# AlgoLab/PIntron

Hardware: AMD Instinct MI355X
Metric: ESTs aligned/sec (whole node) + DP Mcells/s; bit-exact factorizations vs ref (higher is better)
Workload: dtype u8/int32

## Files before the change

include/pintron_gpu.h:

```cpp
#ifndef PINTRON_GPU_H
#define PINTRON_GPU_H

#include <stddef.h>
#include <stdint.h>

#ifdef __cplusplus
extern "C" {
#endif

#define PGPU_OK       0
#define PGPU_EDEVICE (-5)
#define PGPU_ENOMEM  (-12)
#define PGPU_EINVAL  (-22)
#define PGPU_ENOSPC  (-28)
#define PGPU_ERANGE  (-34)
#define PGPU_ENOSYS  (-38)

typedef struct pgpu_ctx pgpu_ctx;
typedef struct pgpu_index pgpu_index;
typedef struct pgpu_dp_plan pgpu_dp_plan;

int pgpu_init(int device, pgpu_ctx** ctx);
int pgpu_destroy(pgpu_ctx* ctx);
const char* pgpu_last_error(const pgpu_ctx* ctx);
// ... 85 lines not shown
  uint64_t est_off; uint32_t est_len;
  uint32_t first_exon, n_exons;
  uint32_t reserved;
  int32_t  suffpref_length_on_est, suffpref_length_for_intron, suffpref_length_on_gen, min_intron_length;
} pgpu_chain_query;

typedef struct {
  int32_t  status;
  uint32_t done;
  uint32_t dropped_first;
  uint32_t pad;
} pgpu_chain_result;

int pgpu_index_refine_chains(pgpu_ctx* ctx, const pgpu_index* idx, const char* ests, size_t ests_len,
                             const pgpu_factor* exons, size_t n_exons_total,
                             const pgpu_chain_query* q, size_t n,
                             pgpu_factor* out_exons, uint8_t* out_steps, pgpu_chain_result* out);
double pgpu_index_refine_chains_kernel_ms(void);

typedef struct {
  uint32_t min_factor_len;
  uint32_t reserved;
  double   min_string_depth_rate;
} pgpu_pairing_params;

typedef struct { int32_t p, t, l; } pgpu_pairing;

int pgpu_pairings(pgpu_ctx* ctx, const pgpu_index* idx,
                  const char* patterns, const uint64_t* pat_off, size_t n_pat,
                  const pgpu_pairing_params* params,
                  pgpu_pairing* out, size_t out_cap, uint64_t* out_first, size_t* n_out);

typedef struct pgpu_pairing_plan pgpu_pairing_plan;
int pgpu_pairing_plan_create(pgpu_ctx* ctx, const pgpu_index* idx, const char* patterns,
                             const uint64_t* pat_off, size_t n_pat, pgpu_pairing_plan** plan);
int pgpu_pairing_plan_create_resident(pgpu_ctx* ctx, const pgpu_index* idx, const char* patterns,
                                      const uint64_t* pat_off, size_t n_pat, pgpu_pairing_plan** plan);
int pgpu_pairing_plan_run(pgpu_ctx* ctx, pgpu_pairing_plan* plan, const pgpu_pairing_params* params);
uint64_t pgpu_pairing_plan_count(const pgpu_pairing_plan* plan);
uint64_t pgpu_pairing_plan_positions(const pgpu_pairing_plan* plan);
double pgpu_pairing_plan_kernel_ms(const pgpu_pairing_plan* plan, int k);
int pgpu_pairing_plan_fetch(pgpu_ctx* ctx, pgpu_pairing_plan* plan, pgpu_pairing* out, size_t out_cap,
                            uint64_t* out_first);
int pgpu_pairing_plan_destroy(pgpu_ctx* ctx, pgpu_pairing_plan* plan);

typedef struct {
  uint32_t min_factor_len;
  int32_t  min_intron_length, max_intron_length;
  uint32_t max_pairings_in_MEG;
  double   max_prefix_discarded_rate, max_suffix_discarded_rate, max_freq_shortest_pairing;
  uint32_t trans_red, short_edge_comp;
} pgpu_meg_params;

#define PGPU_MEG_MAX_VERTICES 64
#define PGPU_MEG_MAX_DEGREE   32
#define PGPU_MEG_TOO_COMPLEX  1u
#define PGPU_MEG_UNAVAILABLE  2u
int pgpu_pairing_plan_run_meg(pgpu_ctx* ctx, pgpu_pairing_plan* plan, const pgpu_meg_params* params);
uint64_t pgpu_pairing_plan_meg_bytes(const pgpu_pairing_plan* plan);
int pgpu_pairing_plan_fetch_meg(pgpu_ctx* ctx, pgpu_pairing_plan* plan, void* out, size_t out_cap,
                                uint64_t* rec_first);
double pgpu_pairing_plan_meg_ms(const pgpu_pairing_plan* plan);

int pgpu_host_alloc(pgpu_ctx* ctx, size_t bytes, void** out);
int pgpu_host_free(pgpu_ctx* ctx, void* p);

typedef struct pgpu_comm pgpu_comm;
typedef struct { char bytes[128]; } pgpu_comm_id;
int pgpu_comm_unique_id(pgpu_ctx* ctx, pgpu_comm_id* id);
int pgpu_comm_init(pgpu_ctx* ctx, int rank, int world, const pgpu_comm_id* id, pgpu_comm** comm);
int pgpu_gather(pgpu_ctx* ctx, pgpu_comm* comm, const void* send, uint64_t send_bytes,
                void* recv, uint64_t recv_cap, uint64_t* counts);
int pgpu_allgather(pgpu_ctx* ctx, pgpu_comm* comm, const void* send, uint64_t bytes, void* recv);
int pgpu_comm_destroy(pgpu_ctx* ctx, pgpu_comm* comm);

enum pgpu_dp_kind {
  PGPU_DP_ALIGN = 0,
  PGPU_DP_GAP = 1,
  PGPU_DP_ED = 2,
  PGPU_DP_KBAND = 3,
  PGPU_DP_LCF = 4,
  PGPU_DP_BORDERS = 5,
  PGPU_DP_AFFIX = 6,
  PGPU_DP_NKINDS = 7
};

#define PGPU_JOB_A_GENOMIC 1u
#define PGPU_JOB_B_GENOMIC 2u

typedef struct {
  uint32_t kind;
  uint32_t flags;
  uint64_t a_off, b_off;
  uint32_t a_len, b_len;
  uint32_t p0, p1, p2;
  uint32_t tail;
} pgpu_dp_job;

typedef struct {
  int32_t status;
  int32_t v[6];
  int32_t pad;
  uint64_t str[2];
} pgpu_dp_result;

#define PGPU_MAX_ROWS_LEV     65536u
#define PGPU_MAX_ROWS_BORDERS 4096u
#define PGPU_MAX_ROWS_GAP     2048u
#define PGPU_MAX_GAP_SIDE    16000u
#define PGPU_MAX_GAP_CELLS (1ull << 27)
#define PGPU_MAX_COLS      1048576u

int pgpu_dp_plan_create(pgpu_ctx* ctx, const pgpu_index* idx,
                        const pgpu_dp_job* jobs, size_t n_jobs,
                        const char* arena, size_t arena_len, pgpu_dp_plan** plan);
typedef struct { const pgpu_dp_job* jobs; size_t n_jobs; const char* arena; size_t arena_len; } pgpu_dp_part;
int pgpu_dp_plan_create_parts(pgpu_ctx* ctx, const pgpu_index* idx, const pgpu_dp_part* parts, size_t n_parts,
                              pgpu_dp_plan** plan);
int pgpu_dp_plan_launch(pgpu_ctx* ctx, pgpu_dp_plan* plan);
int pgpu_dp_plan_sync(pgpu_ctx* ctx, pgpu_dp_plan* plan);
size_t pgpu_dp_plan_string_bytes(const pgpu_dp_plan* plan);
int pgpu_dp_plan_fetch(pgpu_ctx* ctx, pgpu_dp_plan* plan, pgpu_dp_result* results,
                       char* strings, size_t strings_cap);
int pgpu_dp_plan_results_to_device(pgpu_ctx* ctx, pgpu_dp_plan* plan, void* device_dst, size_t cap);
int pgpu_dp_plan_destroy(pgpu_ctx* ctx, pgpu_dp_plan* plan);

uint64_t pgpu_dp_plan_cells(const pgpu_dp_plan* plan, int kind);
uint64_t pgpu_dp_plan_algo_bytes(const pgpu_dp_plan* plan, int kind);
double   pgpu_dp_plan_kernel_ms(const pgpu_dp_plan* plan, int kind);
uint64_t pgpu_dp_plan_launches(const pgpu_dp_plan* plan, int kind);

typedef struct {
  char     name[48];
  int32_t  kind;
  int32_t  pad;
  uint64_t jobs, cells, algo_bytes;
  double   ms;
  double   t0_ms;
} pgpu_group_info;
int pgpu_dp_plan_n_groups(const pgpu_dp_plan* plan);
int pgpu_dp_plan_group_info(const pgpu_dp_plan* plan, int i, pgpu_group_info* out);

int pgpu_dp_batch(pgpu_ctx* ctx, const pgpu_index* idx,
                  const pgpu_dp_job* jobs, size_t n_jobs, const char* arena, size_t arena_len,
                  pgpu_dp_result* results, char* strings, size_t strings_cap,
                  size_t* strings_used);

#ifdef __cplusplus
}
#endif
#endif
```

pintron_amd/capi.py:

```python
import ctypes as C
import os

_HERE = os.path.dirname(os.path.abspath(__file__))
LIB_PATH = os.path.join(_HERE, "lib", "libpintron_gpu.so")

PGPU_OK, PGPU_EDEVICE, PGPU_ENOMEM, PGPU_EINVAL, PGPU_ENOSPC, PGPU_ERANGE, PGPU_ENOSYS = \
    0, -5, -12, -22, -28, -34, -38
ALIGN, GAP, ED, KBAND, LCF, BORDERS, AFFIX = range(7)
KIND_NAMES = ["ALIGN", "GAP", "ED", "KBAND", "LCF", "BORDERS", "AFFIX"]
JOB_A_GENOMIC, JOB_B_GENOMIC = 1, 2


class DpJob(C.Structure):
    _fields_ = [("kind", C.c_uint32), ("flags", C.c_uint32), ("a_off", C.c_uint64),
                ("b_off", C.c_uint64), ("a_len", C.c_uint32), ("b_len", C.c_uint32),
                ("p0", C.c_uint32), ("p1", C.c_uint32), ("p2", C.c_uint32), ("tail", C.c_uint32)]


class DpResult(C.Structure):
    _fields_ = [("status", C.c_int32), ("v", C.c_int32 * 6), ("pad", C.c_int32),
                ("str", C.c_uint64 * 2)]


class GroupInfo(C.Structure):
    _fields_ = [("name", C.c_char * 48), ("kind", C.c_int32), ("pad", C.c_int32),
                ("jobs", C.c_uint64), ("cells", C.c_uint64), ("algo_bytes", C.c_uint64),
                ("ms", C.c_double), ("t0_ms", C.c_double)]


class PairingParams(C.Structure):
    _fields_ = [("min_factor_len", C.c_uint32), ("reserved", C.c_uint32),
                ("min_string_depth_rate", C.c_double)]


class Pairing(C.Structure):
    _fields_ = [("p", C.c_int32), ("t", C.c_int32), ("l", C.c_int32)]


class FindQuery(C.Structure):
    _fields_ = [("pat_off", C.c_uint64), ("pat_len", C.c_uint32), ("reserved", C.c_uint32),
                ("lo", C.c_uint32), ("hi", C.c_uint32)]


class Intron(C.Structure):
    _fields_ = [("start", C.c_uint32), ("end", C.c_uint32)]


class SexonQuery(C.Structure):
    _fields_ = [("e_off", C.c_uint64), ("elen", C.c_uint32), ("allgstart", C.c_uint32), ("allglen", C.c_uint32),
                ("f1slen", C.c_uint32), ("f2plen", C.c_uint32), ("min_intron_len", C.c_uint32), ("reserved", C.c_uint32)]


class SexonResult(C.Structure):
    _fields_ = [("status", C.c_int32), ("len", C.c_uint32), ("offstart", C.c_uint32), ("offend", C.c_uint32),
                ("gpos", C.c_uint32), ("i1type", C.c_uint32), ("i2type", C.c_uint32), ("pad", C.c_uint32)]


class Factor(C.Structure):
    _fields_ = [("EST_start", C.c_int32), ("EST_end", C.c_int32), ("GEN_start", C.c_int32), ("GEN_end", C.c_int32)]


class RefineQuery(C.Structure):
    _fields_ = [("est_off", C.c_uint64), ("est_len", C.c_uint32), ("flags", C.c_uint32), ("rows_off", C.c_uint64),
                ("dim", C.c_uint32), ("factor_cut", C.c_int32), ("intron_start", C.c_int32), ("intron_end", C.c_int32),
                ("intron_start_on_align", C.c_int32), ("intron_end_on_align", C.c_int32), ("donor", Factor), ("acceptor", Factor),
                ("suffpref_length_on_est", C.c_int32), ("suffpref_length_for_intron", C.c_int32),
                ("suffpref_length_on_gen", C.c_int32), ("min_intron_length", C.c_int32)]


class RefineResult(C.Structure):
    _fields_ = [("status", C.c_int32), ("refined", C.c_int32), ("path", C.c_int32), ("pad", C.c_int32),
                ("donor", Factor), ("acceptor", Factor)]


class ChainQuery(C.Structure):
    _fields_ = [("est_off", C.c_uint64), ("est_len", C.c_uint32), ("first_exon", C.c_uint32), ("n_exons", C.c_uint32),
                ("reserved", C.c_uint32), ("suffpref_length_on_est", C.c_int32), ("suffpref_length_for_intron", C.c_int32),
                ("suffpref_length_on_gen", C.c_int32), ("min_intron_length", C.c_int32)]


class ChainResult(C.Structure):
    _fields_ = [("status", C.c_int32), ("done", C.c_uint32), ("dropped_first", C.c_uint32), ("pad", C.c_uint32)]


REFINE_MAX_DIM, REFINE_MAX_ED, REFINE_FIRST_INTRON = 1024, 256, 1
CHAIN_MAX_EST_WINDOW, CHAIN_MAX_GEN_WINDOW = 192, 320
_FACTOR_DTYPE = [("EST_start", "<i4"), ("EST_end", "<i4"), ("GEN_start", "<i4"), ("GEN_end", "<i4")]
REFINE_QUERY_DTYPE = [("est_off", "<u8"), ("est_len", "<u4"), ("flags", "<u4"), ("rows_off", "<u8"), ("dim", "<u4"),
                      ("factor_cut", "<i4"), ("intron_start", "<i4"), ("intron_end", "<i4"), ("intron_start_on_align", "<i4"),
                      ("intron_end_on_align", "<i4"), ("donor", _FACTOR_DTYPE), ("acceptor", _FACTOR_DTYPE),
                      ("suffpref_length_on_est", "<i4"), ("suffpref_length_for_intron", "<i4"), ("suffpref_length_on_gen", "<i4"),
                      ("min_intron_length", "<i4")]
REFINE_RESULT_DTYPE = [("status", "<i4"), ("refined", "<i4"), ("path", "<i4"), ("pad", "<i4"), ("donor", _FACTOR_DTYPE),
                       ("acceptor", _FACTOR_DTYPE)]

CHAIN_QUERY_DTYPE = [("est_off", "<u8"), ("est_len", "<u4"), ("first_exon", "<u4"), ("n_exons", "<u4"), ("reserved", "<u4"),
                     ("suffpref_length_on_est", "<i4"), ("suffpref_length_for_intron", "<i4"), ("suffpref_length_on_gen", "<i4"),
                     ("min_intron_length", "<i4")]
CHAIN_RESULT_DTYPE = [("status", "<i4"), ("done", "<u4"), ("dropped_first", "<u4"), ("pad", "<u4")]
FACTOR_DTYPE = _FACTOR_DTYPE

SEXON_MAX_ELEN = 64
SEXON_QUERY_DTYPE = [("e_off", "<u8"), ("elen", "<u4"), ("allgstart", "<u4"), ("allglen", "<u4"), ("f1slen", "<u4"),
                     ("f2plen", "<u4"), ("min_intron_len", "<u4"), ("reserved", "<u4"), ("_pad", "<u4")]
SEXON_RESULT_DTYPE = [("status", "<i4"), ("len", "<u4"), ("offstart", "<u4"), ("offend", "<u4"), ("gpos", "<u4"),
                      ("i1type", "<u4"), ("i2type", "<u4"), ("pad", "<u4")]

assert C.sizeof(DpJob) == 48 and C.sizeof(DpResult) == 48 and C.sizeof(FindQuery) == 24
assert C.sizeof(Intron) == 8 and C.sizeof(SexonQuery) == 40 and C.sizeof(SexonResult) == 32
assert C.sizeof(Factor) == 16 and C.sizeof(RefineQuery) == 96 and C.sizeof(RefineResult) == 48
assert C.sizeof(ChainQuery) == 40 and C.sizeof(ChainResult) == 16

EXPORTS = [
    "pgpu_init", "pgpu_destroy", "pgpu_last_error", "pgpu_abi_version", "pgpu_set_timing", "pgpu_device_numa_node",
    "pgpu_index_build", "pgpu_index_destroy", "pgpu_index_suffix_array", "pgpu_index_save", "pgpu_index_load", "pgpu_pairings",
    "pgpu_index_find", "pgpu_index_find_kernel_ms",
    "pgpu_index_classify", "pgpu_index_score5", "pgpu_index_small_exons", "pgpu_index_small_exons_kernel_ms",
    "pgpu_index_refine_introns", "pgpu_index_refine_introns_kernel_ms",
    "pgpu_index_refine_chains", "pgpu_index_refine_chains_kernel_ms",
    "pgpu_pairing_plan_create", "pgpu_pairing_plan_create_resident", "pgpu_pairing_plan_run", "pgpu_pairing_plan_count",
    "pgpu_pairing_plan_positions", "pgpu_pairing_plan_kernel_ms", "pgpu_pairing_plan_fetch",
    "pgpu_pairing_plan_destroy",
    "pgpu_pairing_plan_run_meg", "pgpu_pairing_plan_meg_bytes", "pgpu_pairing_plan_fetch_meg",
    "pgpu_pairing_plan_meg_ms", "pgpu_host_alloc", "pgpu_host_free",
    "pgpu_comm_unique_id", "pgpu_comm_init", "pgpu_gather", "pgpu_allgather", "pgpu_comm_destroy",
    "pgpu_range_push", "pgpu_range_pop", "pgpu_build_info",
    "pgpu_dp_plan_create", "pgpu_dp_plan_create_parts", "pgpu_dp_plan_launch", "pgpu_dp_plan_sync",
    "pgpu_dp_plan_string_bytes", "pgpu_dp_plan_fetch", "pgpu_dp_plan_destroy",
    "pgpu_dp_plan_results_to_device",
    "pgpu_dp_plan_cells", "pgpu_dp_plan_algo_bytes", "pgpu_dp_plan_kernel_ms",
    "pgpu_dp_plan_launches", "pgpu_dp_plan_n_groups", "pgpu_dp_plan_group_info", "pgpu_dp_batch",
]

_lib = None


class PgpuError(RuntimeError):
    def __init__(self, code, msg):
        super().__init__("pgpu error %d: %s" % (code, msg))
        self.code = code


def lib():
    global _lib
    if _lib is None:
        if not os.path.exists(LIB_PATH):
            raise ImportError("%s is missing: run `python -c 'import __graft_entry__ as g; "
                              "g.build()'` (hipcc --offload-arch=gfx950)" % LIB_PATH)
        L = C.CDLL(LIB_PATH)
        vp, u64, sz = C.c_void_p, C.c_uint64, C.c_size_t
        L.pgpu_init.argtypes = [C.c_int, C.POINTER(vp)]
        L.pgpu_destroy.argtypes = [vp]
        L.pgpu_set_timing.argtypes = [vp, C.c_int]
        L.pgpu_last_error.argtypes = [vp]
        L.pgpu_last_error.restype = C.c_char_p
        L.pgpu_build_info.restype = C.c_char_p
        L.pgpu_range_push.argtypes = [C.c_char_p]
        L.pgpu_range_push.restype = None
        L.pgpu_range_pop.restype = None
        L.pgpu_allgather.argtypes = [vp, vp, vp, u64, vp]
        L.pgpu_index_build.argtypes = [vp, C.c_char_p, sz, C.POINTER(vp)]
        L.pgpu_index_destroy.argtypes = [vp, vp]
        L.pgpu_index_save.argtypes = [vp, vp, C.c_char_p, C.c_char_p]
        L.pgpu_index_load.argtypes = [vp, C.c_char_p, C.c_char_p, sz, C.POINTER(vp)]
        L.pgpu_index_suffix_array.argtypes = [vp, vp, C.POINTER(C.c_uint32), sz]
        L.pgpu_index_find.argtypes = [vp, vp, C.c_char_p, sz, C.POINTER(FindQuery), sz,
                                      C.POINTER(C.c_uint32), sz, C.POINTER(u64), C.POINTER(sz)]
        L.pgpu_index_find_kernel_ms.argtypes = [C.c_int]
        L.pgpu_index_find_kernel_ms.restype = C.c_double
        L.pgpu_index_classify.argtypes = [vp, vp, C.POINTER(Intron), sz, C.POINTER(C.c_uint8)]
        L.pgpu_index_score5.argtypes = [vp, vp, C.c_int, C.POINTER(C.c_double), sz]
        L.pgpu_index_small_exons.argtypes = [vp, vp, C.c_char_p, sz, C.POINTER(SexonQuery), sz, C.POINTER(SexonResult)]
        L.pgpu_index_small_exons_kernel_ms.argtypes = []
        L.pgpu_index_small_exons_kernel_ms.restype = C.c_double
        L.pgpu_index_refine_introns.argtypes = [vp, vp, C.c_char_p, sz, C.c_char_p, sz, C.POINTER(RefineQuery), sz,
                                                C.POINTER(RefineResult)]
        L.pgpu_index_refine_introns_kernel_ms.argtypes = []
        L.pgpu_index_refine_introns_kernel_ms.restype = C.c_double
        L.pgpu_index_refine_chains.argtypes = [vp, vp, C.c_char_p, sz, C.POINTER(Factor), sz, C.POINTER(ChainQuery), sz,
                                               C.POINTER(Factor), C.POINTER(C.c_uint8), C.POINTER(ChainResult)]
        L.pgpu_index_refine_chains_kernel_ms.argtypes = []
        L.pgpu_index_refine_chains_kernel_ms.restype = C.c_double
        L.pgpu_pairing_plan_run_meg.argtypes = [vp, vp, vp]
        L.pgpu_pairing_plan_meg_bytes.argtypes = [vp]
        L.pgpu_pairing_plan_meg_bytes.restype = u64
        L.pgpu_pairing_plan_meg_ms.argtypes = [vp]
        L.pgpu_pairing_plan_meg_ms.restype = C.c_double
        L.pgpu_pairing_plan_fetch_meg.argtypes = [vp, vp, vp, sz, C.POINTER(u64)]
        L.pgpu_host_alloc.argtypes = [vp, sz, C.POINTER(vp)]
        L.pgpu_host_free.argtypes = [vp, vp]
        L.pgpu_comm_unique_id.argtypes = [vp, vp]
        L.pgpu_comm_init.argtypes = [vp, C.c_int, C.c_int, vp, C.POINTER(vp)]
        L.pgpu_gather.argtypes = [vp, vp, C.c_char_p, u64, vp, u64, C.POINTER(u64)]
        L.pgpu_comm_destroy.argtypes = [vp, vp]
        L.pgpu_pairings.argtypes = [vp, vp, C.c_char_p, C.POINTER(u64), sz,
                                    C.POINTER(PairingParams), C.POINTER(Pairing), sz,
                                    C.POINTER(u64), C.POINTER(sz)]
        L.pgpu_pairing_plan_create.argtypes = [vp, vp, C.c_char_p, C.POINTER(u64), sz, C.POINTER(vp)]
        L.pgpu_pairing_plan_create_resident.argtypes = [vp, vp, C.c_char_p, C.POINTER(u64), sz, C.POINTER(vp)]
        L.pgpu_pairing_plan_run.argtypes = [vp, vp, C.POINTER(PairingParams)]
        L.pgpu_pairing_plan_count.argtypes = [vp]
        L.pgpu_pairing_plan_count.restype = u64
        L.pgpu_pairing_plan_positions.argtypes = [vp]
        L.pgpu_pairing_plan_positions.restype = u64
        L.pgpu_pairing_plan_kernel_ms.argtypes = [vp, C.c_int]
        L.pgpu_pairing_plan_kernel_ms.restype = C.c_double
        L.pgpu_pairing_plan_fetch.argtypes = [vp, vp, C.POINTER(Pairing), sz, C.POINTER(u64)]
        L.pgpu_pairing_plan_destroy.argtypes = [vp, vp]
        L.pgpu_dp_plan_create_parts.argtypes = [vp, vp, vp, sz, C.POINTER(vp)]
        L.pgpu_dp_plan_create.argtypes = [vp, vp, C.POINTER(DpJob), sz, C.c_char_p, sz,
                                          C.POINTER(vp)]
        L.pgpu_dp_plan_launch.argtypes = [vp, vp]
        L.pgpu_dp_plan_sync.argtypes = [vp, vp]
        L.pgpu_dp_plan_string_bytes.argtypes = [vp]
        L.pgpu_dp_plan_string_bytes.restype = sz
        L.pgpu_dp_plan_fetch.argtypes = [vp, vp, C.POINTER(DpResult), C.c_char_p, sz]
        L.pgpu_dp_plan_destroy.argtypes = [vp, vp]
        L.pgpu_dp_plan_results_to_device.argtypes = [vp, vp, vp, sz]
        for nm in ("pgpu_dp_plan_cells", "pgpu_dp_plan_algo_bytes", "pgpu_dp_plan_launches"):
            getattr(L, nm).argtypes = [vp, C.c_int]
            getattr(L, nm).restype = u64
        L.pgpu_dp_plan_kernel_ms.argtypes = [vp, C.c_int]
        L.pgpu_dp_plan_kernel_ms.restype = C.c_double
        L.pgpu_dp_plan_n_groups.argtypes = [vp]
        L.pgpu_dp_plan_group_info.argtypes = [vp, C.c_int, C.POINTER(GroupInfo)]
        L.pgpu_dp_batch.argtypes = [vp, vp, C.POINTER(DpJob), sz, C.c_char_p, sz,
                                    C.POINTER(DpResult), C.c_char_p, sz, C.POINTER(sz)]
        _lib = L
    return _lib


class Context:

    def __init__(self, device=0):
        self.L = lib()
        self.h = C.c_void_p()
        rc = self.L.pgpu_init(device, C.byref(self.h))
        if rc != PGPU_OK:
            raise PgpuError(rc, "pgpu_init(%d) failed (no usable gfx950 device?)" % device)
        self.L.pgpu_set_timing(self.h, 1)

    def check(self, rc):
        if rc != PGPU_OK:
            raise PgpuError(rc, self.L.pgpu_last_error(self.h).decode())

    def close(self):
        if self.h:
            self.L.pgpu_destroy(self.h)
            self.h = C.c_void_p()

    def __enter__(self):
        return self

    def __exit__(self, *a):
        self.close()


class Index:
    def __init__(self, ctx: Context, genomic: bytes, load_from=None):
        self.ctx = ctx
        self.h = C.c_void_p()
        self.n = len(genomic)
        self.genomic = genomic
        if load_from is None:
            ctx.check(ctx.L.pgpu_index_build(ctx.h, genomic, len(genomic), C.byref(self.h)))
        else:
            rc = ctx.L.pgpu_index_load(ctx.h, os.fsencode(load_from), genomic, len(genomic), C.byref(self.h))
            if rc != PGPU_OK:
                raise PgpuError(rc, "index file %s does not fit this sequence" % load_from)

    def save(self, path):
        self.ctx.check(self.ctx.L.pgpu_index_save(self.ctx.h, self.h, self.genomic, os.fsencode(path)))

    def suffix_array(self):
        import numpy as np
        sa = np.empty(self.n, dtype=np.uint32)
        self.ctx.check(self.ctx.L.pgpu_index_suffix_array(
            self.ctx.h, self.h, sa.ctypes.data_as(C.POINTER(C.c_uint32)), self.n))
        return sa

    def find_raw(self, blob: bytes, queries, n_queries: int, out=None):
        import numpy as np
        first = np.zeros(n_queries + 1, dtype=np.uint64)
        total = C.c_size_t(0)
        rc = self.ctx.L.pgpu_index_find(
            self.ctx.h, self.h, blob, len(blob), queries, n_queries,
            out.ctypes.data_as(C.POINTER(C.c_uint32)) if out is not None else None, len(out) if out is not None else 0,
            first.ctypes.data_as(C.POINTER(C.c_uint64)), C.byref(total))
        return rc, first, total.value

    def find(self, patterns, windows=None):
        import numpy as np
        n = len(patterns)
        if windows is None:
            windows = [(0, self.n)] * n
        if len(windows) != n:
            raise ValueError("one window per pattern")
        lens = np.fromiter((len(p) for p in patterns), dtype=np.uint64, count=n)
        offs = np.zeros(n + 1, dtype=np.uint64)
        np.cumsum(lens, out=offs[1:])
        q = np.zeros(n, dtype=np.dtype([("pat_off", "<u8"), ("pat_len", "<u4"), ("reserved", "<u4"),
                                        ("lo", "<u4"), ("hi", "<u4")]))
        q["pat_off"], q["pat_len"] = offs[:n], lens
        if n:
            w = np.asarray(windows, dtype=np.uint32).reshape(n, 2)
            q["lo"], q["hi"] = w[:, 0], w[:, 1]
# ... 123 lines not shown
        self._blob = b"".join(patterns)
        self._off = np.zeros(len(patterns) + 1, dtype=np.uint64)
        np.cumsum([len(p) for p in patterns], out=self._off[1:])
        self.h = C.c_void_p()
        create = ctx.L.pgpu_pairing_plan_create_resident if resident else ctx.L.pgpu_pairing_plan_create
        ctx.check(create(ctx.h, index.h, self._blob, self._off.ctypes.data_as(C.POINTER(C.c_uint64)),
                         self.n_pat, C.byref(self.h)))

    def run(self, min_factor_len=15, rate=0.2):
        prm = PairingParams(min_factor_len, 0, rate)
        self.ctx.check(self.ctx.L.pgpu_pairing_plan_run(self.ctx.h, self.h, C.byref(prm)))
        return self.ctx.L.pgpu_pairing_plan_count(self.h)

    def stage_ms(self):
        return {s: self.ctx.L.pgpu_pairing_plan_kernel_ms(self.h, k) for k, s in enumerate(self.STAGES)}

    def fetch(self):
        import numpy as np
        n = self.ctx.L.pgpu_pairing_plan_count(self.h)
        out = np.zeros((max(n, 1), 3), dtype=np.int32)
        first = np.zeros(self.n_pat + 1, dtype=np.uint64)
        self.ctx.check(self.ctx.L.pgpu_pairing_plan_fetch(
            self.ctx.h, self.h, out.ctypes.data_as(C.POINTER(Pairing)), n,
            first.ctypes.data_as(C.POINTER(C.c_uint64))))
        return out[:n], first

    def run_meg(self, min_factor_len=15, min_intron_length=40, max_intron_length=0, max_pairings_in_MEG=80,
                max_prefix_discarded_rate=0.6, max_suffix_discarded_rate=0.6, max_freq_shortest_pairing=0.4,
                trans_red=True, short_edge_comp=True):
        prm = MegParams(min_factor_len, min_intron_length, max_intron_length, max_pairings_in_MEG,
                        max_prefix_discarded_rate, max_suffix_discarded_rate, max_freq_shortest_pairing,
                        int(trans_red), int(short_edge_comp))
        self.ctx.check(self.ctx.L.pgpu_pairing_plan_run_meg(self.ctx.h, self.h, C.byref(prm)))
        return self.ctx.L.pgpu_pairing_plan_meg_bytes(self.h)

    def fetch_meg(self):
        import numpy as np
        n = self.ctx.L.pgpu_pairing_plan_meg_bytes(self.h)
        out = np.zeros(max(n, 1), dtype=np.uint8)
        first = np.zeros(self.n_pat + 1, dtype=np.uint64)
        self.ctx.check(self.ctx.L.pgpu_pairing_plan_fetch_meg(
            self.ctx.h, self.h, out.ctypes.data_as(C.c_void_p), n, first.ctypes.data_as(C.POINTER(C.c_uint64))))
        raw = out.tobytes()
        return [raw[int(first[i]):int(first[i + 1])] for i in range(self.n_pat)]

    def close(self):
        if self.h:
            self.ctx.L.pgpu_pairing_plan_destroy(self.ctx.h, self.h)
            self.h = C.c_void_p()


class DpPart(C.Structure):
    _fields_ = [("jobs", C.c_void_p), ("n_jobs", C.c_size_t), ("arena", C.c_void_p), ("arena_len", C.c_size_t)]


class JobList:

    def __init__(self):
        self.jobs = []
        self.chunks = []
        self.size = 0

    def _put(self, b: bytes) -> int:
        off = self.size
        self.chunks.append(b)
        self.size += len(b)
        return off

    def add(self, kind, a: bytes, b: bytes, p0=0, p1=0, p2=0, b_tail: bytes = b"",
            a_gen_off=None, b_gen_off=None, tail=None):
        flags = 0
        if a_gen_off is None:
            a_off = self._put(a)
        else:
            a_off, flags = a_gen_off, flags | JOB_A_GENOMIC
        if b_gen_off is None:
            b_off = self._put(b + b_tail)
        else:
            b_off, flags = b_gen_off, flags | JOB_B_GENOMIC
        self.jobs.append(DpJob(kind, flags, a_off, b_off, len(a), len(b), p0, p1, p2,
                               len(b_tail) if tail is None else tail))
        return len(self.jobs) - 1

    def arrays(self):
        arr = (DpJob * max(len(self.jobs), 1))(*self.jobs)
        return arr, b"".join(self.chunks)


class Plan:
    def __init__(self, ctx: Context, joblist: JobList, index: Index = None):
        self.ctx = ctx
        self.n = len(joblist.jobs)
        self._jobs, self._arena = joblist.arrays()
        self.h = C.c_void_p()
        ctx.check(ctx.L.pgpu_dp_plan_create(ctx.h, index.h if index else None, self._jobs, self.n,
                                            self._arena, len(self._arena), C.byref(self.h)))

    @classmethod
    def from_parts(cls, ctx: Context, joblists, index: Index = None):
        self = cls.__new__(cls)
        self.ctx = ctx
        self.n = sum(len(jl.jobs) for jl in joblists)
        self._keep = []
        parts = (DpPart * max(len(joblists), 1))()
        for k, jl in enumerate(joblists):
            jobs, arena = jl.arrays()
            buf = C.create_string_buffer(arena, len(arena) + 1)
            self._keep += [jobs, buf]
            parts[k] = DpPart(C.cast(jobs, C.c_void_p), len(jl.jobs), C.cast(buf, C.c_void_p), len(arena))
        self.h = C.c_void_p()
        ctx.check(ctx.L.pgpu_dp_plan_create_parts(ctx.h, index.h if index else None, parts, len(joblists), C.byref(self.h)))
        return self

    def launch(self):
        self.ctx.check(self.ctx.L.pgpu_dp_plan_launch(self.ctx.h, self.h))

    def sync(self):
        self.ctx.check(self.ctx.L.pgpu_dp_plan_sync(self.ctx.h, self.h))

    def fetch(self):
        L = self.ctx.L
        nbytes = L.pgpu_dp_plan_string_bytes(self.h)
        res = (DpResult * max(self.n, 1))()
        sbuf = C.create_string_buffer(max(nbytes, 1))
        self.ctx.check(L.pgpu_dp_plan_fetch(self.ctx.h, self.h, res, sbuf, nbytes))
        return res, sbuf.raw

    def results_to_device(self, device_ptr: int, cap: int):
        self.ctx.check(self.ctx.L.pgpu_dp_plan_results_to_device(self.ctx.h, self.h, device_ptr, cap))

    def groups(self):
        L = self.ctx.L
        out = []
        for i in range(L.pgpu_dp_plan_n_groups(self.h)):
            g = GroupInfo()
            L.pgpu_dp_plan_group_info(self.h, i, C.byref(g))
            out.append(dict(name=g.name.decode(), kind=g.kind, jobs=g.jobs, cells=g.cells,
                            algo_bytes=g.algo_bytes, ms=g.ms, t0_ms=g.t0_ms))
        return out

    def close(self):
        if self.h:
            self.ctx.L.pgpu_dp_plan_destroy(self.ctx.h, self.h)
            self.h = C.c_void_p()


def cstr(buf: bytes, off: int) -> bytes:
    end = buf.index(b"\0", off)
    return buf[off:end]


def decode(kind, r: DpResult, strings: bytes):
    v = r.v
    if r.status != PGPU_OK:
        return dict(status=r.status)
    if kind == ALIGN:
        return dict(status=0, score=v[0], dim=v[1], ea=cstr(strings, r.str[0]),
                    ga=cstr(strings, r.str[1]))
    if kind == GAP:
        return dict(status=0, dim=v[0], factor_cut=v[1], intron_start=v[2], intron_end=v[3],
                    intron_start_on_align=v[4], intron_end_on_align=v[5],
                    ea=cstr(strings, r.str[0]), ga=cstr(strings, r.str[1]))
    if kind == ED:
        return dict(status=0, score=v[0])
    if kind == KBAND:
        return dict(status=0, ok=v[0], edit=v[1], dust=v[2])
    if kind == LCF:
        return dict(status=0, len=v[0], occ1=v[1], occ2=v[2])
    if kind == BORDERS:
        return dict(status=0, ok=v[0], off_p=v[1], off_t1=v[2], off_t2=v[3], ed=v[4])
    if kind == AFFIX:
        return dict(status=0, valid=v[0], ecut=v[1], gcut=v[2])
    raise ValueError(kind)


def run_jobs(ctx: Context, joblist: JobList, index: Index = None):
    plan = Plan(ctx, joblist, index)
    try:
        plan.launch()
        plan.sync()
        res, strings = plan.fetch()
        return [decode(joblist.jobs[i].kind, res[i], strings) for i in range(plan.n)]
    finally:
        plan.close()
```

pintron_amd/csrc/pgpu_api.hip:

```cpp
#include <algorithm>
#include <cstdarg>
#include <cstdio>
#include <cstdlib>
#include <cstring>
#include <ctime>
#include <time.h>
#include <new>
#include <mutex>
#include <vector>

#include "pgpu_internal.h"
#include "pgpu_index.h"

struct BufPool {
  static constexpr int SLOTS = 24;
  void* ptr[SLOTS] = {nullptr};
  size_t cap[SLOTS] = {0};
  bool busy = false;
  int sharers = 0;
  const void* owner = nullptr;
};

struct pgpu_ctx {
  int device = 0;
  hipStream_t stream = nullptr;
  char err[512] = {0};
  BufPool pools[2];
  bool timing = false;
  static constexpr int NAUX = 4;
  hipStream_t aux[NAUX] = {nullptr};
  hipEvent_t ev_upload = nullptr;
  hipEvent_t ev_aux[NAUX] = {nullptr};
  hipEvent_t ev_done = nullptr;
  hipEvent_t ev_wait = nullptr;
  long wait_poll_us = 20;
  int poison = -1;
  void* pin[2] = {nullptr, nullptr};
  size_t pin_cap[2] = {0, 0};
  std::vector<hipEvent_t> ev_pool;
};

static int wait_stream(pgpu_ctx* ctx, hipStream_t st) {
  if (hipEventRecord(ctx->ev_done, st) != hipSuccess) return -1;
  if (ctx->wait_poll_us != 0) {
    for (;;) {
      const hipError_t q = hipEventQuery(ctx->ev_done);
      if (q == hipSuccess) return 0;
      if (q != hipErrorNotReady) return -1;
      if (ctx->wait_poll_us > 0) { struct timespec ts = {0, ctx->wait_poll_us * 1000L}; nanosleep(&ts, nullptr); }
    }
  }
  return hipEventSynchronize(ctx->ev_done) == hipSuccess ? 0 : -1;
}

static void* pinned(pgpu_ctx* ctx, int slot, size_t bytes) {
  if (ctx->pin_cap[slot] < bytes) {
    if (ctx->pin[slot]) (void)hipHostFree(ctx->pin[slot]);
    ctx->pin[slot] = nullptr; ctx->pin_cap[slot] = 0;
    const size_t want = std::max<size_t>(bytes + bytes / 2 + 4096, (size_t)2 << 20);
    if (hipHostMalloc(&ctx->pin[slot], want, hipHostMallocDefault) != hipSuccess) return nullptr;
    pgpu_trace_alloc(slot ? "ctx pinned down" : "ctx pinned up", ctx->pin[slot], want);
    ctx->pin_cap[slot] = want;
  }
  return ctx->pin[slot];
}

bool pgpu_ctx_pool_acquire(pgpu_ctx* ctx, int pool) {
  if (ctx->pools[pool].busy) return false;
  ctx->pools[pool].busy = true;
  return true;
}
void pgpu_ctx_pool_release(pgpu_ctx* ctx, int pool) { ctx->pools[pool].busy = false; ctx->pools[pool].owner = nullptr; }
bool pgpu_ctx_pool_share(pgpu_ctx* ctx, int pool) {
  BufPool& p = ctx->pools[pool];
  if (p.busy && p.sharers == 0) return false;
  p.busy = true; ++p.sharers;
  return true;
}
void pgpu_ctx_pool_unshare(pgpu_ctx* ctx, int pool, const void* who) {
  BufPool& p = ctx->pools[pool];
  if (p.owner == who) p.owner = nullptr;
  if (p.sharers > 0 && --p.sharers == 0) p.busy = false;
}
void pgpu_ctx_pool_set_owner(pgpu_ctx* ctx, int pool, const void* who) { ctx->pools[pool].owner = who; }
const void* pgpu_ctx_pool_owner(const pgpu_ctx* ctx, int pool) { return ctx->pools[pool].owner; }
void* pgpu_ctx_pool_get(pgpu_ctx* ctx, int pool, int slot, size_t bytes) {
  BufPool& p = ctx->pools[pool];
  if (bytes == 0) bytes = 16;
  if (p.cap[slot] < bytes) {
    if (p.ptr[slot]) (void)hipFree(p.ptr[slot]);
    p.ptr[slot] = nullptr; p.cap[slot] = 0;
    const size_t want = std::max<size_t>(bytes + bytes / 2 + 4096, pool == 0 ? (size_t)64 << 20 : 0);
    if (hipMalloc(&p.ptr[slot], want) != hipSuccess) {
      if (hipMalloc(&p.ptr[slot], bytes) != hipSuccess) return nullptr;
      p.cap[slot] = bytes;
    } else p.cap[slot] = want;
    pgpu_trace_alloc(pool ? "device pool 1" : "device pool 0", p.ptr[slot], p.cap[slot]);
  }
  return p.ptr[slot];
}
bool pgpu_ctx_timing(const pgpu_ctx* ctx) { return ctx->timing; }

extern "C" int pgpu_device_numa_node(pgpu_ctx* ctx) {
  if (!ctx) return -1;
  char bdf[64] = {0};
  if (hipDeviceGetPCIBusId(bdf, (int)sizeof bdf - 1, ctx->device) != hipSuccess) return -1;
  for (char* c = bdf; *c; ++c) if (*c >= 'A' && *c <= 'F') *c = (char)(*c - 'A' + 'a');
  char path[160];
  snprintf(path, sizeof path, "/sys/bus/pci/devices/%s/numa_node", bdf);
  FILE* f = fopen(path, "r");
  if (!f) return -1;
  int node = -1;
  if (fscanf(f, "%d", &node) != 1) node = -1;
  fclose(f);
  return node;
}

extern "C" int pgpu_set_timing(pgpu_ctx* ctx, int enabled) {
  if (!ctx) return PGPU_EINVAL;
  ctx->timing = enabled != 0;
  return PGPU_OK;
}

static int set_err(pgpu_ctx* ctx, int code, const char* fmt, ...) {
  if (ctx) {
    va_list ap;
    va_start(ap, fmt);
    vsnprintf(ctx->err, sizeof(ctx->err), fmt, ap);
    va_end(ap);
  }
  return code;
}

#define HIP_TRY(ctx, call)                                                                  \
  do {                                                                                      \
    hipError_t e_ = (call);                                                                 \
    if (e_ != hipSuccess)                                                                   \
      return set_err(ctx, e_ == hipErrorOutOfMemory ? PGPU_ENOMEM : PGPU_EDEVICE,           \
                     "%s failed: %s (%s:%d)", #call, hipGetErrorString(e_), __FILE__, __LINE__); \
  } while (0)

hipStream_t pgpu_ctx_stream(pgpu_ctx* ctx) { return ctx->stream; }
hipError_t pgpu_ctx_wait(pgpu_ctx* ctx) {
  if (ctx->wait_poll_us <= 0) return hipStreamSynchronize(ctx->stream);
  hipError_t e = hipEventRecord(ctx->ev_wait, ctx->stream);
  if (e != hipSuccess) return e;
  const struct timespec ts = {0, ctx->wait_poll_us * 5000L};
  for (;;) {
    e = hipEventQuery(ctx->ev_wait);
    if (e != hipErrorNotReady) return e;
    nanosleep(&ts, nullptr);
  }
}
int pgpu_ctx_bind(pgpu_ctx* ctx) {
  const hipError_t e = hipSetDevice(ctx->device);
  return e == hipSuccess ? PGPU_OK : set_err(ctx, PGPU_EDEVICE, "hipSetDevice(%d) failed: %s", ctx->device, hipGetErrorString(e));
}
int pgpu_ctx_fail(pgpu_ctx* ctx, int code, const char* msg) { return set_err(ctx, code, "%s", msg); }

extern "C" int pgpu_abi_version(void) { return 1; }

#include <dlfcn.h>
namespace {
struct Roctx { int state = 0; int (*push)(const char*) = nullptr; int (*pop)() = nullptr; };
Roctx g_roctx;
bool roctx_ready() {
  if (g_roctx.state) return g_roctx.state > 0;
  bool want = false;
  { const char* m = getenv("PGPU_MARKERS"); if (m) want = m[0] != '0'; else {
      const char* t = getenv("ROCP_TOOL_LIBRARIES"); const char* pl = getenv("LD_PRELOAD");
      want = (t && t[0]) || (pl && strstr(pl, "rocprofiler")); } }
  if (want) {
    void* so = nullptr;
    for (const char* n : { "librocprofiler-sdk-roctx.so.1", "librocprofiler-sdk-roctx.so", "libroctx64.so.4", "libroctx64.so" })
      if ((so = dlopen(n, RTLD_NOW | RTLD_GLOBAL)) != nullptr) break;
    if (so) {
      *(void**)(&g_roctx.push) = dlsym(so, "roctxRangePushA");
      *(void**)(&g_roctx.pop) = dlsym(so, "roctxRangePop");
    }
  }
  g_roctx.state = (g_roctx.push && g_roctx.pop) ? 1 : -1;
  return g_roctx.state > 0;
}
}
extern "C" void pgpu_range_push(const char* name) { if (roctx_ready()) g_roctx.push(name ? name : ""); }
extern "C" void pgpu_range_pop(void) { if (roctx_ready()) g_roctx.pop(); }

extern "C" const char* pgpu_build_info(void) {
  static char info[256];
  if (!info[0]) {
    const char* stamp = __DATE__ " " __TIME__ " " __VERSION__;
    unsigned long long h = 1469598103934665603ull;
    for (const char* c = stamp; *c; ++c) { h ^= (unsigned char)*c; h *= 1099511628211ull; }
    snprintf(info, sizeof info, "libpintron_gpu abi %d, gfx950, built %s %s, hip %d.%d.%d, stamp %016llx", pgpu_abi_version(), __DATE__,
             __TIME__, HIP_VERSION_MAJOR, HIP_VERSION_MINOR, HIP_VERSION_PATCH, h);
  }
  return info;
}

static bool aux_stream(pgpu_ctx* ctx, int i) {
  if (!ctx->aux[i] && hipStreamCreateWithFlags(&ctx->aux[i], hipStreamNonBlocking) != hipSuccess) { ctx->aux[i] = nullptr; return false; }
  if (!ctx->ev_aux[i] && hipEventCreateWithFlags(&ctx->ev_aux[i], hipEventDisableTiming) != hipSuccess) { ctx->ev_aux[i] = nullptr; return false; }
  return true;
}

static hipEvent_t g_base_event[64];
static std::mutex g_base_mu;
static hipEvent_t base_event(int device, hipStream_t st) {
  if (device < 0 || device >= 64) return nullptr;
  std::lock_guard<std::mutex> lk(g_base_mu);
  if (!g_base_event[device]) {
    hipEvent_t e = nullptr;
    if (hipEventCreate(&e) == hipSuccess && hipEventRecord(e, st) == hipSuccess && hipEventSynchronize(e) == hipSuccess) g_base_event[device] = e;
    else if (e) hipEventDestroy(e);
  }
  return g_base_event[device];
}

extern "C" int pgpu_init(int device, pgpu_ctx** out) {
  if (!out) return PGPU_EINVAL;
  *out = nullptr;
  int n = 0;
  if (hipGetDeviceCount(&n) != hipSuccess || n <= 0) return PGPU_EDEVICE;
  if (device < 0 || device >= n) return PGPU_EINVAL;
  hipDeviceProp_t prop;
  if (hipGetDeviceProperties(&prop, device) != hipSuccess) return PGPU_EDEVICE;
  if (strncmp(prop.gcnArchName, "gfx950", 6) != 0) return PGPU_EDEVICE;
  if (hipSetDevice(device) != hipSuccess) return PGPU_EDEVICE;
  pgpu_ctx* ctx = new (std::nothrow) pgpu_ctx();
  if (!ctx) return PGPU_ENOMEM;
  ctx->device = device;
  if (hipStreamCreateWithFlags(&ctx->stream, hipStreamNonBlocking) != hipSuccess) {
    delete ctx;
    return PGPU_EDEVICE;
  }
  if (hipEventCreateWithFlags(&ctx->ev_upload, hipEventDisableTiming) != hipSuccess) { delete ctx; return PGPU_EDEVICE; }
  if (hipEventCreateWithFlags(&ctx->ev_done, hipEventDisableTiming | hipEventBlockingSync) != hipSuccess) { delete ctx; return PGPU_EDEVICE; }
  if (hipEventCreateWithFlags(&ctx->ev_wait, hipEventDisableTiming) != hipSuccess) { delete ctx; return PGPU_EDEVICE; }
  { const char* f = getenv("PGPU_WAIT"); if (f) ctx->wait_poll_us = atol(f); }
  { const char* f = getenv("PGPU_POISON"); if (f && f[0]) ctx->poison = atoi(f) & 255; }
  base_event(device, ctx->stream);
  *out = ctx;
  return PGPU_OK;
}

extern "C" int pgpu_destroy(pgpu_ctx* ctx) {
  if (!ctx) return PGPU_EINVAL;
  hipSetDevice(ctx->device);
  hipStreamSynchronize(ctx->stream);
  for (auto& pl : ctx->pools) for (auto& q : pl.ptr) if (q) hipFree(q);
  for (auto& a : ctx->aux) if (a) { hipStreamSynchronize(a); hipStreamDestroy(a); }
  if (ctx->ev_upload) hipEventDestroy(ctx->ev_upload);
  if (ctx->ev_done) hipEventDestroy(ctx->ev_done);
  if (ctx->ev_wait) hipEventDestroy(ctx->ev_wait);
  for (auto& e : ctx->ev_aux) if (e) hipEventDestroy(e);
  for (auto& e : ctx->ev_pool) if (e) hipEventDestroy(e);
  for (auto& q : ctx->pin) if (q) hipHostFree(q);
  hipStreamDestroy(ctx->stream);
  delete ctx;
  return PGPU_OK;
}

extern "C" const char* pgpu_last_error(const pgpu_ctx* ctx) { return ctx ? ctx->err : "null context"; }

namespace {

uint32_t row_class(uint32_t rows) {
  if (rows > 4096u) return ROW_CLASS_STRIPS;
  uint32_t R = 1;
  while (64u * R < rows) R <<= 1;
  return R;
}

enum DpRoute : uint8_t {
  RT_ALIGN_STRIPS, RT_ALIGN_COOP, RT_ALIGN_WAVE, RT_GAP_SLOW, RT_GAP, RT_ED, RT_KBAND, RT_LCF,
  RT_BORDERS_SLOW, RT_BORDERS_COOP, RT_BORDERS_WAVE, RT_AFFIX_STRIPS, RT_AFFIX_COOP, RT_AFFIX_WAVE,
  RT_LCFSA, RT_LCFW, RT_ALIGNB,
  RT_BATCH,
  RT_COUNT
};

enum BatchPlace { OUTSIDE, SEGMENT, ROLE_BORDERS, ROLE_AFFIX, ROLE_ALIGN };

using WsBytes = size_t (*)(uint32_t la, uint32_t lb, uint32_t R);
size_t ws_align_wave(uint32_t, uint32_t lb, uint32_t) { return ((size_t)lb + 64) * 64; }
size_t ws_align_coop(uint32_t, uint32_t lb, uint32_t R) { return ((size_t)lb + 256) * 256 * align_coop_entry_bytes(R); }
size_t ws_align_strips(uint32_t la, uint32_t lb, uint32_t R) {
  return 2 * strip_bnd_bytes(lb) + (size_t)((la + 4095u) / 4096u) * ((size_t)lb + 64) * 64 * align_entry_bytes(R);
}
size_t ws_gap(uint32_t, uint32_t lb, uint32_t R) { return ((size_t)lb + 64) * 64 * gap_entry_bytes(R); }
size_t ws_gap_slow(uint32_t la, uint32_t lb, uint32_t) { return (size_t)9 * ((size_t)la + 1) * 4 + ((size_t)la + 1) * ((size_t)lb + 1); }
size_t ws_borders_slow(uint32_t la, uint32_t, uint32_t) { return (size_t)7 * ((size_t)la + 1) * 4; }
size_t ws_affix_strips(uint32_t, uint32_t lb, uint32_t) { return 2 * strip_bnd_bytes(lb); }
size_t ws_ed_strips(uint32_t la, uint32_t lb, uint32_t R) { return R == ROW_CLASS_STRIPS ? 2 * strip_bnd_bytes(std::max(la, lb)) : 0; }

using AlgoBytes = uint64_t (*)(uint64_t la, uint64_t lb, uint64_t p2);
uint64_t bytes_operands(uint64_t la, uint64_t lb, uint64_t) { return la + lb; }
uint64_t bytes_align(uint64_t la, uint64_t lb, uint64_t) { return la + lb + la * lb + 3 * (la + lb); }
uint64_t bytes_gap(uint64_t la, uint64_t lb, uint64_t) { return la + lb + 3 * la * lb + 3 * (la + lb); }
uint64_t bytes_borders(uint64_t la, uint64_t lb, uint64_t p2) { return la + std::min(lb, 2 * std::min(la + p2, lb)) + 2 * 8 * la; }
uint64_t bytes_lcfsa(uint64_t, uint64_t lb, uint64_t) { return lb + 64u * 96u; }

struct RouteInfo {
  const char* name;
  int kind;
  int family;
  WsBytes ws_bytes;
  bool strings;
  uint32_t cell_factor;
  AlgoBytes algo_bytes;
  BatchPlace place;
  int seg_pos;
  uint32_t big_from;
  long weight; bool by_rows; int lane; DpLauncher launch;
  bool keyed;
};

constexpr RouteInfo ROUTES[] = {
  {"lev_wave<ALIGN,strips>",  PGPU_DP_ALIGN,   KF_ALIGN,   ws_align_strips, true,  1, bytes_align,    OUTSIDE,      0,  0,  5000, false,  2, launch_align_big,    false},
  {"align_coop",              PGPU_DP_ALIGN,   KF_ALIGN,   ws_align_coop,   true,  1, bytes_align,    ROLE_ALIGN,   0,  0,     0, false,  0, nullptr,             false},
  {"lev_wave<ALIGN>",         PGPU_DP_ALIGN,   KF_ALIGN,   ws_align_wave,   true,  1, bytes_align,    SEGMENT,      1,  0,     0, false,  0, nullptr,             false},
  {"gap_slow",                PGPU_DP_GAP,     KF_GAP,     ws_gap_slow,     true,  3, bytes_gap,      OUTSIDE,      0,  0,  4000, false,  3, launch_gap_slow,     false},
  {"gap_wave",                PGPU_DP_GAP,     KF_GAP,     ws_gap,          true,  3, bytes_gap,      SEGMENT,      2,  8,  4000, false,  3, launch_gap_big,      false},
  {"lev_wave<ED>",            PGPU_DP_ED,      KF_ED,      ws_ed_strips,    false, 1, bytes_operands, SEGMENT,      8, 32,  1000, false,  1, launch_ed_big,       false},
  {"lev_wave<KBAND>",         PGPU_DP_KBAND,   KF_KBAND,   ws_ed_strips,    false, 1, bytes_operands, SEGMENT,      3, 32,  2000, false,  2, launch_kband_big,    false},
  {"lcf",                     PGPU_DP_LCF,     KF_LCF,     nullptr,         false, 1, bytes_operands, OUTSIDE,      0,  0,  3000, false,  3, launch_lcf,          true},
  {"borders_slow",            PGPU_DP_BORDERS, KF_BORDERS, ws_borders_slow, false, 2, bytes_borders,  OUTSIDE,      0,  0, 10000, true,   1, launch_borders_slow, false},
  {"borders_coop",            PGPU_DP_BORDERS, KF_BORDERS, nullptr,         false, 2, bytes_borders,  ROLE_BORDERS, 0,  0, 10000, true,   1, launch_borders_coop, false},
  {"lev_wave<BORDERS,R=1>",   PGPU_DP_BORDERS, KF_BORDERS, nullptr,         false, 2, bytes_borders,  SEGMENT,      4,  0,     0, false,  0, nullptr,             false},
  {"lev_wave<AFFIX,strips>",  PGPU_DP_AFFIX,   KF_AFFIX,   ws_affix_strips, false, 1, bytes_operands, OUTSIDE,      0,  0, 10000, true,   0, launch_affix_strips, false},
  {"affix_coop",              PGPU_DP_AFFIX,   KF_AFFIX,   nullptr,         false, 1, bytes_operands, ROLE_AFFIX,   0,  0,     0, false,  0, nullptr,             false},
  {"lev_wave<AFFIX,R=1>",     PGPU_DP_AFFIX,   KF_AFFIX,   nullptr,         false, 1, bytes_operands, SEGMENT,      5,  0,     0, false,  0, nullptr,             false},
  {"lcf_sa",                  PGPU_DP_LCF,     KF_LCFSA,   nullptr,         false, 0, bytes_lcfsa,    SEGMENT,      6,  0,     0, false,  0, nullptr,             false},
  {"lcf_small",               PGPU_DP_LCF,     KF_LCFW,    nullptr,         false, 1, bytes_operands, SEGMENT,      7,  0,     0, false,  0, nullptr,             false},
  {"align_band",              PGPU_DP_ALIGN,   KF_ALIGNB,  ws_align_coop,   true,  1, bytes_align,    SEGMENT,      0,  0,     0, false,  0, nullptr,             false},
  {"dp_batch",                PGPU_DP_ALIGN,   KF_COUNT,   nullptr,         false, 0, nullptr,        OUTSIDE,      0,  0, 20000, false, -1, nullptr,             false},
};
static_assert(sizeof ROUTES / sizeof ROUTES[0] == RT_COUNT, "one entry per route, in the enum's order");
constexpr bool routes_consistent() {
  unsigned seen = 0;
  for (const RouteInfo& ri : ROUTES) {
    if (ri.lane >= pgpu_ctx::NAUX) return false;
    if (ri.big_from && (ri.place != SEGMENT || !ri.launch)) return false;
    if (ri.place != SEGMENT) continue;
    if (ri.seg_pos >= MAX_WAVE_SEGS || (seen & (1u << ri.seg_pos))) return false;
    seen |= 1u << ri.seg_pos;
  }
  return true;
}
static_assert(routes_consistent(), "routing table");

struct Slice { size_t first = 0, count = 0; uint64_t cells = 0, algo_bytes = 0; };

struct Group {
  DpRoute route;
  Slice own;
  uint32_t max_chunks = 0, max_l2 = 0;
  uint32_t max_rows = 0;
  hipEvent_t ev0 = nullptr, ev1 = nullptr;
  float ms = 0.f;
  float t0_ms = -1.f;
};

struct BatchPlan {
  BatchDesc desc;
  uint32_t bc_max_rows;
  int ab_start, ab_count;
};

struct Keyed { DevJob j; uint64_t a_off, b_off; bool ag, bg; DpRoute route; uint32_t R; uint64_t size; };

}

struct pgpu_dp_plan {
  size_t n_jobs = 0;
  std::vector<Group> groups;
  std::vector<pgpu_dp_result> prefill;
  DevJob* d_jobs = nullptr;
  DevResult* d_results = nullptr;
  uint8_t* d_arena = nullptr;
  uint8_t* d_ws = nullptr;
  uint8_t* d_strs = nullptr;
  unsigned long long* d_keys = nullptr;
  size_t n_dev_jobs = 0, ws_bytes = 0, strs_bytes = 0, n_keys = 0;
  uint64_t cells[PGPU_DP_NKINDS] = {0}, algo_bytes[PGPU_DP_NKINDS] = {0};
  double ms[PGPU_DP_NKINDS] = {0};
  uint64_t launches[PGPU_DP_NKINDS] = {0};
  bool launched = false, synced = false;
  bool pooled = false;
  pgpu_ctx* owner = nullptr;
  uint8_t* d_base = nullptr;
  uint8_t* h_up = nullptr; uint8_t* h_down = nullptr;
  size_t up_bytes = 0, off_results = 0, down_bytes = 0;
  BatchPlan batch{};
  std::vector<uint32_t> lcf_out;
  size_t off_keys = 0;
  bool lcf_decoded = false;
};

static void plan_free(pgpu_dp_plan* p) {
  if (!p) return;
  if (p->pooled) pgpu_ctx_pool_release(p->owner, 0);
  else {
    for (auto& g : p->groups) {
      if (g.ev0) hipEventDestroy(g.ev0);
      if (g.ev1) hipEventDestroy(g.ev1);
    }
    if (p->d_base) hipFree(p->d_base);
    if (p->h_up) hipHostFree(p->h_up);
    if (p->h_down) hipHostFree(p->h_down);
  }
  delete p;
}

extern "C" int pgpu_dp_plan_create(pgpu_ctx* ctx, const pgpu_index* idx, const pgpu_dp_job* jobs,
                                   size_t n_jobs, const char* arena, size_t arena_len,
                                   pgpu_dp_plan** out) {
  const pgpu_dp_part one = { jobs, n_jobs, arena, arena_len };
  return pgpu_dp_plan_create_parts(ctx, idx, &one, 1, out);
}

static int classify(const pgpu_dp_job& in, const char* arena, bool ag, bool bg, const LcfIndexView& lcf, Keyed& k) {
  const uint32_t la = in.a_len, lb = in.b_len;
  k.size = (uint64_t)la * lb;
  switch (in.kind) {
    case PGPU_DP_ALIGN:
      if (la > PGPU_MAX_ROWS_LEV || lb > PGPU_MAX_COLS) return PGPU_ERANGE;
      k.R = row_class(la);
      if (la > 64u && la <= 4096u && (la > lb ? la - lb : lb - la) <= ALIGN_BAND_HALF) k.route = RT_ALIGNB;
      else k.route = k.R == 1 ? RT_ALIGN_WAVE : (k.R == ROW_CLASS_STRIPS ? RT_ALIGN_STRIPS : RT_ALIGN_COOP);
      return PGPU_OK;
    case PGPU_DP_GAP:
      if (lb > PGPU_MAX_GAP_SIDE || la > PGPU_MAX_GAP_SIDE || ((uint64_t)la + 1) * ((uint64_t)lb + 1) > PGPU_MAX_GAP_CELLS) return PGPU_ERANGE;
      k.R = la > PGPU_MAX_ROWS_GAP ? ROW_CLASS_STRIPS : row_class(la);
      k.route = k.R == ROW_CLASS_STRIPS ? RT_GAP_SLOW : RT_GAP;
      return PGPU_OK;
    case PGPU_DP_ED:
      if (std::min(la, lb) > PGPU_MAX_ROWS_LEV || std::max(la, lb) > PGPU_MAX_COLS) return PGPU_ERANGE;
      k.R = row_class(std::min(la, lb)); k.route = RT_ED;
      return PGPU_OK;
    case PGPU_DP_KBAND: {
      const uint32_t n = std::max(la, lb), m = std::min(la, lb), ub = in.p0;
      if (n > PGPU_MAX_COLS || m > PGPU_MAX_ROWS_LEV) return PGPU_ERANGE;
      k.R = row_class(m); k.route = RT_KBAND;
      if (2ull * ub + 1 < n) k.size = (uint64_t)m * (2ull * ub + 1);
      return PGPU_OK;
    }
    case PGPU_DP_LCF:
      if (lb > 65535u || la >= (1u << 28)) return PGPU_ERANGE;
      k.R = 0; k.route = RT_LCF;
      if (lcf.focc && lcf.rmq && ag && !bg && in.a_off == 0 && la <= lcf.first_bad && lb <= 64u) {
        const unsigned char* b = (const unsigned char*)arena + in.b_off;
        bool acgt = true;
        uint32_t n_wild = 0, wild_at = 0;
        for (uint32_t q = 0; q < lb && acgt; ++q) {
          if (b[q] == 'N' || b[q] == 'n') { ++n_wild; wild_at = q; }
          else acgt = b[q] == 'A' || b[q] == 'C' || b[q] == 'G' || b[q] == 'T';
        }
        if (acgt && n_wild <= 1u) { k.route = RT_LCFSA; k.j.p0 = n_wild ? wild_at + 1u : 0u; }
      }
      if (k.route == RT_LCF && (uint64_t)la * lb <= 16384u && la + lb <= 4096u) k.route = RT_LCFW;
      return PGPU_OK;
    case PGPU_DP_BORDERS: {
      const uint64_t t_win = std::min<uint64_t>((uint64_t)la + in.p2, lb);
      if (la > PGPU_MAX_ROWS_LEV || t_win > PGPU_MAX_COLS) return PGPU_ERANGE;
      if (in.p0 > in.p1 || in.p1 > la) return PGPU_EINVAL;
      k.R = row_class(la); k.size = (uint64_t)la * t_win;
      k.route = k.R == 1 ? RT_BORDERS_WAVE : (k.R == ROW_CLASS_STRIPS ? RT_BORDERS_SLOW : RT_BORDERS_COOP);
      return PGPU_OK;
    }
    case PGPU_DP_AFFIX:
      if (la > PGPU_MAX_ROWS_LEV || lb > PGPU_MAX_COLS) return PGPU_ERANGE;
      k.R = row_class(la);
      k.route = k.R == 1 ? RT_AFFIX_WAVE : (k.R == ROW_CLASS_STRIPS ? RT_AFFIX_STRIPS : RT_AFFIX_COOP);
      return PGPU_OK;
    default: return PGPU_EINVAL;
  }
}

static std::vector<Keyed> classify_jobs(const pgpu_dp_part* parts, size_t n_parts, size_t n_jobs, const LcfIndexView& lcf,
                                        bool has_genomic, size_t gen_len, std::vector<pgpu_dp_result>& prefill) {
  std::vector<Keyed> v;
  v.reserve(n_jobs);
  prefill.assign(n_jobs, pgpu_dp_result{});
  size_t i = 0, part_base = 0;
  for (size_t q = 0; q < n_parts; part_base += parts[q].arena_len, ++q)
    for (size_t w = 0; w < parts[q].n_jobs; ++w, ++i) {
      const pgpu_dp_job& in = parts[q].jobs[w];
      const size_t own_arena = parts[q].arena_len;
      prefill[i].status = PGPU_EINVAL;
      if (in.kind >= PGPU_DP_NKINDS) continue;
      const bool ag = in.flags & PGPU_JOB_A_GENOMIC, bg = in.flags & PGPU_JOB_B_GENOMIC;
      if ((ag || bg) && !has_genomic) continue;
      const size_t a_space = ag ? gen_len : own_arena, b_space = bg ? gen_len : own_arena;
      if (in.a_off > a_space || in.a_len > a_space - in.a_off) continue;
      if (in.b_off > b_space || in.b_len > b_space - in.b_off) continue;
      Keyed k{};
      k.a_off = in.a_off + (ag ? 0 : part_base); k.b_off = in.b_off + (bg ? 0 : part_base); k.ag = ag; k.bg = bg;
      k.j.la = in.a_len; k.j.lb = in.b_len;
      k.j.p0 = in.p0; k.j.p1 = in.p1; k.j.p2 = in.p2; k.j.tail = in.tail;
      k.j.out_idx = (uint32_t)i;
      prefill[i].status = classify(in, parts[q].arena, ag, bg, lcf, k);
      if (prefill[i].status != PGPU_OK) continue;
      k.j.r_class = k.R;
      v.push_back(k);
    }
  return v;
}

static void sort_jobs(std::vector<Keyed>& v) {
  auto key_of = [](const Keyed& k) -> uint32_t {
    uint32_t rcls = 0;
    while ((1u << rcls) < k.R) ++rcls;
    const uint32_t mag = 63u - (uint32_t)__builtin_clzll(k.size | 1ull);
    return ((uint32_t)ROUTES[k.route].family << 10) | ((7u - rcls) << 6) | (63u - mag);
  };
  constexpr uint32_t NKEYS = (uint32_t)KF_COUNT << 10;
  std::vector<uint32_t> start(NKEYS + 1, 0);
  std::vector<uint32_t> kk(v.size());
  for (size_t q = 0; q < v.size(); ++q) { kk[q] = key_of(v[q]); ++start[kk[q] + 1]; }
  for (uint32_t c = 0; c < NKEYS; ++c) start[c + 1] += start[c];
  std::vector<Keyed> sorted;
  sorted.resize(v.size());
  for (size_t q = 0; q < v.size(); ++q) sorted[start[kk[q]]++] = v[q];
  v.swap(sorted);
}

struct DpSpace { size_t ws = 0, strs = 0; };
static DpSpace assign_workspace(std::vector<Keyed>& v, std::vector<uint32_t>& lcf_out) {
  DpSpace sp;
  for (auto& k : v) {
    const RouteInfo& ri = ROUTES[k.route];
    const size_t wb = ri.ws_bytes ? ri.ws_bytes(k.j.la, k.j.lb, k.R) : 0;
    if (wb) { k.j.ws_off = sp.ws; sp.ws += wb; }
    if (ri.strings) { k.j.str_off = sp.strs; sp.strs += 2 * ((size_t)k.j.la + k.j.lb + 1); }
    if (ri.keyed) lcf_out.push_back(k.j.out_idx);
    sp.ws = (sp.ws + 15) & ~(size_t)15;
  }
  return sp;
}

static void form_groups(const std::vector<Keyed>& v, std::vector<Group>& groups, std::vector<Slice>& batched,
                        uint64_t* cells, uint64_t* algo_bytes) {
  for (size_t i = 0, j; i < v.size(); i = j) {
    const RouteInfo& ri = ROUTES[v[i].route];
    Group g{};
    g.route = v[i].route;
    Slice big, rest;
    for (j = i; j < v.size() && v[j].route == g.route && !(ri.keyed && j - i == 65535); ++j) {
      const Keyed& k = v[j];
      Slice& s = ri.big_from && k.R >= ri.big_from ? big : rest;
      ++s.count; s.cells += ri.cell_factor * k.size; s.algo_bytes += ri.algo_bytes(k.j.la, k.j.lb, k.j.p2);
      g.max_rows = std::max(g.max_rows, k.j.la);
      if (ri.keyed) {
        g.max_chunks = std::max(g.max_chunks, (uint32_t)(((uint64_t)k.j.la + k.j.lb + 254) / 256));
        g.max_l2 = std::max(g.max_l2, k.j.lb);
      }
    }
    big.first = i; rest.first = i + big.count;
    cells[ri.kind] += big.cells + rest.cells; algo_bytes[ri.kind] += big.algo_bytes + rest.algo_bytes;
    const bool in_batch = ri.place == ROLE_BORDERS ? dp_batch_lds_bytes(true, 1, g.max_rows, 1, 1) <= DP_BATCH_MAX_LDS : ri.place != OUTSIDE;
    g.own = in_batch ? big : rest;
    groups.push_back(g);
    batched.push_back(in_batch ? rest : Slice{});
  }
}

static void form_batch(std::vector<Group>& groups, const std::vector<Slice>& batched, BatchPlan& b) {
  Group m{};
  m.route = RT_BATCH;
  const Slice* seg[MAX_WAVE_SEGS] = {nullptr};
  int seg_family[MAX_WAVE_SEGS] = {0};
  BatchDesc& d = b.desc;
  for (size_t gi = 0; gi < groups.size(); ++gi) {
    const Slice& s = batched[gi];
    if (!s.count) continue;
    const RouteInfo& ri = ROUTES[groups[gi].route];
    switch (ri.place) {
      case SEGMENT:      seg[ri.seg_pos] = &s; seg_family[ri.seg_pos] = ri.family; break;
      case ROLE_BORDERS: d.bc_start = (int)s.first; d.bc_count = (int)s.count; b.bc_max_rows = groups[gi].max_rows; break;
      case ROLE_AFFIX:   d.ac_start = (int)s.first; d.ac_count = (int)s.count; break;
      case ROLE_ALIGN:   d.lc_start = (int)s.first; d.lc_count = (int)s.count; break;
      case OUTSIDE:      break;
    }
    if (groups[gi].route == RT_ALIGNB) { b.ab_start = (int)s.first; b.ab_count = (int)s.count; }
    m.own.count += s.count; m.own.cells += s.cells; m.own.algo_bytes += s.algo_bytes;
  }
  int waves = 0;
  for (int q = 0; q < MAX_WAVE_SEGS; ++q) {
    if (!seg[q]) continue;
    d.segs.family[d.segs.n] = seg_family[q]; d.segs.start[d.segs.n] = (int)seg[q]->first; d.segs.count[d.segs.n] = (int)seg[q]->count;
    ++d.segs.n;
    waves += (int)seg[q]->count;
  }
  d.wave_blocks = (waves + 3) / 4;
  if (m.own.count) groups.push_back(m);
}

static int plan_upload(pgpu_ctx* ctx, pgpu_dp_plan* p, const pgpu_dp_part* parts, size_t n_parts, size_t arena_len,
                       const std::vector<Keyed>& v, const uint8_t* d_gen) {
  if (ctx->timing) {
    const size_t need = 2 * p->groups.size();
    if (p->pooled) {
      while (ctx->ev_pool.size() < need) {
        hipEvent_t e = nullptr;
        if (hipEventCreate(&e) != hipSuccess) return set_err(ctx, PGPU_EDEVICE, "hipEventCreate failed");
        ctx->ev_pool.push_back(e);
      }
      for (size_t g = 0; g < p->groups.size(); ++g) { p->groups[g].ev0 = ctx->ev_pool[2 * g]; p->groups[g].ev1 = ctx->ev_pool[2 * g + 1]; }
    } else {
      for (auto& g : p->groups)
        if (hipEventCreate(&g.ev0) != hipSuccess || hipEventCreate(&g.ev1) != hipSuccess) return set_err(ctx, PGPU_EDEVICE, "hipEventCreate failed");
    }
  }

  auto up256 = [](size_t x) { return (x + 255) & ~(size_t)255; };
  const size_t n_jobs = p->n_jobs, strs = p->strs_bytes;
  const size_t off_arena = 0;
  const size_t off_jobs = up256(arena_len + 16);
  const size_t off_keys = up256(off_jobs + std::max<size_t>(v.size(), 1) * sizeof(DevJob));
  const size_t off_results = up256(off_keys + (p->n_keys + 1) * sizeof(unsigned long long));
  const size_t off_strs = off_results + std::max<size_t>(n_jobs, 1) * sizeof(DevResult);
  const size_t off_ws = up256(off_strs + strs + 16);
  const size_t total = off_ws + p->ws_bytes + 16;
  p->up_bytes = off_strs;
  p->off_results = off_results;
  p->off_keys = off_keys;
  p->down_bytes = (off_strs - off_keys) + strs;
  if (p->pooled) {
    p->d_base = (uint8_t*)pgpu_ctx_pool_get(ctx, 0, 0, total);
    p->h_up = (uint8_t*)pinned(ctx, 0, p->up_bytes);
    p->h_down = (uint8_t*)pinned(ctx, 1, p->down_bytes + 16);
  } else {
    void* q = nullptr;
    if (hipMalloc(&q, total) == hipSuccess) p->d_base = (uint8_t*)q;
    if (hipHostMalloc(&q, p->up_bytes, hipHostMallocDefault) == hipSuccess) p->h_up = (uint8_t*)q;
    if (hipHostMalloc(&q, p->down_bytes + 16, hipHostMallocDefault) == hipSuccess) p->h_down = (uint8_t*)q;
  }
  if (!p->d_base || !p->h_up || !p->h_down)
    return set_err(ctx, PGPU_ENOMEM, "batch buffers (%zu B device, %zu B pinned) could not be allocated", total, p->up_bytes + p->down_bytes);
  p->d_arena = p->d_base + off_arena;
  p->d_jobs = (DevJob*)(p->d_base + off_jobs);
  p->d_keys = (unsigned long long*)(p->d_base + off_keys);
  p->d_results = (DevResult*)(p->d_base + off_results);
  p->d_strs = p->d_base + off_strs;
  p->d_ws = p->d_base + off_ws;

  {
    size_t at = off_arena;
    for (size_t q = 0; q < n_parts; ++q) { if (parts[q].arena_len) memcpy(p->h_up + at, parts[q].arena, parts[q].arena_len); at += parts[q].arena_len; }
  }
  DevJob* hj = (DevJob*)(p->h_up + off_jobs);
  for (size_t q = 0; q < v.size(); ++q) {
    DevJob d = v[q].j;
    d.a = (v[q].ag ? d_gen : p->d_arena) + v[q].a_off;
    d.b = (v[q].bg ? d_gen : p->d_arena) + v[q].b_off;
    hj[q] = d;
  }
  memset(p->h_up + off_keys, 0, off_results - off_keys);
  if (n_jobs) memcpy(p->h_up + off_results, p->prefill.data(), n_jobs * sizeof(DevResult));
  const hipError_t e = hipMemcpyAsync(p->d_base, p->h_up, p->up_bytes, hipMemcpyHostToDevice, ctx->stream);
  if (e != hipSuccess) return set_err(ctx, PGPU_EDEVICE, "upload failed: %s", hipGetErrorString(e));
  if (ctx->poison >= 0) {
    if (hipMemsetAsync(p->d_base + off_strs, ctx->poison, total - off_strs, ctx->stream) != hipSuccess) return set_err(ctx, PGPU_EDEVICE, "poison fill failed");
  }
  return PGPU_OK;
}

extern "C" int pgpu_dp_plan_create_parts(pgpu_ctx* ctx, const pgpu_index* idx, const pgpu_dp_part* parts,
                                         size_t n_parts, pgpu_dp_plan** out) {
  if (!ctx || !out || (n_parts && !parts)) return set_err(ctx, PGPU_EINVAL, "bad argument");
  *out = nullptr;
  size_t n_jobs = 0, arena_len = 0;
  for (size_t q = 0; q < n_parts; ++q) {
    if ((parts[q].n_jobs && !parts[q].jobs) || (parts[q].arena_len && !parts[q].arena)) return set_err(ctx, PGPU_EINVAL, "bad argument");
    n_jobs += parts[q].n_jobs; arena_len += parts[q].arena_len;
  }
  if (n_jobs >= (size_t)1 << 30) return set_err(ctx, PGPU_EINVAL, "too many jobs");
  HIP_TRY(ctx, hipSetDevice(ctx->device));
  pgpu_dp_plan* p = new (std::nothrow) pgpu_dp_plan();
  if (!p) return set_err(ctx, PGPU_ENOMEM, "out of host memory");
  p->n_jobs = n_jobs;
  p->owner = ctx;
  p->pooled = pgpu_ctx_pool_acquire(ctx, 0);
  p->batch.desc.ix = pgpu_index_lcf_view(idx);

  std::vector<Keyed> v = classify_jobs(parts, n_parts, n_jobs, p->batch.desc.ix, idx != nullptr, idx ? pgpu_index_length(idx) : 0, p->prefill);
  sort_jobs(v);
  const DpSpace sp = assign_workspace(v, p->lcf_out);
  p->ws_bytes = sp.ws; p->strs_bytes = sp.strs; p->n_keys = p->lcf_out.size(); p->n_dev_jobs = v.size();
  std::vector<Slice> batched;
  form_groups(v, p->groups, batched, p->cells, p->algo_bytes);
  form_batch(p->groups, batched, p->batch);

  const int rc = plan_upload(ctx, p, parts, n_parts, arena_len, v, idx ? pgpu_index_genomic(idx) : nullptr);
  if (rc != PGPU_OK) { plan_free(p); return rc; }
  *out = p;
  return PGPU_OK;
}

extern "C" int pgpu_dp_plan_launch(pgpu_ctx* ctx, pgpu_dp_plan* p) {
  if (!ctx || !p) return set_err(ctx, PGPU_EINVAL, "bad argument");
  HIP_TRY(ctx, hipSetDevice(ctx->device));
  p->synced = false; p->lcf_decoded = false;
  std::vector<size_t> order;
  std::vector<size_t> key_of(p->groups.size(), 0);
  auto weight = [&](size_t gi) -> long {
    const RouteInfo& ri = ROUTES[p->groups[gi].route];
    return ri.weight + (ri.by_rows ? (long)p->groups[gi].max_rows : 0);
  };
  {
    size_t kb = 0;
    for (size_t gi = 0; gi < p->groups.size(); ++gi) {
      const Group& g = p->groups[gi];
      if (ROUTES[g.route].keyed) { key_of[gi] = kb; kb += g.own.count; }
      if (g.own.count) order.push_back(gi);
    }
    std::stable_sort(order.begin(), order.end(), [&](size_t a, size_t b) { return weight(a) > weight(b); });
  }
  unsigned used_mask = 0;
  for (size_t gi : order) { const int l = ROUTES[p->groups[gi].route].lane; if (l >= 0) used_mask |= 1u << l; }
  if (used_mask) {
    HIP_TRY(ctx, hipEventRecord(ctx->ev_upload, ctx->stream));
    for (int i = 0; i < pgpu_ctx::NAUX; ++i)
      if (used_mask & (1u << i)) {
        if (!aux_stream(ctx, i)) return set_err(ctx, PGPU_EDEVICE, "auxiliary stream %d could not be created", i);
        HIP_TRY(ctx, hipStreamWaitEvent(ctx->aux[i], ctx->ev_upload, 0));
      }
  }
  for (size_t gi : order) {
    Group& g = p->groups[gi];
    const RouteInfo& ri = ROUTES[g.route];
    hipStream_t st = ri.lane >= 0 ? ctx->aux[ri.lane] : ctx->stream;
    if (g.ev0) HIP_TRY(ctx, hipEventRecord(g.ev0, st));
    pgpu_range_push(ri.name);
    struct PopAtExit { ~PopAtExit() { pgpu_range_pop(); } } pop_at_exit;
    if (g.route == RT_BATCH) {
      if (!launch_dp_batch(p->d_jobs, p->batch.desc, p->batch.bc_max_rows, p->d_results, p->d_ws, p->d_strs, st))
        return set_err(ctx, PGPU_EDEVICE, "batch launch: LDS budget exceeded");
    } else {
      if (!ri.launch) return set_err(ctx, PGPU_EDEVICE, "no kernel for %zu jobs of %s outside the batch launch", g.own.count, ri.name);
      ri.launch(DpLaunch{p->d_jobs + g.own.first, (int)g.own.count, g.max_rows, g.max_chunks, g.max_l2, p->d_results, p->d_ws,
                         p->d_strs, p->d_keys + key_of[gi], st});
    }
    if (g.ev1) HIP_TRY(ctx, hipEventRecord(g.ev1, st));
    if (g.route == RT_BATCH) launch_align_fallback(p->d_jobs + p->batch.ab_start, p->batch.ab_count, p->d_results, p->d_ws, p->d_strs, st);
    HIP_TRY(ctx, hipGetLastError());
  }
  for (int i = 0; i < pgpu_ctx::NAUX; ++i) {
    if (!(used_mask & (1u << i))) continue;
    HIP_TRY(ctx, hipEventRecord(ctx->ev_aux[i], ctx->aux[i]));
    HIP_TRY(ctx, hipStreamWaitEvent(ctx->stream, ctx->ev_aux[i], 0));
  }
  if (p->down_bytes)
    HIP_TRY(ctx, hipMemcpyAsync(p->h_down, p->d_base + p->off_keys, p->down_bytes, hipMemcpyDeviceToHost, ctx->stream));
  p->launched = true;
  return PGPU_OK;
}

static void decode_lcf_keys(pgpu_dp_plan* p) {
  if (p->lcf_decoded) return;
  p->lcf_decoded = true;
  const unsigned long long* keys = (const unsigned long long*)p->h_down;
  DevResult* res = (DevResult*)(p->h_down + (p->off_results - p->off_keys));
  for (size_t k = 0; k < p->lcf_out.size(); ++k) {
    DevResult& r = res[p->lcf_out[k]];
    const unsigned long long key = keys[k];
    r.status = PGPU_OK;
    r.v[0] = (int32_t)(key >> 44);
    r.v[1] = key ? (int32_t)(0x0FFFFFFFu - (uint32_t)((key >> 16) & 0x0FFFFFFFu)) : 0;
    r.v[2] = key ? (int32_t)(0xFFFFu - (uint32_t)(key & 0xFFFFu)) : 0;
  }
}

extern "C" int pgpu_dp_plan_sync(pgpu_ctx* ctx, pgpu_dp_plan* p) {
  if (!ctx || !p) return set_err(ctx, PGPU_EINVAL, "bad argument");
  if (wait_stream(ctx, ctx->stream) != 0) return set_err(ctx, PGPU_EDEVICE, "waiting for the batch failed");
  p->synced = p->launched;
  if (p->launched) {
    decode_lcf_keys(p);
    for (int k = 0; k < PGPU_DP_NKINDS; ++k) { p->ms[k] = 0; p->launches[k] = 0; }
    for (auto& g : p->groups) {
      float ms = 0.f;
      if (!g.own.count) continue;
      if (g.ev0 && g.ev1 && hipEventElapsedTime(&ms, g.ev0, g.ev1) == hipSuccess) g.ms = ms;
      if (g.ev0) { hipEvent_t b = base_event(ctx->device, ctx->stream); float t0 = 0.f; g.t0_ms = (b && hipEventElapsedTime(&t0, b, g.ev0) == hipSuccess) ? t0 : -1.f; }
      p->ms[ROUTES[g.route].kind] += g.ms;
      p->launches[ROUTES[g.route].kind] += 1;
    }
  }
  return PGPU_OK;
}

extern "C" size_t pgpu_dp_plan_string_bytes(const pgpu_dp_plan* p) { return p ? p->strs_bytes : 0; }

extern "C" int pgpu_dp_plan_fetch(pgpu_ctx* ctx, pgpu_dp_plan* p, pgpu_dp_result* results,
                                  char* strings, size_t cap) {
  if (!ctx || !p || (p->n_jobs && !results)) return set_err(ctx, PGPU_EINVAL, "bad argument");
  if (p->strs_bytes && strings && cap < p->strs_bytes) return set_err(ctx, PGPU_ENOSPC, "string buffer too small: need %zu", p->strs_bytes);
  if (!p->launched) return set_err(ctx, PGPU_EINVAL, "the plan has not been launched");
  if (!p->synced && wait_stream(ctx, ctx->stream) != 0) return set_err(ctx, PGPU_EDEVICE, "result download failed");
  p->synced = true;
  decode_lcf_keys(p);
  const size_t rb = p->n_jobs * sizeof(DevResult);
  if (rb) memcpy(results, p->h_down + (p->off_results - p->off_keys), rb);
  if (p->strs_bytes && strings) memcpy(strings, p->h_down + (p->down_bytes - p->strs_bytes), p->strs_bytes);
  return PGPU_OK;
}

extern "C" int pgpu_dp_plan_results_to_device(pgpu_ctx* ctx, pgpu_dp_plan* p, void* dst, size_t cap) {
  if (!ctx || !p || !dst) return set_err(ctx, PGPU_EINVAL, "bad argument");
  const size_t bytes = p->n_jobs * sizeof(DevResult);
  if (cap < bytes) return set_err(ctx, PGPU_ENOSPC, "device buffer too small: need %zu", bytes);
  HIP_TRY(ctx, hipSetDevice(ctx->device));
  if (!p->launched) return set_err(ctx, PGPU_EINVAL, "the plan has not been launched");
  if (!p->synced && wait_stream(ctx, ctx->stream) != 0) return set_err(ctx, PGPU_EDEVICE, "result download failed");
  p->synced = true;
  decode_lcf_keys(p);
  if (bytes) HIP_TRY(ctx, hipMemcpyAsync(dst, p->h_down + (p->off_results - p->off_keys), bytes, hipMemcpyHostToDevice, ctx->stream));
  HIP_TRY(ctx, hipStreamSynchronize(ctx->stream));
  return PGPU_OK;
}

extern "C" int pgpu_dp_plan_destroy(pgpu_ctx* ctx, pgpu_dp_plan* p) {
  if (!ctx || !p) return PGPU_EINVAL;
  hipSetDevice(ctx->device);
  hipStreamSynchronize(ctx->stream);
  plan_free(p);
  return PGPU_OK;
}

extern "C" uint64_t pgpu_dp_plan_cells(const pgpu_dp_plan* p, int kind) {
  return (p && kind >= 0 && kind < PGPU_DP_NKINDS) ? p->cells[kind] : 0;
}
extern "C" uint64_t pgpu_dp_plan_algo_bytes(const pgpu_dp_plan* p, int kind) {
  return (p && kind >= 0 && kind < PGPU_DP_NKINDS) ? p->algo_bytes[kind] : 0;
}
extern "C" double pgpu_dp_plan_kernel_ms(const pgpu_dp_plan* p, int kind) {
  return (p && kind >= 0 && kind < PGPU_DP_NKINDS) ? p->ms[kind] : 0.0;
}
extern "C" uint64_t pgpu_dp_plan_launches(const pgpu_dp_plan* p, int kind) {
  return (p && kind >= 0 && kind < PGPU_DP_NKINDS) ? p->launches[kind] : 0;
}

extern "C" int pgpu_dp_plan_n_groups(const pgpu_dp_plan* p) { return p ? (int)p->groups.size() : 0; }

extern "C" int pgpu_dp_plan_group_info(const pgpu_dp_plan* p, int i, pgpu_group_info* out) {
  if (!p || !out || i < 0 || i >= (int)p->groups.size()) return PGPU_EINVAL;
  const Group& g = p->groups[i];
  memset(out, 0, sizeof(*out));
  snprintf(out->name, sizeof(out->name), "%s", ROUTES[g.route].name);
  out->kind = ROUTES[g.route].kind; out->jobs = g.own.count; out->cells = g.own.cells; out->algo_bytes = g.own.algo_bytes;
  out->ms = g.ms; out->t0_ms = g.t0_ms;
  return PGPU_OK;
}

extern "C" int pgpu_dp_batch(pgpu_ctx* ctx, const pgpu_index* idx, const pgpu_dp_job* jobs,
                             size_t n_jobs, const char* arena, size_t arena_len,
                             pgpu_dp_result* results, char* strings, size_t strings_cap,
                             size_t* strings_used) {
  pgpu_dp_plan* p = nullptr;
  int rc = pgpu_dp_plan_create(ctx, idx, jobs, n_jobs, arena, arena_len, &p);
  if (rc != PGPU_OK) return rc;
  if (strings_used) *strings_used = p->strs_bytes;
  rc = pgpu_dp_plan_launch(ctx, p);
  if (rc == PGPU_OK) rc = pgpu_dp_plan_sync(ctx, p);
  if (rc == PGPU_OK) rc = pgpu_dp_plan_fetch(ctx, p, results, strings, strings_cap);
  pgpu_dp_plan_destroy(ctx, p);
  return rc;
}
```

pintron_amd/csrc/pgpu_chain.hip:

```cpp
#include <stdlib.h>
#include <string.h>

#include "pgpu_internal.h"
#include "pgpu_wave_dp.h"
#include "pgpu_refine_body.h"

namespace {

constexpr int MAX_EW = PGPU_CHAIN_MAX_EST_WINDOW;
constexpr int MAX_GW = PGPU_CHAIN_MAX_GEN_WINDOW;
constexpr uint32_t CHAIN_R = 4;
static_assert(MAX_EW <= 64 * (int)CHAIN_R && MAX_EW + MAX_GW <= MAX_DIM, "the caps fit the sweep and the decision");

constexpr size_t WS_DIRS = ((size_t)MAX_GW + 64) * 64 * CHAIN_R;
constexpr size_t WS_STRS = WS_DIRS;
constexpr size_t WS_STRS_BYTES = (2 * ((size_t)MAX_EW + MAX_GW + 1) + 15) & ~(size_t)15;
constexpr size_t WS_WIN_E = WS_STRS + WS_STRS_BYTES;
constexpr size_t WS_WIN_G = WS_WIN_E + ((MAX_EW + 15) & ~15);
constexpr size_t WS_RES = WS_WIN_G + ((MAX_GW + 15) & ~15);
constexpr size_t WS_WAVE = (WS_RES + sizeof(DevResult) + 255) & ~(size_t)255;

struct ChainLds {
  union {
    struct { __attribute__((aligned(16))) uint8_t win[TB_WIN_BYTES]; uint8_t path[TB_PATH]; } tb;
    RefineLds refine;
  };
};

__device__ __forceinline__ int append_piece(uint8_t* dst, int at, int cap, const Seq& s, int index, int length, int lane) {
  if (at > cap) return at;
  if (index < 0) { length += index; index = 0; }
  if (length > cap - at + 1) length = cap - at + 1;
  const Piece p = substring(s, index, length, lane);
  if (p.len > cap - at) return cap + 1;
  for (int k = lane; k < p.len; k += 64) dst[at + k] = s.p[p.start + k];
  return at + p.len;
}

__global__ __launch_bounds__(64)
void chain_kernel(const uint8_t* __restrict__ T, uint32_t n, const uint8_t* __restrict__ ests, const pgpu_factor* __restrict__ exons,
                  const pgpu_chain_query* __restrict__ queries, uint32_t n_chains, uint8_t* __restrict__ ws,
                  pgpu_factor* __restrict__ out_exons, uint8_t* __restrict__ out_steps, pgpu_chain_result* __restrict__ out) {
  __shared__ ChainLds S;
  const int lane = (int)threadIdx.x;
  uint8_t* const w = ws + (size_t)blockIdx.x * WS_WAVE;
  uint8_t* const win_e = w + WS_WIN_E;
  uint8_t* const win_g = w + WS_WIN_G;
  DevResult* const res = reinterpret_cast<DevResult*>(w + WS_RES);
  for (uint32_t c = blockIdx.x; c < n_chains; c += gridDim.x) {
    const pgpu_chain_query q = queries[c];
    Seq est, gen;
    est.p = ests + q.est_off; est.len = (int)q.est_len;
    gen.p = T; gen.len = (int)n;
    const int sp_est = q.suffpref_length_on_est, sp_int = q.suffpref_length_for_intron, sp_gen = q.suffpref_length_on_gen;
    pgpu_chain_result cr;
    cr.status = PGPU_OK; cr.done = 0; cr.dropped_first = 0; cr.pad = 0;
    pgpu_factor donor = exons[q.first_exon];
    const int first_est_start = donor.EST_start;
    int second_est_start = 0;
    uint32_t i = 0;
    for (; i + 1 < q.n_exons; ++i) {
      const pgpu_factor acceptor = exons[q.first_exon + i + 1];
      int dsl_gen = donor.GEN_start;
      if (donor.GEN_end - sp_gen + 1 >= dsl_gen) dsl_gen = donor.GEN_end - sp_gen + 1;
      int dsl_est = donor.EST_start;
      if (donor.EST_end - sp_est + 1 >= dsl_est) dsl_est = donor.EST_end - sp_est + 1;
      int apr_gen = acceptor.GEN_end;
      if (acceptor.GEN_start + sp_gen - 1 <= apr_gen) apr_gen = acceptor.GEN_start + sp_gen - 1;
      int apr_est = acceptor.EST_end;
      if (acceptor.EST_start + sp_est - 1 <= apr_est) apr_est = acceptor.EST_start + sp_est - 1;
      int le = 0, lg = 0;
      le = append_piece(win_e, le, MAX_EW, est, dsl_est, donor.EST_end - dsl_est + 1, lane);
      if (donor.EST_end != acceptor.EST_start - 1)
        le = append_piece(win_e, le, MAX_EW, est, donor.EST_end + 1, acceptor.EST_start - donor.EST_end - 1, lane);
      le = append_piece(win_e, le, MAX_EW, est, acceptor.EST_start, apr_est - acceptor.EST_start + 1, lane);
      lg = append_piece(win_g, lg, MAX_GW, gen, dsl_gen, donor.GEN_end - dsl_gen + 1, lane);
      lg = append_piece(win_g, lg, MAX_GW, gen, donor.GEN_end + 1, sp_int, lane);
      lg = append_piece(win_g, lg, MAX_GW, gen, acceptor.GEN_start - sp_int, sp_int, lane);
      lg = append_piece(win_g, lg, MAX_GW, gen, acceptor.GEN_start, apr_gen - acceptor.GEN_start + 1, lane);
      if (le > MAX_EW || lg > MAX_GW) { cr.status = PGPU_ERANGE; break; }
      DevJob job;
      job.a = win_e; job.b = win_g; job.la = (uint32_t)le; job.lb = (uint32_t)lg;
      job.p0 = job.p1 = job.p2 = job.tail = 0;
      job.ws_off = 0; job.str_off = WS_STRS; job.out_idx = 0;
      job.r_class = le <= 64 ? 1u : (le <= 128 ? 2u : 4u);
      own_stores_visible();
      switch (job.r_class) {
        case 1:  gap_wave_body<1>(job, res, w, (uint32_t)lane); break;
        case 2:  gap_wave_body<2>(job, res, w, (uint32_t)lane); break;
        default: gap_wave_body<4>(job, res, w, (uint32_t)lane); break;
      }
      own_stores_visible();
      gap_traceback_wave(job, res, w, w, (uint32_t)lane, S.tb.win, S.tb.path);
      own_stores_visible();
      pgpu_refine_query rq;
      rq.est_off = q.est_off; rq.est_len = q.est_len; rq.flags = i == 0 ? PGPU_REFINE_FIRST_INTRON : 0u;
      rq.rows_off = 0; rq.dim = (uint32_t)__builtin_amdgcn_readfirstlane(res->v[0]);
      rq.factor_cut = __builtin_amdgcn_readfirstlane(res->v[1]);
      rq.intron_start = __builtin_amdgcn_readfirstlane(res->v[2]);
      rq.intron_end = __builtin_amdgcn_readfirstlane(res->v[3]);
      rq.intron_start_on_align = __builtin_amdgcn_readfirstlane(res->v[4]);
      rq.intron_end_on_align = __builtin_amdgcn_readfirstlane(res->v[5]);
      rq.donor = donor; rq.acceptor = acceptor;
      rq.suffpref_length_on_est = sp_est; rq.suffpref_length_for_intron = sp_int; rq.suffpref_length_on_gen = sp_gen;
      rq.min_intron_length = q.min_intron_length;
      const int dim = (int)rq.dim;
      const uint8_t* const row_e = w + (uint32_t)__builtin_amdgcn_readfirstlane((int)res->str[0]);
      const uint8_t* const row_g = w + (uint32_t)__builtin_amdgcn_readfirstlane((int)res->str[1]);
      __syncthreads();
      for (int k = lane; k < dim; k += 64) { S.refine.rows[k] = row_e[k]; S.refine.rows[dim + k] = row_g[k]; }
      __syncthreads();
      pgpu_refine_result r;
      r.status = PGPU_OK; r.refined = 0; r.path = 0; r.pad = 0; r.donor = donor; r.acceptor = acceptor;
      refine_decide(S.refine, S.refine.rows, S.refine.rows + dim, dim, rq, T, n, ests, lane, r);
      __syncthreads();
      if (r.status != PGPU_OK) { cr.status = PGPU_ERANGE; break; }
      if (lane == 0) {
        out_exons[q.first_exon + i] = r.donor;
        out_steps[q.first_exon + i + 1] = (uint8_t)((uint32_t)r.path | ((uint32_t)r.refined << 7));
      }
      if (i == 0) second_est_start = r.acceptor.EST_start;
      donor = r.acceptor;
    }
    cr.done = i;
    if (lane == 0) out_exons[q.first_exon + i] = donor;
    if (cr.status == PGPU_OK && q.n_exons > 1 && first_est_start == second_est_start) cr.dropped_first = 1;
    if (lane == 0) out[c] = cr;
  }
}

thread_local double t_chain_ms = 0.0;

inline size_t up256(size_t x) { return (x + 255) & ~(size_t)255; }

struct CallBuffers {
  uint8_t* d = nullptr; hipEvent_t ev[2] = {nullptr, nullptr}; hipStream_t st; bool failed = false;
  explicit CallBuffers(hipStream_t s) : st(s) {}
  ~CallBuffers() {
    if (failed) (void)hipStreamSynchronize(st);
    for (auto& e : ev) if (e) (void)hipEventDestroy(e);
    (void)hipFree(d);
  }
};

bool coordinate_ok(int32_t v, size_t len) { return v >= -1 && (v < 0 || (size_t)v <= len); }

constexpr unsigned WAVES_PER_CU = 16;

}

#define TRY_HIP(call)                                                                        \
  do {                                                                                       \
    hipError_t e_ = (call);                                                                  \
    if (e_ != hipSuccess) { cb.failed = true;                                                \
      return pgpu_ctx_fail(ctx, e_ == hipErrorOutOfMemory ? PGPU_ENOMEM : PGPU_EDEVICE, hipGetErrorString(e_)); } \
  } while (0)

extern "C" double pgpu_index_refine_chains_kernel_ms(void) { return t_chain_ms; }

extern "C" int pgpu_index_refine_chains(pgpu_ctx* ctx, const pgpu_index* idx, const char* ests, size_t ests_len,
                                        const pgpu_factor* exons, size_t n_exons_total,
                                        const pgpu_chain_query* q, size_t n,
                                        pgpu_factor* out_exons, uint8_t* out_steps, pgpu_chain_result* out) {
  static_assert(sizeof(pgpu_chain_query) == 40 && sizeof(pgpu_chain_result) == 16 && sizeof(pgpu_factor) == 16, "ABI layout");
  if (!ctx || !idx || (n && (!q || !out)) || (ests_len && !ests) || (n_exons_total && (!exons || !out_exons || !out_steps)))
    return PGPU_EINVAL;
  if (n > 0x7fffffffull || n_exons_total > 0x7fffffffull)
    return pgpu_ctx_fail(ctx, PGPU_EINVAL, "more than 2^31 - 1 chains or exons in one call");
  const size_t glen = pgpu_index_length(idx);
  struct Freed { uint8_t* p; ~Freed() { free(p); } } named_block{ (uint8_t*)calloc(n_exons_total ? n_exons_total : 1, 1) };
  uint8_t* const named = named_block.p;
  if (!named) return pgpu_ctx_fail(ctx, PGPU_ENOMEM, "no memory for the table of the exons the chains name");
  for (size_t i = 0; i < n; ++i) {
    const pgpu_chain_query& x = q[i];
    bool ok = x.est_off <= ests_len && x.est_len <= ests_len - x.est_off && x.est_len <= 0x7fffffffu && x.reserved == 0 &&
              x.n_exons != 0 && x.first_exon <= n_exons_total && x.n_exons <= n_exons_total - x.first_exon;
    for (int32_t v : { x.suffpref_length_on_est, x.suffpref_length_for_intron, x.suffpref_length_on_gen })
      ok = ok && v >= 0 && v <= (1 << 24);
    for (uint32_t k = 0; ok && k < x.n_exons; ++k) {
      const pgpu_factor& f = exons[x.first_exon + k];
      ok = !named[x.first_exon + k] && coordinate_ok(f.EST_start, x.est_len) && coordinate_ok(f.EST_end, x.est_len) &&
           coordinate_ok(f.GEN_start, glen) && coordinate_ok(f.GEN_end, glen);
      named[x.first_exon + k] = 1;
      if (ok && k + 1 < x.n_exons) {
        const pgpu_factor& g = exons[x.first_exon + k + 1];
        ok = f.EST_end < g.EST_start && f.GEN_end < g.GEN_start;
      }
    }
    if (!ok)
      return pgpu_ctx_fail(ctx, PGPU_EINVAL, "bad chain query (a range past its buffer, reserved != 0, no exon, an exon two chains "
                                             "share, a donor that is not in front of its acceptor, or a coordinate outside what it "
                                             "indexes)");
  }
  t_chain_ms = 0.0;
  if (n == 0) {
    if (n_exons_total) { memcpy(out_exons, exons, n_exons_total * sizeof(pgpu_factor)); memset(out_steps, 0, n_exons_total); }
    return PGPU_OK;
  }
  if (pgpu_ctx_bind(ctx) != PGPU_OK) return PGPU_EDEVICE;
  hipStream_t st = pgpu_ctx_stream(ctx);
  CallBuffers cb(st);
  pgpu_range_push("refine chains");
  struct PopAtExit { ~PopAtExit() { pgpu_range_pop(); } } pop_at_exit;
  int dev = 0, cus = 0;
  TRY_HIP(hipGetDevice(&dev));
  TRY_HIP(hipDeviceGetAttribute(&cus, hipDeviceAttributeMultiprocessorCount, dev));
  const size_t waves = n < (size_t)cus * WAVES_PER_CU ? n : (size_t)cus * WAVES_PER_CU;
  const size_t ex_bytes = n_exons_total * sizeof(pgpu_factor);
  const size_t o_ex = up256(ests_len + 64), o_q = o_ex + up256(ex_bytes), o_oex = o_q + up256(n * sizeof(pgpu_chain_query)),
               o_st = o_oex + up256(ex_bytes), o_r = o_st + up256(n_exons_total), o_ws = o_r + up256(n * sizeof(pgpu_chain_result)),
               total = o_ws + waves * WS_WAVE;
  TRY_HIP(hipMalloc((void**)&cb.d, total));
  if (pgpu_ctx_timing(ctx)) for (auto& e : cb.ev) TRY_HIP(hipEventCreate(&e));
  if (ests_len) TRY_HIP(hipMemcpyAsync(cb.d, ests, ests_len, hipMemcpyHostToDevice, st));
  TRY_HIP(hipMemcpyAsync(cb.d + o_ex, exons, ex_bytes, hipMemcpyHostToDevice, st));
  TRY_HIP(hipMemcpyAsync(cb.d + o_q, q, n * sizeof(pgpu_chain_query), hipMemcpyHostToDevice, st));
  TRY_HIP(hipMemcpyAsync(cb.d + o_oex, cb.d + o_ex, ex_bytes, hipMemcpyDeviceToDevice, st));
  TRY_HIP(hipMemsetAsync(cb.d + o_st, 0, n_exons_total, st));
  if (cb.ev[0]) TRY_HIP(hipEventRecord(cb.ev[0], st));
  hipLaunchKernelGGL(chain_kernel, dim3((unsigned)waves), dim3(64), 0, st, pgpu_index_genomic(idx), (uint32_t)glen, cb.d,
                     (const pgpu_factor*)(cb.d + o_ex), (const pgpu_chain_query*)(cb.d + o_q), (uint32_t)n, cb.d + o_ws,
                     (pgpu_factor*)(cb.d + o_oex), cb.d + o_st, (pgpu_chain_result*)(cb.d + o_r));
  if (cb.ev[1]) TRY_HIP(hipEventRecord(cb.ev[1], st));
  TRY_HIP(hipMemcpyAsync(out_exons, cb.d + o_oex, ex_bytes, hipMemcpyDeviceToHost, st));
  TRY_HIP(hipMemcpyAsync(out_steps, cb.d + o_st, n_exons_total, hipMemcpyDeviceToHost, st));
  TRY_HIP(hipMemcpyAsync(out, cb.d + o_r, n * sizeof(pgpu_chain_result), hipMemcpyDeviceToHost, st));
  TRY_HIP(pgpu_ctx_wait(ctx));
  TRY_HIP(hipGetLastError());
  if (cb.ev[0]) { float ms = 0.f; (void)hipEventElapsedTime(&ms, cb.ev[0], cb.ev[1]); t_chain_ms = ms; }
  return PGPU_OK;
}
```

pintron_amd/csrc/pgpu_internal.h:

```cpp
#pragma once

#include <hip/hip_runtime.h>
#include <stdint.h>

#include "../../include/pintron_gpu.h"
#include "pgpu_index.h"

struct DevJob {
  const uint8_t* a;
  const uint8_t* b;
  uint32_t la, lb;
  uint32_t p0, p1, p2, tail;
  uint64_t ws_off;
  uint64_t str_off;
  uint32_t out_idx;
  uint32_t r_class;
};
static_assert(sizeof(DevJob) == 64, "DevJob layout");

using DevResult = pgpu_dp_result;

enum KernelFamily {
  KF_ALIGN = 0, KF_GAP, KF_ED, KF_KBAND, KF_LCF, KF_BORDERS, KF_AFFIX,
  KF_LCFSA,
  KF_LCFW,
  KF_ALIGNB,
  KF_COUNT
};

constexpr uint32_t ROW_CLASS_STRIPS = 128;
constexpr int32_t ALIGN_BAND_RETRY = 1;
constexpr uint32_t ALIGN_BAND_HALF = 31u;

constexpr int MAX_WAVE_SEGS = 10;
struct WaveSegs { int n; int start[MAX_WAVE_SEGS]; int count[MAX_WAVE_SEGS]; int family[MAX_WAVE_SEGS]; };
struct BatchDesc { WaveSegs segs; int wave_blocks; int bc_start, bc_count, ac_start, ac_count, lc_start, lc_count; LcfIndexView ix; };
constexpr size_t DP_BATCH_MAX_LDS = 64 * 1024;
size_t dp_batch_lds_bytes(bool wave_jobs, int bc_count, uint32_t bc_max_rows, int ac_count, int lc_count);
bool launch_dp_batch(const DevJob* jobs, const BatchDesc& d, uint32_t bc_max_rows, DevResult* res, uint8_t* ws, uint8_t* strs,
                     hipStream_t st);
void launch_align_fallback(const DevJob* jobs, int njobs, DevResult* res, uint8_t* ws, uint8_t* strs, hipStream_t st);

struct DpLaunch {
  const DevJob* jobs; int njobs;
  uint32_t max_rows;
  uint32_t max_chunks, max_l2;
  DevResult* res; uint8_t* ws; uint8_t* strs;
  unsigned long long* keys;
  hipStream_t st;
};
using DpLauncher = void (*)(const DpLaunch&);
void launch_align_big(const DpLaunch& l);
void launch_ed_big(const DpLaunch& l);
void launch_kband_big(const DpLaunch& l);
void launch_gap_big(const DpLaunch& l);
void launch_gap_slow(const DpLaunch& l);
void launch_borders_coop(const DpLaunch& l);
void launch_borders_slow(const DpLaunch& l);
void launch_affix_strips(const DpLaunch& l);
void launch_lcf(const DpLaunch& l);

__host__ __device__ inline size_t strip_bnd_bytes(uint32_t nc) { return (((size_t)nc + 1) * 4 + 15) & ~(size_t)15; }
static inline uint32_t align_entry_bytes(uint32_t R) { return R == ROW_CLASS_STRIPS ? 16u : (R <= 4 ? 1u : R / 4); }
static inline uint32_t align_coop_entry_bytes(uint32_t r_class) { const uint32_t R = r_class <= 4 ? 1u : r_class / 4; return R <= 4 ? 1u : R / 4; }
static inline uint32_t gap_entry_bytes(uint32_t R) { return R; }
```

pintron_amd/host/ef_fact.c:

```c
#include <math.h>
#include <stdlib.h>
#include <string.h>

#include "estfact.h"

typedef struct { int p, t, l; } ptl;

static size_t view_len(const char* s, int index, int length) {
  if (length <= 0) return 0;
  const char* z = (const char*)memchr(s + index, 0, (size_t)length);
  return z ? (size_t)(z - (s + index)) : (size_t)length;
}

char* ef_real_substring(int index, int length, const char* s) {
  if (index < 0) { length += index; index = 0; }
  if (length < 0) length = 0;
  char* r = (char*)malloc((size_t)length + 1);
  strncpy(r, s + index, (size_t)length);
  r[length] = '\0';
  return r;
}

static ef_factor* factor_new(int es, int ee, int gs, int ge) {
  ef_factor* f = (ef_factor*)malloc(sizeof(ef_factor));
// ... 782 lines not shown
  for (size_t v = 0; v < nx; ++v) if (slot[v] >= 0 && rs[slot[v]].v[2] != 0) idx[n++] = (int)v + 1;
  fact = keep_best_run(fact, idx, n);
  if (!efl_empty(fact)) {
    ef_phase(EFP_NOISY);
    n = 0;
    int index = 1;
    size_t v = 0;
    it = efl_begin(fact);
    while (efi_has_next(&it)) {
      const ef_factor* x = (const ef_factor*)efi_next(&it);
      while (v < nx && xs[v] != x) ++v;
      const bool ok = v < nx && slot[v] >= 0 && rs[slot[v]].v[0] != 0;
      if (!ok) idx[n++] = index;
      ++index;
    }
    fact = keep_best_run(fact, idx, n);
  }
  if (!small) { free(xs); free(slot); free(idx); free(rq); free(rs); }
  return fact;
}

static ef_list* clean_candidates(ef_list* cands, ef_list* flist, unsigned est_len, const char* GEN, const char* EST,
                                 const ef_config* cfg, ef_backend* be) {
  ef_iter ci = efl_begin(cands);
  while (efi_has_next(&ci)) {
    ef_list* f = (ef_list*)efi_next(&ci);
    bool ok = not_source_sink(f, (int)est_len);
    if (ok) ok = exon_start_end_ok(f);
    if (ok) { ef_phase(EFP_ENDPOINTS); f = handle_endpoints(f, GEN, EST, cfg, be); if (efl_empty(f)) ok = false; }
    if (ok) { ef_phase(EFP_EXTERNAL); f = ef_clean_external_exons(f, GEN, EST, be); if (efl_empty(f)) ok = false; }
    if (ok) { ef_phase(EFP_DUST); f = clean_complexity_and_noise(f, GEN, EST, cfg, be); if (efl_empty(f)) ok = false; }
    ef_phase(EFP_ADD);
    if (ok) ok = est_coverage_ok(f, EST);
    if (ok) {
      bool added;
      flist = ef_add_if_not_exists(f, flist, cfg, &added);
      if (!added) ef_factorization_free(f);
    } else {
      ef_factorization_free(f);
    }
  }
  efl_free(cands, NULL);
  return flist;
}

static bool chain_embedding(const void* rec, const ef_config* cfg, const char* GEN, ef_work* wk, emb** out) {
  const uint32_t* head = (const uint32_t*)rec;
  const uint32_t nv = head[0];
  if (nv < 2 || nv > 64) return false;
  const int32_t* vt = (const int32_t*)((const char*)rec + 16);
  const uint16_t* first = (const uint16_t*)((const char*)rec + 16 + 12 * (size_t)nv);
  const uint8_t* tgt = (const uint8_t*)rec + 16 + 12 * (size_t)nv + 2 * ((size_t)nv + 1);
  if (vt[0] != EF_SOURCE_START) return false;
  uint8_t path[64];
  uint64_t seen = 0;
  uint32_t k = 0, n = 0;
  for (;;) {
    if (seen >> k & 1u) return false;
    seen |= 1ull << k; path[n++] = (uint8_t)k;
    const uint32_t deg = (uint32_t)first[k + 1] - first[k];
    if (deg == 0) break;
    if (deg != 1) return false;
    k = tgt[first[k]];
    if (k >= nv) return false;
  }
  if (n != nv || vt[3 * (size_t)path[n - 1]] != EF_SINK_START) return false;
  wk->used += nv;
  ef_pairing node;
  memset(&node, 0, sizeof node);
  emb* e = emb_new(1);
  { const int32_t* s3 = vt + 3 * (size_t)path[n - 1]; e->e[0].p = s3[0]; e->e[0].t = s3[1]; e->e[0].l = s3[2]; }
  for (uint32_t q = n - 1; q-- > 0 && e;) {
    const int32_t* v3 = vt + 3 * (size_t)path[q];
    node.p = v3[0]; node.t = v3[1]; node.l = v3[2];
    emb* nx = update_embedding(e, &node, GEN, cfg);
    embedding_free(e);
    e = nx;
    if (e) ++wk->used;
  }
  *out = e;
  return true;
}

ef_est* ef_get_est_factorizations(const ef_seq* est_info, ef_meg* V, const ef_config* cfg,
                                  const ef_seq* gen_info, ef_backend* be) {
  ef_phase(EFP_EMBED);
  ef_est* est = (ef_est*)calloc(1, sizeof(ef_est));
  est->info = est_info;
  const char* GEN = gen_info->seq;
  const char* EST = est_info->seq;
  const unsigned est_len = (unsigned)V->n - 2;
  ef_list* flist = efl_new();
  ef_work wk = { 0, work_limit(cfg) };
  emb* chain = NULL;
  if (V->rec && !V->v && ef_chain_fast_path && chain_embedding(V->rec, cfg, GEN, &wk, &chain)) {
    if (ef_prof_on) ++ef_prof.chain_graphs;
    if (wk.used > wk.limit) {
      if (chain) embedding_free(chain);
      efl_free(flist, ef_factorization_free);
      free(est);
      return NULL;
    }
    if (chain) {
      ef_list* embs = efl_new();
      efl_push_back(embs, chain);
      ef_list* cands = factorizations_from_embeddings(embs, cfg);
      efl_free(embs, embedding_free);
      flist = clean_candidates(cands, flist, est_len, GEN, EST, cfg, be);
    }
  } else {
  if (ef_prof_on) ++ef_prof.other_graphs;
  V = ef_meg_lists(V);
  EF_MEG_FOR_POS(V, i, 0, V->n) {
    ef_iter it = efl_begin(V->v[i]);
    while (efi_has_next(&it)) { ef_pairing* p = (ef_pairing*)efi_next(&it); p->visited = false; p->emb_memo = NULL; }
  }
  EF_MEG_FOR_POS(V, i, 0, V->n) {
    ef_iter it = efl_begin(V->v[i]);
    while (efi_has_next(&it)) {
      ef_pairing* root = (ef_pairing*)efi_next(&it);
      if (root->visited) continue;
      ef_phase(EFP_EMBED);
      ef_list* embs = subtree_embeddings(root, cfg, GEN, &wk);
      if (!embs) {
        EF_MEG_FOR_POS(V, j, 0, V->n) {
          ef_iter jt = efl_begin(V->v[j]);
          while (efi_has_next(&jt)) { ef_pairing* q = (ef_pairing*)efi_next(&jt); if (q->emb_memo) { efl_free(q->emb_memo, embedding_free); q->emb_memo = NULL; } }
        }
        efl_free(flist, ef_factorization_free);
        free(est);
        return NULL;
      }
      flist = clean_candidates(factorizations_from_embeddings(embs, cfg), flist, est_len, GEN, EST, cfg, be);
    }
  }
  EF_MEG_FOR_POS(V, i, 0, V->n) {
    ef_iter it = efl_begin(V->v[i]);
    while (efi_has_next(&it)) { ef_pairing* p = (ef_pairing*)efi_next(&it); if (p->emb_memo) { efl_free(p->emb_memo, embedding_free); p->emb_memo = NULL; } }
  }
  }
  {
    unsigned long long hw = __atomic_load_n(&work_high_water, __ATOMIC_RELAXED);
    while (wk.used > hw && !__atomic_compare_exchange_n(&work_high_water, &hw, wk.used, true, __ATOMIC_RELAXED, __ATOMIC_RELAXED)) { }
  }

  ef_phase(EFP_FILTERS);
  {
    const size_t nf = efl_size(flist);
    double cov_small[32];
    double* cov = nf < 32 ? cov_small : (double*)malloc((nf + 1) * sizeof(double));
    double max_cov = 0.0;
    size_t k = 0;
    ef_iter it = efl_begin(flist);
    while (efi_has_next(&it)) {
      ef_list* f = (ef_list*)efi_next(&it);
      bool src_sink = false;
      if (efl_size(f) == 1) {
        const ef_factor* h = (const ef_factor*)efl_head(f);
        if (h->EST_start < 0 || h->EST_start >= (int)est_len) { cov[k] = -1.0; src_sink = true; }
      }
      if (!src_sink) { cov[k] = coverage_of(f, est_len); if (max_cov < cov[k]) max_cov = cov[k]; }
      ++k;
    }
    k = 0;
    it = efl_begin(flist);
    const int slen = (int)strlen(EST);
    while (efi_has_next(&it)) {
      efi_next(&it);
      const double c = cov[k++];
      if (c == -1.0 || max_cov - c > cfg->max_coverage_diff) efi_remove(&it, ef_factorization_free);
      else if ((max_cov - c) * slen > 100) efi_remove(&it, ef_factorization_free);
    }
    if (cov != cov_small) free(cov);
  }
  {
    const size_t nf = efl_size(flist);
    int gl_small[32];
    int* gl = nf < 32 ? gl_small : (int*)malloc((nf + 1) * sizeof(int));
    int min_gl = -1;
    size_t k = 0;
    ef_iter it = efl_begin(flist);
    while (efi_has_next(&it)) {
      gl[k] = gap_length_of((ef_list*)efi_next(&it));
      if (min_gl == -1 || min_gl > gl[k]) min_gl = gl[k];
      ++k;
    }
    k = 0;
    it = efl_begin(flist);
    while (efi_has_next(&it)) {
      efi_next(&it);
      const int g = gl[k++];
      if (cfg->max_gapLength_diff != -1 && g - min_gl > cfg->max_gapLength_diff) efi_remove(&it, ef_factorization_free);
    }
    if (gl != gl_small) free(gl);
  }
  ef_phase(EFP_GAPERR);
  if (be->ahead) {
    ef_ahead_collect(be, true);
    ef_iter it = efl_begin(flist);
    while (efi_has_next(&it)) check_gap_errors((ef_list*)efi_next(&it), EST, GEN, cfg, be);
    ef_ahead_collect(be, false);
    if (ef_ahead_flush(be) != 0) { fprintf(stderr, "* FATAL dynamic-programming backend failed\n"); abort(); }
  }
  {
    ef_iter it = efl_begin(flist);
    while (efi_has_next(&it)) {
      ef_list* f = (ef_list*)efi_next(&it);
      if (!check_gap_errors(f, EST, GEN, cfg, be)) efi_remove(&it, ef_factorization_free);
    }
  }
  if (cfg->max_number_of_factorizations != 0 && (int)efl_size(flist) > cfg->max_number_of_factorizations) {
    efl_free(flist, ef_factorization_free);
    flist = efl_new();
  }
  ef_phase(EFP_INTRON);
  {
    enum { GAP_AHEAD_MAX = 24 };
    ef_gap_ahead* pre = NULL; size_t n_pre = 0;
    if (be->ahead && be->dp_many) {
      size_t total = 0;
      ef_iter it = efl_begin(flist);
      while (efi_has_next(&it)) { const size_t k = efl_size((ef_list*)efi_next(&it)); total += k ? k - 1 : 0; }
      if (total >= 2 && total <= GAP_AHEAD_MAX) {
        pre = (ef_gap_ahead*)malloc(total * sizeof(ef_gap_ahead));
        ef_dp_req rq[GAP_AHEAD_MAX]; ef_dp_res rs[GAP_AHEAD_MAX];
        it = efl_begin(flist);
        while (efi_has_next(&it)) {
          ef_list* f = (ef_list*)efi_next(&it);
          if (efl_empty(f)) continue;
          ef_iter fi = efl_begin(f);
          const ef_factor* donor = (const ef_factor*)efi_next(&fi);
          while (efi_has_next(&fi)) {
            const ef_factor* acc = (const ef_factor*)efi_next(&fi);
            ef_gap_window_build(cfg, gen_info, est_info, donor, acc, &pre[n_pre].w);
            pre[n_pre].donor = *donor; pre[n_pre].acceptor = *acc;
            const ef_dp_req q = { EF_DP_GAP, pre[n_pre].w.seq_est, pre[n_pre].w.le, pre[n_pre].w.seq_gen, pre[n_pre].w.lg, 0, 0, 0, 0, 1 };
            rq[n_pre++] = q;
            donor = acc;
          }
        }
        memset(rs, 0, n_pre * sizeof(ef_dp_res));
        if (be->dp_many(be->self, rq, rs, n_pre) != 0) { fprintf(stderr, "* FATAL gap alignment backend failed\n"); abort(); }
        for (size_t k = 0; k < n_pre; ++k) pre[k].res = rs[k];
        if (ef_prof_on) ef_prof.ahead_asked += n_pre;
      }
    }
    size_t at = 0;
    ef_iter it = efl_begin(flist);
    while (efi_has_next(&it)) {
      ef_list* f = (ef_list*)efi_next(&it);
      if (efl_empty(f)) continue;
      ef_iter fi = efl_begin(f);
      ef_factor* donor = (ef_factor*)efi_next(&fi);
      bool first = true;
      while (efi_has_next(&fi)) {
        ef_factor* acc = (ef_factor*)efi_next(&fi);
        ef_refine_intron(cfg, gen_info, est_info, donor, acc, first, be, pre && at < n_pre ? &pre[at] : NULL);
        ++at;
        first = false;
        donor = acc;
      }
      fi = efl_begin(f);
      const ef_factor* e1 = (const ef_factor*)efi_next(&fi);
      if (efi_has_next(&fi)) {
        const ef_factor* e2 = (const ef_factor*)efi_next(&fi);
        if (e1->EST_start == e2->EST_start) free(efl_pop_front(f));
      }
    }
    for (size_t k = 0; k < n_pre; ++k) { ef_gap_window_release(&pre[k].w); ef_dp_res_release(&pre[k].res); }
    free(pre);
  }
  ef_phase(EFP_TAIL);
  est->polyA_signals = efl_new();
  est->polyadenil_signals = efl_new();
  {
    ef_iter it = efl_begin(flist);
    while (efi_has_next(&it)) {
      ef_list* f = (ef_list*)efi_next(&it);
      correct_tail(f, GEN, est_info->original_seq);
      bool polyadenil = false;
      const bool polyA = detect_polyA(f, GEN, est_info->original_seq, &polyadenil);
      efl_push_back(est->polyA_signals, polyA ? (void*)1 : (void*)2);
      efl_push_back(est->polyadenil_signals, polyadenil ? (void*)1 : (void*)2);
    }
  }
  est->factorizations = flist;
  return est;
}
```

pintron_amd/host/ef_gpu.h:

```cpp
#ifndef EF_GPU_H
#define EF_GPU_H

#include "estfact.h"
#include "../../include/pintron_gpu.h"

typedef struct {
  pgpu_dp_job* jobs; size_t n, cap;
  char* arena; size_t arena_len, arena_cap;
} ef_jobbuf;

void ef_jobbuf_init(ef_jobbuf* jb);
void ef_jobbuf_reset(ef_jobbuf* jb);
void ef_jobbuf_free(ef_jobbuf* jb);
size_t ef_jobbuf_add(ef_jobbuf* jb, const ef_dp_req* q, const char* gen, size_t gen_len);
int ef_decode_result(int kind, const pgpu_dp_result* r, const char* strings, ef_dp_res* out);
int ef_dp_trace_enabled(void);
void ef_dp_trace(const ef_dp_req* q, const ef_dp_res* r, uint32_t unit);
void ef_dp_trace_flush(void);
int ef_gpu_device_from_env(void);

ef_backend* ef_gpu_open(const ef_seq* gen);
void ef_gpu_close(ef_backend* be);

#endif
```

pintron_amd/host/ef_gpu_backend.c:

```c
#include <pthread.h>
#include <stdlib.h>
#include <string.h>

#include "estfact.h"
#include "ef_gpu.h"

static FILE* trace_file;
static pthread_mutex_t trace_mu = PTHREAD_MUTEX_INITIALIZER;
static pthread_once_t trace_once = PTHREAD_ONCE_INIT;
static void trace_open(void) {
  const char* path = getenv("PINTRON_DP_TRACE");
  if (path && path[0]) trace_file = fopen(path, "wb");
}
int ef_dp_trace_enabled(void) { pthread_once(&trace_once, trace_open); return trace_file != NULL; }
void ef_dp_trace(const ef_dp_req* q, const ef_dp_res* r, uint32_t unit) {
  if (!ef_dp_trace_enabled()) return;
  const uint32_t tail = q->tail > 2 ? 2 : q->tail;
  const uint32_t n0 = r->s0 ? (uint32_t)strlen(r->s0) : 0, n1 = r->s1 ? (uint32_t)strlen(r->s1) : 0;
  const uint32_t head[9] = { 0x31545044u, unit, (uint32_t)q->kind, (uint32_t)q->la, (uint32_t)q->lb, q->p0, q->p1, q->p2, q->tail };
  const uint32_t lens[2] = { n0, n1 };
  pthread_mutex_lock(&trace_mu);
  fwrite(head, 4, 9, trace_file); fwrite(r->v, 4, 6, trace_file); fwrite(lens, 4, 2, trace_file);
  fwrite(q->a, 1, q->la, trace_file); fwrite(q->b, 1, q->lb + tail, trace_file);
  if (n0) fwrite(r->s0, 1, n0, trace_file);
  if (n1) fwrite(r->s1, 1, n1, trace_file);
  pthread_mutex_unlock(&trace_mu);
}
void ef_dp_trace_flush(void) { if (trace_file) { pthread_mutex_lock(&trace_mu); fflush(trace_file); pthread_mutex_unlock(&trace_mu); } }

int ef_gpu_device_from_env(void) {
  const char* d = getenv("PINTRON_GPU_DEVICE");
  return d ? atoi(d) : 0;
}

void ef_jobbuf_init(ef_jobbuf* jb) { memset(jb, 0, sizeof(*jb)); }

void ef_jobbuf_reset(ef_jobbuf* jb) { jb->n = 0; jb->arena_len = 0; }

void ef_jobbuf_free(ef_jobbuf* jb) { free(jb->jobs); free(jb->arena); memset(jb, 0, sizeof(*jb)); }

static uint64_t put(ef_jobbuf* jb, const char* s, size_t n) {
  if (jb->arena_len + n + 8 > jb->arena_cap) {
    jb->arena_cap = (jb->arena_len + n + 8) * 2 + 4096;
    jb->arena = (char*)realloc(jb->arena, jb->arena_cap);
  }
  const uint64_t off = jb->arena_len;
  memcpy(jb->arena + off, s, n);
  jb->arena_len += n;
  return off;
}

size_t ef_jobbuf_add(ef_jobbuf* jb, const ef_dp_req* q, const char* gen, size_t gen_len) {
  if (jb->n == jb->cap) { jb->cap = jb->cap ? jb->cap * 2 : 256; jb->jobs = (pgpu_dp_job*)realloc(jb->jobs, jb->cap * sizeof(pgpu_dp_job)); }
  pgpu_dp_job* j = &jb->jobs[jb->n];
  memset(j, 0, sizeof(*j));
  j->kind = (uint32_t)q->kind;
  j->a_len = (uint32_t)q->la; j->b_len = (uint32_t)q->lb;
  j->p0 = q->p0; j->p1 = q->p1; j->p2 = q->p2; j->tail = q->tail;
  if (q->a >= gen && q->a + q->la <= gen + gen_len) { j->flags |= PGPU_JOB_A_GENOMIC; j->a_off = (uint64_t)(q->a - gen); }
  else j->a_off = put(jb, q->a, q->la);
  if (q->b >= gen && q->b + q->lb + q->tail <= gen + gen_len) { j->flags |= PGPU_JOB_B_GENOMIC; j->b_off = (uint64_t)(q->b - gen); }
  else j->b_off = put(jb, q->b, q->lb + (q->tail > 2 ? 2 : q->tail));
  return jb->n++;
}

int ef_decode_result(int kind, const pgpu_dp_result* r, const char* strings, ef_dp_res* out) {
  memset(out, 0, sizeof(*out));
  if (r->status != PGPU_OK) return r->status;
  for (int k = 0; k < 6; ++k) out->v[k] = r->v[k];
  if (kind == EF_DP_ALIGN || kind == EF_DP_GAP) {
    const char* row0 = strings + r->str[0]; const char* row1 = strings + r->str[1];
    const size_t n0 = strlen(row0), n1 = strlen(row1);
    char* blk = (char*)malloc(n0 + n1 + 2 * EF_ROW_PAD);
    memcpy(blk, row0, n0); memset(blk + n0, 0, EF_ROW_PAD);
    memcpy(blk + n0 + EF_ROW_PAD, row1, n1); memset(blk + n0 + EF_ROW_PAD + n1, 0, EF_ROW_PAD);
    out->s0 = blk; out->s1 = blk + n0 + EF_ROW_PAD;
  }
  return 0;
}

typedef struct {
  pgpu_ctx* ctx;
  pgpu_index* idx;
  const char* gen; size_t gen_len;
  ef_jobbuf jb;
  char* strings; size_t strings_cap;
} direct_be;

static int direct_pairings(void* self, const char* pattern, size_t m, unsigned L, double rate, ef_triple** out, size_t* n) {
  direct_be* d = (direct_be*)self;
  const uint64_t off[2] = { 0, m };
  pgpu_pairing_params prm = { L, 0, rate };
  size_t cap = 4096, cnt = 0;
  uint64_t first[2];
  pgpu_pairing* buf = (pgpu_pairing*)malloc(cap * sizeof(pgpu_pairing));
  int rc = pgpu_pairings(d->ctx, d->idx, pattern, off, 1, &prm, buf, cap, first, &cnt);
  if (rc == PGPU_ENOSPC) {
    cap = cnt; buf = (pgpu_pairing*)realloc(buf, cap * sizeof(pgpu_pairing));
    rc = pgpu_pairings(d->ctx, d->idx, pattern, off, 1, &prm, buf, cap, first, &cnt);
  }
  if (rc != PGPU_OK) { fprintf(stderr, "* FATAL pgpu_pairings: %s\n", pgpu_last_error(d->ctx)); free(buf); return -1; }
  *out = (ef_triple*)buf; *n = cnt;
  return 0;
}

static int direct_dp(void* self, const ef_dp_req* q, ef_dp_res* res) {
  direct_be* d = (direct_be*)self;
  ef_jobbuf_reset(&d->jb);
  ef_jobbuf_add(&d->jb, q, d->gen, d->gen_len);
  const size_t need = 2 * (q->la + q->lb + 1) + 16;
  if (need > d->strings_cap) { d->strings_cap = need * 2; d->strings = (char*)realloc(d->strings, d->strings_cap); }
  pgpu_dp_result r;
  size_t used = 0;
  const int rc = pgpu_dp_batch(d->ctx, d->idx, d->jb.jobs, 1, d->jb.arena, d->jb.arena_len, &r, d->strings, d->strings_cap, &used);
  if (rc != PGPU_OK) { fprintf(stderr, "* FATAL pgpu_dp_batch: %s\n", pgpu_last_error(d->ctx)); return -1; }
  if (r.status != PGPU_OK) { fprintf(stderr, "* FATAL DP job of kind %d and size %zu x %zu exceeds the device limits\n", q->kind, q->la, q->lb); return -1; }
  const int drc = ef_decode_result(q->kind, &r, d->strings, res);
  if (drc == 0) ef_dp_trace(q, res, 0);
  return drc;
}

static int direct_dp_many(void* self, const ef_dp_req* reqs, ef_dp_res* res, size_t n) {
  direct_be* d = (direct_be*)self;
  if (n == 0) return 0;
  ef_jobbuf_reset(&d->jb);
  size_t need = 16;
  for (size_t k = 0; k < n; ++k) { ef_jobbuf_add(&d->jb, &reqs[k], d->gen, d->gen_len); need += 2 * (reqs[k].la + reqs[k].lb + 1); }
  if (need > d->strings_cap) { d->strings_cap = need * 2; d->strings = (char*)realloc(d->strings, d->strings_cap); }
  pgpu_dp_result* r = (pgpu_dp_result*)malloc(n * sizeof(pgpu_dp_result));
  size_t used = 0;
  int rc = pgpu_dp_batch(d->ctx, d->idx, d->jb.jobs, n, d->jb.arena, d->jb.arena_len, r, d->strings, d->strings_cap, &used);
  if (rc != PGPU_OK) fprintf(stderr, "* FATAL pgpu_dp_batch: %s\n", pgpu_last_error(d->ctx));
  for (size_t k = 0; k < n && rc == PGPU_OK; ++k) {
    if (r[k].status != PGPU_OK) { fprintf(stderr, "* FATAL DP job of kind %d and size %zu x %zu exceeds the device limits\n", reqs[k].kind, reqs[k].la, reqs[k].lb); rc = -1; }
    else { rc = ef_decode_result(reqs[k].kind, &r[k], d->strings, &res[k]); if (rc == PGPU_OK) ef_dp_trace(&reqs[k], &res[k], 0); }
  }
  free(r);
  return rc == PGPU_OK ? 0 : -1;
}

ef_backend* ef_gpu_open(const ef_seq* gen) {
  direct_be* d = (direct_be*)calloc(1, sizeof(direct_be));
  if (pgpu_init(ef_gpu_device_from_env(), &d->ctx) != PGPU_OK) { free(d); return NULL; }
  d->gen = gen->seq; d->gen_len = strlen(gen->seq);
  if (pgpu_index_build(d->ctx, d->gen, d->gen_len, &d->idx) != PGPU_OK) {
    fprintf(stderr, "* FATAL pgpu_index_build: %s\n", pgpu_last_error(d->ctx));
    pgpu_destroy(d->ctx); free(d);
    return NULL;
  }
  ef_jobbuf_init(&d->jb);
  ef_backend* be = (ef_backend*)calloc(1, sizeof(ef_backend));
  be->self = d; be->pairings = direct_pairings; be->dp = direct_dp; be->dp_many = direct_dp_many;
  return be;
}

void ef_gpu_close(ef_backend* be) {
  if (!be) return;
  direct_be* d = (direct_be*)be->self;
  pgpu_index_destroy(d->ctx, d->idx);
  pgpu_destroy(d->ctx);
  ef_jobbuf_free(&d->jb);
  free(d->strings); free(d); free(be);
}
```

pintron_amd/host/ef_sched.c:

```c
#define _GNU_SOURCE
#include <malloc.h>
#include <pthread.h>
#include <sys/uio.h>
#include <errno.h>
#include <sys/prctl.h>
#include <sys/syscall.h>
#include <linux/futex.h>
#include <sys/resource.h>
#include <sched.h>
#include <dirent.h>
#include <time.h>
#include <stdlib.h>
#include <string.h>
#include <stdint.h>
#include <ucontext.h>
#include <sys/mman.h>

#if defined(__x86_64__) && !defined(EF_USE_UCONTEXT)
typedef struct { void* sp; } ef_ctx;
void ef_ctx_switch(void** save_sp, void* new_sp);
void ef_ctx_entry(void);
__asm__(
  ".text\n"
  ".globl ef_ctx_switch\n.type ef_ctx_switch,@function\n"
// ... 312 lines not shown
    ef_phase(EFP_OUTPUT);
    if (aligned) {
      ef_write_multifasta_output(in->gen, fe, &fs[0], in->cfg.retain_externals);
      ef_write_factorization_records(in->gen, fe, &fs[6], in->cfg.retain_externals, (uint32_t)f->unit);
      ef_write_single_est_info(&fs[1], fe->info);
    }
    ef_phase(EFP_FREE);
    ef_est_free(fe);
    ef_phase(EFP_OTHER);
    if (aligned) break;
  }
  ef_phase(EFP_OUTPUT);
  for (int k = 0; k < EF_N_OUT; ++k) {
    u->len[k] = fs[k].len;
    u->buf[k] = fs[k].len ? out_alloc(f->w, fs[k].len) : NULL;
    if (fs[k].len) memcpy(u->buf[k], fs[k].mem, fs[k].len);
  }
  f->state = F_DONE;
  if (EF_TSAN) tsan_to(f->w->tsan_sched);
  ctx_switch(&f->ctx, &f->w->sched);
}

static inline bool unit_ready(const shared* sh, size_t u) {
  if (!sh->n_pre) return true;
  const size_t last = sh->units[u].first + (sh->units[u].has_sibling ? 1 : 0);
  return last < __atomic_load_n(&sh->ready_entries, __ATOMIC_ACQUIRE);
}
static void wait_unit_ready(shared* sh, size_t u) {
  const size_t last = sh->units[u].first + (sh->units[u].has_sibling ? 1 : 0);
  const int was = ef_phase(EFP_WAIT_PREFETCH);
  pthread_mutex_lock(&sh->mu);
  while (last >= sh->ready_entries && !sh->failed) pthread_cond_wait(&sh->ready_cv, &sh->mu);
  pthread_mutex_unlock(&sh->mu);
  ef_phase(was);
}
static inline bool worker_has_work(const worker* w) {
  for (int k = 0; k < w->sh->n_lanes; ++k) if (w->lanes[k].n_fibers > 0 || w->lanes[k].posted) return true;
  return false;
}

enum { START_NONE = 0, START_OK = 1, START_LATER = 2 };
static int start_fiber(worker* w, int li) {
  shared* sh = w->sh;
  lane* ln = &w->lanes[li];
  fiber* f = w->free_fibers;
  size_t u;
  if (w->holding) u = w->held_unit;
  else {
    u = __atomic_fetch_add(&sh->next_unit, 1, __ATOMIC_RELAXED);
    if (u >= sh->n_units) return START_NONE;
  }
  if (!unit_ready(sh, u)) {
    if (worker_has_work(w)) { w->held_unit = u; w->holding = true; return START_LATER; }
    wait_unit_ready(sh, u);
  }
  w->holding = false;
  if (__atomic_load_n(&sh->failed, __ATOMIC_RELAXED)) return START_NONE;
  if (f) w->free_fibers = f->pool_next;
  else if (__atomic_load_n(&sh->fiber_pool, __ATOMIC_RELAXED)) {
    pthread_mutex_lock(&sh->mu);
    if (sh->fiber_pool) {
      f = sh->fiber_pool;
      fiber* last = f;
      for (int k = 0; k < 32 && last->pool_next; ++k) last = last->pool_next;
      sh->fiber_pool = last->pool_next;
      last->pool_next = NULL;
      w->free_fibers = f->pool_next; f->pool_next = NULL;
    }
    pthread_mutex_unlock(&sh->mu);
  }
  if (f) {
    char* st = f->stack;
    const bool gd = f->guarded;
    void* ts = f->tsan;
    ef_sink keep[EF_N_OUT];
    memcpy(keep, f->out, sizeof keep);
    memset(f, 0, sizeof(fiber));
    f->stack = st; f->guarded = gd; f->tsan = ts;
    memcpy(f->out, keep, sizeof keep);
  }
  else { f = (fiber*)calloc(1, sizeof(fiber)); f->stack = stack_alloc(sh->stack_size, &f->guarded); }
  f->w = w; f->unit = u; f->state = F_RUNNABLE; f->lane = li;
  f->be.self = f; f->be.pairings = fiber_pairings; f->be.dp = fiber_dp; f->be.dp_many = fiber_dp_many; f->be.meg = fiber_meg;
  memcpy(f->stack, FIBER_SENTINEL, sizeof FIBER_SENTINEL);
#if EF_TSAN
  if (f->tsan) __tsan_destroy_fiber(f->tsan);
  f->tsan = __tsan_create_fiber(0);
  w->tsan_sched = __tsan_get_current_fiber();
#endif
  ctx_make(&f->ctx, f->stack, sh->stack_size, fiber_main, f);
  ln->fibers[ln->n_fibers++] = f;
  return START_OK;
}

static int submit_pairings(worker* w, lane* ln) {
  fiber** wait = (fiber**)malloc((ln->n_fibers + 1) * sizeof(fiber*));
  size_t nw = 0;
  for (size_t i = 0; i < ln->n_fibers; ++i) if (ln->fibers[i]->state == F_WAIT_PAIR) wait[nw++] = ln->fibers[i];
  int rc = 0;
  while (nw > 0 && rc == 0) {
    const unsigned L = wait[0]->pat_L; const double rate = wait[0]->pat_rate;
    size_t ng = 0, total = 0;
    for (size_t i = 0; i < nw; ++i) if (wait[i]->pat_L == L && wait[i]->pat_rate == rate) { ++ng; total += wait[i]->pat_len; }
    char* blob = (char*)malloc(total + 1);
    uint64_t* off = (uint64_t*)malloc((ng + 1) * sizeof(uint64_t));
    fiber** grp = (fiber**)malloc(ng * sizeof(fiber*));
    size_t g = 0, pos = 0, rest = 0;
    for (size_t i = 0; i < nw; ++i) {
      fiber* f = wait[i];
      if (f->pat_L == L && f->pat_rate == rate) { off[g] = pos; memcpy(blob + pos, f->pat, f->pat_len); pos += f->pat_len; grp[g++] = f; }
      else wait[rest++] = f;
    }
    off[ng] = pos;
    pgpu_pairing_plan* plan = NULL;
    pgpu_pairing_params prm = { L, 0, rate };
    if (!w->ctx && pgpu_init(ef_gpu_device_from_env(), &w->ctx) != PGPU_OK) { free(blob); free(off); free(grp); free(wait); return 1; }
    rc = pgpu_pairing_plan_create(w->ctx, w->sh->idx, blob, off, ng, &plan);
    if (rc == PGPU_OK) rc = pgpu_pairing_plan_run(w->ctx, plan, &prm);
    if (rc == PGPU_OK) {
      const size_t cnt = (size_t)pgpu_pairing_plan_count(plan);
      pgpu_pairing* out = (pgpu_pairing*)malloc((cnt + 1) * sizeof(pgpu_pairing));
      uint64_t* first = (uint64_t*)malloc((ng + 1) * sizeof(uint64_t));
      rc = pgpu_pairing_plan_fetch(w->ctx, plan, out, cnt, first);
      if (rc == PGPU_OK) {
        for (size_t i = 0; i < ng; ++i) {
          const size_t n = (size_t)(first[i + 1] - first[i]);
          ef_triple* t = (ef_triple*)malloc((n + 1) * sizeof(ef_triple));
          memcpy(t, out + first[i], n * sizeof(ef_triple));
          *grp[i]->pat_out = t; *grp[i]->pat_n = n;
          grp[i]->rc = 0; grp[i]->state = F_RUNNABLE;
        }
        w->stats.pairing_batches++; w->stats.pairing_requests += ng;
      }
      free(out); free(first);
    }
    if (plan) pgpu_pairing_plan_destroy(w->ctx, plan);
    if (rc != PGPU_OK) fprintf(stderr, "* FATAL pairing batch failed: %s\n", pgpu_last_error(w->ctx));
    free(blob); free(off); free(grp);
    nw = rest;
  }
  free(wait);
  return rc;
}

static void kstat_add(ef_sched_stats* st, const ef_kernel_stat* k);

static void* service_main(void* arg) {
  pthread_setname_np(pthread_self(), "ef-gpu-service");
  prctl(PR_SET_TIMERSLACK, 1000UL, 0, 0, 0);
  service_thread* me = (service_thread*)arg;
  service* sv = me->sv;
  shared* sh = sv->sh;
  pgpu_dp_part* parts = NULL; size_t parts_cap = 0;
  for (;;) {
    pthread_mutex_lock(&sv->mu);
    const double t_idle = now_s();
    while (!sv->head && !sv->stop) pthread_cond_wait(&sv->posted, &sv->mu);
    me->phase_s[0] += now_s() - t_idle;
    if (sv->coalesce_us > 0 && sv->head && !sv->stop) {
      pthread_mutex_unlock(&sv->mu);
      struct timespec ts = { 0, sv->coalesce_us * 1000L };
      nanosleep(&ts, NULL);
      pthread_mutex_lock(&sv->mu);
    }
    dp_request* list = sv->head;
    sv->head = sv->tail = NULL;
// ... 1239 lines not shown
```

pintron_amd/host/estfact.h:

```cpp
#ifndef ESTFACT_H
#define ESTFACT_H

#include <limits.h>
#include <stdbool.h>
#include <stddef.h>
#include <stdint.h>
#include <stdio.h>
#include <string.h>

#include "ef_list.h"

typedef struct {
  unsigned min_factor_len;
  int min_intron_length, max_intron_length;
  double min_string_depth_rate;
  double max_prefix_discarded_rate, max_suffix_discarded_rate;
  int max_prefix_discarded, max_suffix_discarded;
  unsigned max_site_difference;
  int max_number_of_factorizations;
  double max_coverage_diff;
  int max_exonNUM_diff, max_gapLength_diff;
  char retain_externals;
  unsigned max_pairings_in_MEG;
  double max_freq_shortest_pairing;
// ... 109 lines not shown
void ef_transitive_reduction(ef_meg* V);
void ef_compact_short_edges(ef_meg* V, const ef_config* cfg);
bool ef_is_too_complex_for_compaction(ef_meg* V);
bool ef_is_too_complex(ef_meg* V, const ef_config* cfg);
void ef_meg_stats(ef_meg* V, size_t* pairings, size_t* edges);
struct ef_sink;
void ef_meg_write(struct ef_sink* f, ef_meg* V);
void ef_intronic_edges_write(struct ef_sink* f, ef_meg* V);

typedef struct ef_sink { FILE* f; char* mem; size_t len, cap; } ef_sink;
static inline void ef_sink_write(ef_sink* s, const char* p, size_t n) {
  if (s->f) { fwrite(p, 1, n, s->f); return; }
  if (s->len + n > s->cap) { s->cap = (s->len + n) * 2 + 256; s->mem = (char*)realloc(s->mem, s->cap); }
  memcpy(s->mem + s->len, p, n); s->len += n;
}
static inline void ef_sink_puts(ef_sink* s, const char* str) { ef_sink_write(s, str, strlen(str)); }

typedef struct { ef_sink* s; char* p; char* end; char b[4096]; } ef_wbuf;
static inline void efw_room(ef_wbuf* w, size_t need);
static inline void efw_open(ef_wbuf* w, ef_sink* s) {
  w->s = s;
  if (s->f) { w->p = w->b; w->end = w->b + sizeof w->b; }
  else { w->p = w->end = NULL; efw_room(w, 128); }
}
static inline void efw_flush(ef_wbuf* w) {
  if (w->s->f) { if (w->p != w->b) { fwrite(w->b, 1, (size_t)(w->p - w->b), w->s->f); w->p = w->b; } }
  else if (w->p) w->s->len = (size_t)(w->p - w->s->mem);
}
static inline void efw_room(ef_wbuf* w, size_t need) {
  if (w->p && (size_t)(w->end - w->p) >= need) return;
  ef_sink* s = w->s;
  if (s->f) { efw_flush(w); return; }
  if (w->p) s->len = (size_t)(w->p - s->mem);
  if (s->len + need > s->cap) { s->cap = (s->len + need) * 2 + 256; s->mem = (char*)realloc(s->mem, s->cap); }
  w->p = s->mem + s->len; w->end = s->mem + s->cap;
}
static inline void efw_ch(ef_wbuf* w, char c) { efw_room(w, 1); *w->p++ = c; }
static inline void efw_mem(ef_wbuf* w, const char* s, size_t n) {
  if (w->s->f && n > 2048) { efw_flush(w); fwrite(s, 1, n, w->s->f); return; }
  efw_room(w, n);
  memcpy(w->p, s, n); w->p += n;
}
static inline void efw_str(ef_wbuf* w, const char* s) { efw_mem(w, s, strlen(s)); }
static inline void efw_strn(ef_wbuf* w, const char* s, int prec) {
  if (prec <= 0) return;
  const char* z = (const char*)memchr(s, 0, (size_t)prec);
  efw_mem(w, s, z ? (size_t)(z - s) : (size_t)prec);
}
static inline void efw_int(ef_wbuf* w, long long v) {
  char t[24]; int k = 0;
  unsigned long long u = v < 0 ? 0ull - (unsigned long long)v : (unsigned long long)v;
  do { t[k++] = (char)('0' + u % 10); u /= 10; } while (u);
  efw_room(w, 24);
  if (v < 0) *w->p++ = '-';
  while (k) *w->p++ = t[--k];
}

enum { EFP_OTHER = 0, EFP_MEG, EFP_EMBED, EFP_ENDPOINTS, EFP_EXTERNAL, EFP_DUST, EFP_NOISY, EFP_ADD, EFP_FILTERS,
       EFP_GAPERR, EFP_INTRON, EFP_TAIL, EFP_FACTREF, EFP_OUTPUT, EFP_SIDE, EFP_FREE, EFP_SCHED, EFP_SLEEP,
       EFP_REF_AFFIX, EFP_REF_FALSE_SMALL, EFP_REF_NEW_SMALL, EFP_REF_CLEAN, EFP_SCHED_LAUNCH, EFP_SCHED_COLLECT, EFP_SCHED_START, EFP_WAIT_PREFETCH,
       EFP_NS_PREFIX, EFP_NS_BETWEEN_ASK, EFP_NS_BETWEEN_CLASS, EFP_NS_BETWEEN_SEARCH, EFP_TMP1, EFP_TMP2, EFP_TMP3, EFP_N };
extern int ef_prof_on;
typedef struct { unsigned long long cyc[EFP_N], susp[EFP_N], jobs[EFP_N]; unsigned long long last; int dummy; int* cur;
                 unsigned long long ahead_hits, ahead_misses, ahead_asked, chain_graphs, other_graphs; } ef_prof_state;
extern _Thread_local ef_prof_state ef_prof;
static inline unsigned long long ef_prof_now(void) {
#if defined(__x86_64__)
  unsigned lo, hi; __asm__ volatile("rdtsc" : "=a"(lo), "=d"(hi)); return ((unsigned long long)hi << 32) | lo;
#else
  return 0;
#endif
}
static inline int ef_phase(int id) {
  if (!ef_prof_on) return 0;
  ef_prof_state* p = &ef_prof;
  int* cur = p->cur ? p->cur : &p->dummy;
  const unsigned long long t = ef_prof_now();
  const int was = *cur;
  p->cyc[was] += t - p->last; p->last = t; *cur = id;
  return was;
}

enum { EF_DP_ALIGN = 0, EF_DP_GAP = 1, EF_DP_ED = 2, EF_DP_KBAND = 3, EF_DP_LCF = 4,
       EF_DP_BORDERS = 5, EF_DP_AFFIX = 6 };
typedef struct {
  int kind;
  const char* a; size_t la;
  const char* b; size_t lb;
  uint32_t p0, p1, p2, tail;
  uint32_t temp;
} ef_dp_req;
typedef struct {
  int32_t v[6];
  char* s0; char* s1;
} ef_dp_res;
#define EF_ROW_PAD 64
static inline void ef_dp_res_rows(ef_dp_res* r, size_t cap) {
  r->s0 = (char*)calloc(2 * (cap + EF_ROW_PAD), 1);
  r->s1 = r->s0 + cap + EF_ROW_PAD;
}
static inline void ef_dp_res_release(ef_dp_res* r) { free(r->s0); r->s0 = r->s1 = NULL; }

#define EF_AHEAD_MAX 96
#define EF_DP_PENDING 1
#define EF_AHEAD_SLOTS 256
typedef struct {
  int n, n_pending;
  bool collecting;
  unsigned char slot[EF_AHEAD_SLOTS];
  ef_dp_req q[EF_AHEAD_MAX]; int32_t v[EF_AHEAD_MAX][6];
} ef_ahead;
static inline void ef_ahead_init(ef_ahead* ah) { ah->n = ah->n_pending = 0; ah->collecting = false; memset(ah->slot, 0, sizeof ah->slot); }

typedef struct ef_backend {
  void* self;
  int (*pairings)(void* self, const char* pattern, size_t m, unsigned min_factor_len, double rate,
                  ef_triple** out, size_t* n);
  int (*dp)(void* self, const ef_dp_req* req, ef_dp_res* res);
  int (*dp_many)(void* self, const ef_dp_req* reqs, ef_dp_res* res, size_t n);
  const void* (*meg)(void* self, const char* pattern, size_t m, const ef_config* cfg);
  ef_ahead* ahead;
} ef_backend;

static inline bool ef_req_same(const ef_dp_req* x, const ef_dp_req* y) {
  return x->kind == y->kind && x->a == y->a && x->b == y->b && x->la == y->la && x->lb == y->lb &&
         x->p0 == y->p0 && x->p1 == y->p1 && x->p2 == y->p2 && x->tail == y->tail;
}
static inline bool ef_req_keepable(const ef_dp_req* q) { return q->temp == 0 && q->kind != EF_DP_ALIGN && q->kind != EF_DP_GAP; }
static inline unsigned ef_req_hash(const ef_dp_req* q) {
  uint64_t h = (uint64_t)(uintptr_t)q->a * 0x9E3779B97F4A7C15ull ^ (uint64_t)(uintptr_t)q->b * 0xC2B2AE3D27D4EB4Full;
  h ^= ((uint64_t)q->la << 32 | (uint64_t)q->lb) * 0x165667B19E3779F9ull + (uint64_t)q->kind;
  return (unsigned)(h >> 40) & (EF_AHEAD_SLOTS - 1);
}
static inline const int32_t* ef_ahead_find(const ef_ahead* ah, const ef_dp_req* q) {
  if (ah->n == 0 || !ef_req_keepable(q)) return NULL;
  for (unsigned s = ef_req_hash(q); ah->slot[s]; s = (s + 1) & (EF_AHEAD_SLOTS - 1))
    if (ef_req_same(&ah->q[ah->slot[s] - 1], q)) return ah->v[ah->slot[s] - 1];
  return NULL;
}
static inline unsigned ef_req_hash(const ef_dp_req* q);
static inline void ef_ahead_put(ef_ahead* ah, const ef_dp_req* q, const int32_t* v) {
  if (ah->n_pending || ah->n >= EF_AHEAD_MAX || !ef_req_keepable(q) || ef_ahead_find(ah, q)) return;
  ah->q[ah->n] = *q; memcpy(ah->v[ah->n], v, 6 * sizeof(int32_t));
  unsigned s = ef_req_hash(q);
  while (ah->slot[s]) s = (s + 1) & (EF_AHEAD_SLOTS - 1);
  ah->slot[s] = (unsigned char)(++ah->n);
}
static inline void ef_ahead_keep_next(ef_ahead* ah, const int32_t* v) {
  memcpy(ah->v[ah->n], v, 6 * sizeof(int32_t));
  unsigned s = ef_req_hash(&ah->q[ah->n]);
  while (ah->slot[s]) s = (s + 1) & (EF_AHEAD_SLOTS - 1);
  ah->slot[s] = (unsigned char)(++ah->n);
}
static inline int ef_backend_ask(ef_backend* be, const ef_dp_req* reqs, ef_dp_res* res, size_t n) {
  if (be->dp_many) return be->dp_many(be->self, reqs, res, n);
  for (size_t k = 0; k < n; ++k) { const int rc = be->dp(be->self, &reqs[k], &res[k]); if (rc != 0) return rc; }
  return 0;
}
int ef_dp_many_ahead(ef_backend* be, const ef_dp_req* reqs, ef_dp_res* res, size_t n);
static inline int ef_dp_many(ef_backend* be, const ef_dp_req* reqs, ef_dp_res* res, size_t n) {
  if (n == 0) return 0;
  memset(res, 0, n * sizeof(ef_dp_res));
  if (be->ahead && (be->ahead->n || be->ahead->collecting)) return ef_dp_many_ahead(be, reqs, res, n);
  return ef_backend_ask(be, reqs, res, n);
}
static inline int ef_dp_one(ef_backend* be, const ef_dp_req* req, ef_dp_res* res) { return ef_dp_many(be, req, res, 1); }
static inline void ef_ahead_collect(ef_backend* be, bool on) { if (be->ahead) be->ahead->collecting = on; }
static inline bool ef_collecting(const ef_backend* be) { return be->ahead && be->ahead->collecting; }
int ef_ahead_flush(ef_backend* be);
extern int ef_ahead_on;

typedef struct { int EST_start, EST_end, GEN_start, GEN_end; } ef_factor;

typedef struct {
  const ef_seq* info;
  ef_list* factorizations;
  ef_list* polyA_signals;
  ef_list* polyadenil_signals;
} ef_est;

void ef_factorization_free(void* fact);
void ef_est_free(ef_est* e);

unsigned long long ef_work_high_water(void);
ef_est* ef_get_est_factorizations(const ef_seq* est, ef_meg* V, const ef_config* cfg,
                                  const ef_seq* gen, ef_backend* be);
void ef_refine_est_factorizations(const ef_seq* gen, ef_est* e, const ef_config* cfg, ef_backend* be);
void ef_remove_factorizations_with_very_small_exons(ef_list* facts);
void ef_remove_duplicated_factorizations(ef_list* facts);
typedef struct {
  char* seq_est; char* seq_gen; size_t le, lg;
  int dsl_est, dsl_gen, deleted_intron_dim;
  char buf_e[512], buf_g[512];
} ef_gap_window;
typedef struct { ef_gap_window w; ef_dp_res res; ef_factor donor, acceptor; } ef_gap_ahead;
void ef_gap_window_build(const ef_config* cfg, const ef_seq* gen, const ef_seq* est, const ef_factor* donor,
                         const ef_factor* acceptor, ef_gap_window* w);
void ef_gap_window_release(ef_gap_window* w);
bool ef_refine_intron(const ef_config* cfg, const ef_seq* gen, const ef_seq* est, ef_factor* donor,
                      ef_factor* acceptor, bool first_intron, ef_backend* be, ef_gap_ahead* ahead);
int ef_classify_intron(const ef_seq* gen, int start, int end);
int ef_burset_frequency(const char* donor, const char* acceptor);
int ef_burset_adaptor(const char* t, size_t cut1, size_t cut2);
int ef_check_burset_patterns(const char* gen, int donor_left_on_gen, int acceptor_right_on_gen);
// ... 40 lines not shown
```

Baseline: 880,600.

## Offload whole intron-refinement chains to a GPU chain DP job kind

Adds a CHAIN DP job kind that sends an EST together with its full exon chain to the device. A persistent chain kernel refines every intron of the chain in one job instead of the host issuing one DP request per intron pair. This is meant to cut host round trips and per-request launch and batching overhead in the intron refinement phase. It is on by default unless disabled by env var or tracing, and it adds arena alignment padding, new validation, and a host fallback for chains the device cannot finish.

```diff
diff --git a/include/pintron_gpu.h b/include/pintron_gpu.h
--- a/include/pintron_gpu.h
+++ b/include/pintron_gpu.h
@@ -191,8 +191,10 @@
   PGPU_DP_LCF = 4,
   PGPU_DP_BORDERS = 5,
   PGPU_DP_AFFIX = 6,
-  PGPU_DP_NKINDS = 7
+  PGPU_DP_CHAIN = 7,
+  PGPU_DP_NKINDS = 8
 };
+int pgpu_dp_has_kind(int kind);
 
 #define PGPU_JOB_A_GENOMIC 1u
 #define PGPU_JOB_B_GENOMIC 2u
diff --git a/pintron_amd/capi.py b/pintron_amd/capi.py
--- a/pintron_amd/capi.py
+++ b/pintron_amd/capi.py
@@ -6,8 +6,8 @@
 
 PGPU_OK, PGPU_EDEVICE, PGPU_ENOMEM, PGPU_EINVAL, PGPU_ENOSPC, PGPU_ERANGE, PGPU_ENOSYS = \
     0, -5, -12, -22, -28, -34, -38
-ALIGN, GAP, ED, KBAND, LCF, BORDERS, AFFIX = range(7)
-KIND_NAMES = ["ALIGN", "GAP", "ED", "KBAND", "LCF", "BORDERS", "AFFIX"]
+ALIGN, GAP, ED, KBAND, LCF, BORDERS, AFFIX, CHAIN = range(8)
+KIND_NAMES = ["ALIGN", "GAP", "ED", "KBAND", "LCF", "BORDERS", "AFFIX", "CHAIN"]
 JOB_A_GENOMIC, JOB_B_GENOMIC = 1, 2
 
 
@@ -129,7 +129,7 @@
     "pgpu_dp_plan_string_bytes", "pgpu_dp_plan_fetch", "pgpu_dp_plan_destroy",
     "pgpu_dp_plan_results_to_device",
     "pgpu_dp_plan_cells", "pgpu_dp_plan_algo_bytes", "pgpu_dp_plan_kernel_ms",
-    "pgpu_dp_plan_launches", "pgpu_dp_plan_n_groups", "pgpu_dp_plan_group_info", "pgpu_dp_batch",
+    "pgpu_dp_plan_launches", "pgpu_dp_plan_n_groups", "pgpu_dp_plan_group_info", "pgpu_dp_batch", "pgpu_dp_has_kind",
 ]
 
 _lib = None
@@ -222,6 +222,7 @@
             getattr(L, nm).restype = u64
         L.pgpu_dp_plan_kernel_ms.argtypes = [vp, C.c_int]
         L.pgpu_dp_plan_kernel_ms.restype = C.c_double
+        L.pgpu_dp_has_kind.argtypes = [C.c_int]
         L.pgpu_dp_plan_n_groups.argtypes = [vp]
         L.pgpu_dp_plan_group_info.argtypes = [vp, C.c_int, C.POINTER(GroupInfo)]
         L.pgpu_dp_batch.argtypes = [vp, vp, C.POINTER(DpJob), sz, C.c_char_p, sz,
@@ -511,6 +512,15 @@
                                len(b_tail) if tail is None else tail))
         return len(self.jobs) - 1
 
+    def add_chain(self, est: bytes, exons, suffpref_on_est=30, suffpref_for_intron=70, suffpref_on_gen=30, min_intron_length=60):
+        import numpy as np
+        a_off = self._put(est)
+        self._put(b"\0" * (-self.size % 4))
+        ex = np.asarray(exons, dtype="<i4").reshape(-1, 4)
+        block = np.array([suffpref_on_est, suffpref_for_intron, suffpref_on_gen, min_intron_length], dtype="<i4").tobytes() + ex.tobytes()
+        self.jobs.append(DpJob(CHAIN, 0, a_off, self._put(block), len(est), len(block), 0, 0, 0, 0))
+        return len(self.jobs) - 1
+
     def arrays(self):
         arr = (DpJob * max(len(self.jobs), 1))(*self.jobs)
         return arr, b"".join(self.chunks)
@@ -603,6 +613,16 @@
     raise ValueError(kind)
 
 
+def decode_chain(r: DpResult, strings: bytes):
+    import numpy as np
+    n = r.v[2]
+    off = r.str[0]
+    exons = np.frombuffer(strings, dtype="<i4", count=4 * n, offset=off).reshape(n, 4)
+    steps = np.frombuffer(strings, dtype=np.uint8, count=n, offset=off + 16 * n)
+    return dict(status=r.status, done=r.v[0], dropped_first=r.v[1], n_exons=n, exons=exons, steps=steps,
+                cells=(r.v[3] & 0xffffffff) | ((r.v[4] & 0xffffffff) << 32))
+
+
 def run_jobs(ctx: Context, joblist: JobList, index: Index = None):
     plan = Plan(ctx, joblist, index)
     try:
diff --git a/pintron_amd/csrc/pgpu_api.hip b/pintron_amd/csrc/pgpu_api.hip
--- a/pintron_amd/csrc/pgpu_api.hip
+++ b/pintron_amd/csrc/pgpu_api.hip
@@ -23,6 +23,7 @@
 
 struct pgpu_ctx {
   int device = 0;
+  int cus = 1;
   hipStream_t stream = nullptr;
   char err[512] = {0};
   BufPool pools[2];
@@ -159,6 +160,7 @@
 int pgpu_ctx_fail(pgpu_ctx* ctx, int code, const char* msg) { return set_err(ctx, code, "%s", msg); }
 
 extern "C" int pgpu_abi_version(void) { return 1; }
+extern "C" int pgpu_dp_has_kind(int kind) { return kind >= 0 && kind < PGPU_DP_NKINDS; }
 
 #include <dlfcn.h>
 namespace {
@@ -230,6 +232,7 @@
   pgpu_ctx* ctx = new (std::nothrow) pgpu_ctx();
   if (!ctx) return PGPU_ENOMEM;
   ctx->device = device;
+  ctx->cus = prop.multiProcessorCount > 0 ? prop.multiProcessorCount : 1;
   if (hipStreamCreateWithFlags(&ctx->stream, hipStreamNonBlocking) != hipSuccess) {
     delete ctx;
     return PGPU_EDEVICE;
@@ -275,7 +278,7 @@
 enum DpRoute : uint8_t {
   RT_ALIGN_STRIPS, RT_ALIGN_COOP, RT_ALIGN_WAVE, RT_GAP_SLOW, RT_GAP, RT_ED, RT_KBAND, RT_LCF,
   RT_BORDERS_SLOW, RT_BORDERS_COOP, RT_BORDERS_WAVE, RT_AFFIX_STRIPS, RT_AFFIX_COOP, RT_AFFIX_WAVE,
-  RT_LCFSA, RT_LCFW, RT_ALIGNB,
+  RT_LCFSA, RT_LCFW, RT_ALIGNB, RT_CHAIN,
   RT_BATCH,
   RT_COUNT
 };
@@ -334,6 +337,7 @@
   {"lcf_sa",                  PGPU_DP_LCF,     KF_LCFSA,   nullptr,         false, 0, bytes_lcfsa,    SEGMENT,      6,  0,     0, false,  0, nullptr,             false},
   {"lcf_small",               PGPU_DP_LCF,     KF_LCFW,    nullptr,         false, 1, bytes_operands, SEGMENT,      7,  0,     0, false,  0, nullptr,             false},
   {"align_band",              PGPU_DP_ALIGN,   KF_ALIGNB,  ws_align_coop,   true,  1, bytes_align,    SEGMENT,      0,  0,     0, false,  0, nullptr,             false},
+  {"chain_jobs",              PGPU_DP_CHAIN,   KF_CHAIN,   nullptr,         false, 0, bytes_operands, OUTSIDE,      0,  0, 15000, false,  0, launch_chain_jobs,   false},
   {"dp_batch",                PGPU_DP_ALIGN,   KF_COUNT,   nullptr,         false, 0, nullptr,        OUTSIDE,      0,  0, 20000, false, -1, nullptr,             false},
 };
 static_assert(sizeof ROUTES / sizeof ROUTES[0] == RT_COUNT, "one entry per route, in the enum's order");
@@ -396,6 +400,9 @@
   std::vector<uint32_t> lcf_out;
   size_t off_keys = 0;
   bool lcf_decoded = false;
+  std::vector<uint32_t> chain_out;
+  bool chain_counted = false;
+  const uint8_t* d_gen = nullptr; uint32_t gen_len = 0;
 };
 
 static void plan_free(pgpu_dp_plan* p) {
@@ -474,22 +481,46 @@
       k.R = row_class(la);
       k.route = k.R == 1 ? RT_AFFIX_WAVE : (k.R == ROW_CLASS_STRIPS ? RT_AFFIX_STRIPS : RT_AFFIX_COOP);
       return PGPU_OK;
+    case PGPU_DP_CHAIN:
+      k.R = 0; k.route = RT_CHAIN; k.size = (lb - 16u) / 16u;
+      return PGPU_OK;
     default: return PGPU_EINVAL;
   }
 }
 
+static bool chain_job_ok(const pgpu_dp_job& in, const char* arena, size_t arena_len, bool has_genomic, size_t gen_len) {
+  if (!has_genomic || in.flags != 0 || in.a_len > 0x7fffffffu) return false;
+  if (in.a_off > arena_len || in.a_len > arena_len - in.a_off || in.b_off > arena_len || in.b_len > arena_len - in.b_off) return false;
+  if (in.b_len < 32u || (in.b_len & 15u) != 0 || (in.b_off & 3u) != 0) return false;
+  int32_t head[4];
+  memcpy(head, arena + in.b_off, sizeof head);
+  for (int q = 0; q < 3; ++q) if (head[q] < 0 || head[q] > (1 << 24)) return false;
+  auto coordinate_ok = [](int32_t v, size_t len) { return v >= -1 && (v < 0 || (size_t)v <= len); };
+  const uint32_t n_exons = (in.b_len - 16u) / 16u;
+  pgpu_factor f{}, g{};
+  for (uint32_t q = 0; q < n_exons; ++q, f = g) {
+    memcpy(&g, arena + in.b_off + 16 + (size_t)q * sizeof g, sizeof g);
+    if (!coordinate_ok(g.EST_start, in.a_len) || !coordinate_ok(g.EST_end, in.a_len) || !coordinate_ok(g.GEN_start, gen_len) ||
+        !coordinate_ok(g.GEN_end, gen_len)) return false;
+    if (q && !(f.EST_end < g.EST_start && f.GEN_end < g.GEN_start)) return false;
+  }
+  return true;
+}
+
+static inline size_t arena_stride(size_t arena_len) { return (arena_len + 3) & ~(size_t)3; }
 static std::vector<Keyed> classify_jobs(const pgpu_dp_part* parts, size_t n_parts, size_t n_jobs, const LcfIndexView& lcf,
-                                        bool has_genomic, size_t gen_len, std::vector<pgpu_dp_result>& prefill) {
+                                        bool has_genomic, size_t gen_len, std::vector<pgpu_dp_result>& prefill, bool& bad_chain) {
   std::vector<Keyed> v;
   v.reserve(n_jobs);
   prefill.assign(n_jobs, pgpu_dp_result{});
   size_t i = 0, part_base = 0;
-  for (size_t q = 0; q < n_parts; part_base += parts[q].arena_len, ++q)
+  for (size_t q = 0; q < n_parts; part_base += arena_stride(parts[q].arena_len), ++q)
     for (size_t w = 0; w < parts[q].n_jobs; ++w, ++i) {
       const pgpu_dp_job& in = parts[q].jobs[w];
       const size_t own_arena = parts[q].arena_len;
       prefill[i].status = PGPU_EINVAL;
       if (in.kind >= PGPU_DP_NKINDS) continue;
+      if (in.kind == PGPU_DP_CHAIN && !chain_job_ok(in, parts[q].arena, own_arena, has_genomic, gen_len)) { bad_chain = true; continue; }
       const bool ag = in.flags & PGPU_JOB_A_GENOMIC, bg = in.flags & PGPU_JOB_B_GENOMIC;
       if ((ag || bg) && !has_genomic) continue;
       const size_t a_space = ag ? gen_len : own_arena, b_space = bg ? gen_len : own_arena;
@@ -527,15 +558,27 @@
 }
 
 struct DpSpace { size_t ws = 0, strs = 0; };
-static DpSpace assign_workspace(std::vector<Keyed>& v, std::vector<uint32_t>& lcf_out) {
+static DpSpace assign_workspace(std::vector<Keyed>& v, std::vector<uint32_t>& lcf_out, std::vector<uint32_t>& chain_out, int cus) {
   DpSpace sp;
   for (auto& k : v) {
     const RouteInfo& ri = ROUTES[k.route];
+    if (k.route == RT_CHAIN) {
+      const size_t n_exons = (k.j.lb - 16u) / 16u;
+      sp.strs = (sp.strs + 3) & ~(size_t)3;
+      k.j.str_off = sp.strs; sp.strs += n_exons * (sizeof(pgpu_factor) + 1);
+      chain_out.push_back(k.j.out_idx);
+      continue;
+    }
     const size_t wb = ri.ws_bytes ? ri.ws_bytes(k.j.la, k.j.lb, k.R) : 0;
     if (wb) { k.j.ws_off = sp.ws; sp.ws += wb; }
     if (ri.strings) { k.j.str_off = sp.strs; sp.strs += 2 * ((size_t)k.j.la + k.j.lb + 1); }
     if (ri.keyed) lcf_out.push_back(k.j.out_idx);
     sp.ws = (sp.ws + 15) & ~(size_t)15;
+  }
+  if (!chain_out.empty()) {
+    sp.ws = (sp.ws + 255) & ~(size_t)255;
+    for (auto& k : v) if (k.route == RT_CHAIN) k.j.ws_off = sp.ws;
+    sp.ws += chain_jobs_ws_bytes(chain_out.size(), cus);
   }
   return sp;
 }
@@ -648,7 +691,7 @@
 
   {
     size_t at = off_arena;
-    for (size_t q = 0; q < n_parts; ++q) { if (parts[q].arena_len) memcpy(p->h_up + at, parts[q].arena, parts[q].arena_len); at += parts[q].arena_len; }
+    for (size_t q = 0; q < n_parts; ++q) { if (parts[q].arena_len) memcpy(p->h_up + at, parts[q].arena, parts[q].arena_len); at += arena_stride(parts[q].arena_len); }
   }
   DevJob* hj = (DevJob*)(p->h_up + off_jobs);
   for (size_t q = 0; q < v.size(); ++q) {
@@ -674,7 +717,7 @@
   size_t n_jobs = 0, arena_len = 0;
   for (size_t q = 0; q < n_parts; ++q) {
     if ((parts[q].n_jobs && !parts[q].jobs) || (parts[q].arena_len && !parts[q].arena)) return set_err(ctx, PGPU_EINVAL, "bad argument");
-    n_jobs += parts[q].n_jobs; arena_len += parts[q].arena_len;
+    n_jobs += parts[q].n_jobs; arena_len += arena_stride(parts[q].arena_len);
   }
   if (n_jobs >= (size_t)1 << 30) return set_err(ctx, PGPU_EINVAL, "too many jobs");
   HIP_TRY(ctx, hipSetDevice(ctx->device));
@@ -685,9 +728,18 @@
   p->pooled = pgpu_ctx_pool_acquire(ctx, 0);
   p->batch.desc.ix = pgpu_index_lcf_view(idx);
 
-  std::vector<Keyed> v = classify_jobs(parts, n_parts, n_jobs, p->batch.desc.ix, idx != nullptr, idx ? pgpu_index_length(idx) : 0, p->prefill);
+  bool bad_chain = false;
+  std::vector<Keyed> v = classify_jobs(parts, n_parts, n_jobs, p->batch.desc.ix, idx != nullptr, idx ? pgpu_index_length(idx) : 0, p->prefill,
+                                       bad_chain);
+  if (bad_chain) {
+    plan_free(p);
+    return set_err(ctx, PGPU_EINVAL, "bad chain job (no index, an operand outside its arena or by PGPU_JOB_*_GENOMIC, b_len not 16 + 16 x "
+                                     "exons or b_off not a multiple of 4, a suffpref length outside [0, 2^24], a donor that is not in "
+                                     "front of its acceptor, or a coordinate outside what it indexes)");
+  }
+  if (idx) { p->d_gen = pgpu_index_genomic(idx); p->gen_len = (uint32_t)pgpu_index_length(idx); }
   sort_jobs(v);
-  const DpSpace sp = assign_workspace(v, p->lcf_out);
+  const DpSpace sp = assign_workspace(v, p->lcf_out, p->chain_out, ctx->cus);
   p->ws_bytes = sp.ws; p->strs_bytes = sp.strs; p->n_keys = p->lcf_out.size(); p->n_dev_jobs = v.size();
   std::vector<Slice> batched;
   form_groups(v, p->groups, batched, p->cells, p->algo_bytes);
@@ -703,6 +755,11 @@
   if (!ctx || !p) return set_err(ctx, PGPU_EINVAL, "bad argument");
   HIP_TRY(ctx, hipSetDevice(ctx->device));
   p->synced = false; p->lcf_decoded = false;
+  if (p->chain_counted) {
+    p->chain_counted = false;
+    p->cells[PGPU_DP_CHAIN] = 0;
+    for (auto& g : p->groups) if (g.route == RT_CHAIN) g.own.cells = 0;
+  }
   std::vector<size_t> order;
   std::vector<size_t> key_of(p->groups.size(), 0);
   auto weight = [&](size_t gi) -> long {
@@ -741,7 +798,7 @@
     } else {
       if (!ri.launch) return set_err(ctx, PGPU_EDEVICE, "no kernel for %zu jobs of %s outside the batch launch", g.own.count, ri.name);
       ri.launch(DpLaunch{p->d_jobs + g.own.first, (int)g.own.count, g.max_rows, g.max_chunks, g.max_l2, p->d_results, p->d_ws,
-                         p->d_strs, p->d_keys + key_of[gi], st});
+                         p->d_strs, p->d_keys + key_of[gi], st, p->d_gen, p->gen_len, p->d_arena, ctx->cus});
     }
     if (g.ev1) HIP_TRY(ctx, hipEventRecord(g.ev1, st));
     if (g.route == RT_BATCH) launch_align_fallback(p->d_jobs + p->batch.ab_start, p->batch.ab_count, p->d_results, p->d_ws, p->d_strs, st);
@@ -773,12 +830,23 @@
   }
 }
 
+static void count_chain_cells(pgpu_dp_plan* p) {
+  if (p->chain_counted || p->chain_out.empty()) return;
+  p->chain_counted = true;
+  const DevResult* res = (const DevResult*)(p->h_down + (p->off_results - p->off_keys));
+  uint64_t cells = 0;
+  for (uint32_t i : p->chain_out) cells += (uint64_t)(uint32_t)res[i].v[3] | ((uint64_t)(uint32_t)res[i].v[4] << 32);
+  p->cells[PGPU_DP_CHAIN] += cells;
+  for (auto& g : p->groups) if (g.route == RT_CHAIN) g.own.cells += cells;
+}
+
 extern "C" int pgpu_dp_plan_sync(pgpu_ctx* ctx, pgpu_dp_plan* p) {
   if (!ctx || !p) return set_err(ctx, PGPU_EINVAL, "bad argument");
   if (wait_stream(ctx, ctx->stream) != 0) return set_err(ctx, PGPU_EDEVICE, "waiting for the batch failed");
   p->synced = p->launched;
   if (p->launched) {
     decode_lcf_keys(p);
+    count_chain_cells(p);
     for (int k = 0; k < PGPU_DP_NKINDS; ++k) { p->ms[k] = 0; p->launches[k] = 0; }
     for (auto& g : p->groups) {
       float ms = 0.f;
@@ -802,6 +870,7 @@
   if (!p->synced && wait_stream(ctx, ctx->stream) != 0) return set_err(ctx, PGPU_EDEVICE, "result download failed");
   p->synced = true;
   decode_lcf_keys(p);
+  count_chain_cells(p);
   const size_t rb = p->n_jobs * sizeof(DevResult);
   if (rb) memcpy(results, p->h_down + (p->off_results - p->off_keys), rb);
   if (p->strs_bytes && strings) memcpy(strings, p->h_down + (p->down_bytes - p->strs_bytes), p->strs_bytes);
diff --git a/pintron_amd/csrc/pgpu_chain.hip b/pintron_amd/csrc/pgpu_chain.hip
--- a/pintron_amd/csrc/pgpu_chain.hip
+++ b/pintron_amd/csrc/pgpu_chain.hip
@@ -1,41 +1,9 @@
 #include <stdlib.h>
 #include <string.h>
 
-#include "pgpu_internal.h"
-#include "pgpu_wave_dp.h"
-#include "pgpu_refine_body.h"
+#include "pgpu_chain_body.h"
 
 namespace {
-
-constexpr int MAX_EW = PGPU_CHAIN_MAX_EST_WINDOW;
-constexpr int MAX_GW = PGPU_CHAIN_MAX_GEN_WINDOW;
-constexpr uint32_t CHAIN_R = 4;
-static_assert(MAX_EW <= 64 * (int)CHAIN_R && MAX_EW + MAX_GW <= MAX_DIM, "the caps fit the sweep and the decision");
-
-constexpr size_t WS_DIRS = ((size_t)MAX_GW + 64) * 64 * CHAIN_R;
-constexpr size_t WS_STRS = WS_DIRS;
-constexpr size_t WS_STRS_BYTES = (2 * ((size_t)MAX_EW + MAX_GW + 1) + 15) & ~(size_t)15;
-constexpr size_t WS_WIN_E = WS_STRS + WS_STRS_BYTES;
-constexpr size_t WS_WIN_G = WS_WIN_E + ((MAX_EW + 15) & ~15);
-constexpr size_t WS_RES = WS_WIN_G + ((MAX_GW + 15) & ~15);
-constexpr size_t WS_WAVE = (WS_RES + sizeof(DevResult) + 255) & ~(size_t)255;
-
-struct ChainLds {
-  union {
-    struct { __attribute__((aligned(16))) uint8_t win[TB_WIN_BYTES]; uint8_t path[TB_PATH]; } tb;
-    RefineLds refine;
-  };
-};
-
-__device__ __forceinline__ int append_piece(uint8_t* dst, int at, int cap, const Seq& s, int index, int length, int lane) {
-  if (at > cap) return at;
-  if (index < 0) { length += index; index = 0; }
-  if (length > cap - at + 1) length = cap - at + 1;
-  const Piece p = substring(s, index, length, lane);
-  if (p.len > cap - at) return cap + 1;
-  for (int k = lane; k < p.len; k += 64) dst[at + k] = s.p[p.start + k];
-  return at + p.len;
-}
 
 __global__ __launch_bounds__(64)
 void chain_kernel(const uint8_t* __restrict__ T, uint32_t n, const uint8_t* __restrict__ ests, const pgpu_factor* __restrict__ exons,
@@ -44,88 +12,44 @@
   __shared__ ChainLds S;
   const int lane = (int)threadIdx.x;
   uint8_t* const w = ws + (size_t)blockIdx.x * WS_WAVE;
-  uint8_t* const win_e = w + WS_WIN_E;
-  uint8_t* const win_g = w + WS_WIN_G;
-  DevResult* const res = reinterpret_cast<DevResult*>(w + WS_RES);
   for (uint32_t c = blockIdx.x; c < n_chains; c += gridDim.x) {
     const pgpu_chain_query q = queries[c];
-    Seq est, gen;
-    est.p = ests + q.est_off; est.len = (int)q.est_len;
-    gen.p = T; gen.len = (int)n;
-    const int sp_est = q.suffpref_length_on_est, sp_int = q.suffpref_length_for_intron, sp_gen = q.suffpref_length_on_gen;
-    pgpu_chain_result cr;
-    cr.status = PGPU_OK; cr.done = 0; cr.dropped_first = 0; cr.pad = 0;
-    pgpu_factor donor = exons[q.first_exon];
-    const int first_est_start = donor.EST_start;
-    int second_est_start = 0;
-    uint32_t i = 0;
-    for (; i + 1 < q.n_exons; ++i) {
-      const pgpu_factor acceptor = exons[q.first_exon + i + 1];
-      int dsl_gen = donor.GEN_start;
-      if (donor.GEN_end - sp_gen + 1 >= dsl_gen) dsl_gen = donor.GEN_end - sp_gen + 1;
-      int dsl_est = donor.EST_start;
-      if (donor.EST_end - sp_est + 1 >= dsl_est) dsl_est = donor.EST_end - sp_est + 1;
-      int apr_gen = acceptor.GEN_end;
-      if (acceptor.GEN_start + sp_gen - 1 <= apr_gen) apr_gen = acceptor.GEN_start + sp_gen - 1;
-      int apr_est = acceptor.EST_end;
-      if (acceptor.EST_start + sp_est - 1 <= apr_est) apr_est = acceptor.EST_start + sp_est - 1;
-      int le = 0, lg = 0;
-      le = append_piece(win_e, le, MAX_EW, est, dsl_est, donor.EST_end - dsl_est + 1, lane);
-      if (donor.EST_end != acceptor.EST_start - 1)
-        le = append_piece(win_e, le, MAX_EW, est, donor.EST_end + 1, acceptor.EST_start - donor.EST_end - 1, lane);
-      le = append_piece(win_e, le, MAX_EW, est, acceptor.EST_start, apr_est - acceptor.EST_start + 1, lane);
-      lg = append_piece(win_g, lg, MAX_GW, gen, dsl_gen, donor.GEN_end - dsl_gen + 1, lane);
-      lg = append_piece(win_g, lg, MAX_GW, gen, donor.GEN_end + 1, sp_int, lane);
-      lg = append_piece(win_g, lg, MAX_GW, gen, acceptor.GEN_start - sp_int, sp_int, lane);
-      lg = append_piece(win_g, lg, MAX_GW, gen, acceptor.GEN_start, apr_gen - acceptor.GEN_start + 1, lane);
-      if (le > MAX_EW || lg > MAX_GW) { cr.status = PGPU_ERANGE; break; }
-      DevJob job;
-      job.a = win_e; job.b = win_g; job.la = (uint32_t)le; job.lb = (uint32_t)lg;
-      job.p0 = job.p1 = job.p2 = job.tail = 0;
-      job.ws_off = 0; job.str_off = WS_STRS; job.out_idx = 0;
-      job.r_class = le <= 64 ? 1u : (le <= 128 ? 2u : 4u);
-      own_stores_visible();
-      switch (job.r_class) {
-        case 1:  gap_wave_body<1>(job, res, w, (uint32_t)lane); break;
-        case 2:  gap_wave_body<2>(job, res, w, (uint32_t)lane); break;
-        default: gap_wave_body<4>(job, res, w, (uint32_t)lane); break;
-      }
-      own_stores_visible();
-      gap_traceback_wave(job, res, w, w, (uint32_t)lane, S.tb.win, S.tb.path);
-      own_stores_visible();
-      pgpu_refine_query rq;
-      rq.est_off = q.est_off; rq.est_len = q.est_len; rq.flags = i == 0 ? PGPU_REFINE_FIRST_INTRON : 0u;
-      rq.rows_off = 0; rq.dim = (uint32_t)__builtin_amdgcn_readfirstlane(res->v[0]);
-      rq.factor_cut = __builtin_amdgcn_readfirstlane(res->v[1]);
-      rq.intron_start = __builtin_amdgcn_readfirstlane(res->v[2]);
-      rq.intron_end = __builtin_amdgcn_readfirstlane(res->v[3]);
-      rq.intron_start_on_align = __builtin_amdgcn_readfirstlane(res->v[4]);
-      rq.intron_end_on_align = __builtin_amdgcn_readfirstlane(res->v[5]);
-      rq.donor = donor; rq.acceptor = acceptor;
-      rq.suffpref_length_on_est = sp_est; rq.suffpref_length_for_intron = sp_int; rq.suffpref_length_on_gen = sp_gen;
-      rq.min_intron_length = q.min_intron_length;
-      const int dim = (int)rq.dim;
-      const uint8_t* const row_e = w + (uint32_t)__builtin_amdgcn_readfirstlane((int)res->str[0]);
-      const uint8_t* const row_g = w + (uint32_t)__builtin_amdgcn_readfirstlane((int)res->str[1]);
-      __syncthreads();
-      for (int k = lane; k < dim; k += 64) { S.refine.rows[k] = row_e[k]; S.refine.rows[dim + k] = row_g[k]; }
-      __syncthreads();
-      pgpu_refine_result r;
-      r.status = PGPU_OK; r.refined = 0; r.path = 0; r.pad = 0; r.donor = donor; r.acceptor = acceptor;
-      refine_decide(S.refine, S.refine.rows, S.refine.rows + dim, dim, rq, T, n, ests, lane, r);
-      __syncthreads();
-      if (r.status != PGPU_OK) { cr.status = PGPU_ERANGE; break; }
-      if (lane == 0) {
-        out_exons[q.first_exon + i] = r.donor;
-        out_steps[q.first_exon + i + 1] = (uint8_t)((uint32_t)r.path | ((uint32_t)r.refined << 7));
-      }
-      if (i == 0) second_est_start = r.acceptor.EST_start;
-      donor = r.acceptor;
+    uint64_t cells = 0;
+    const pgpu_chain_result cr = chain_body(T, n, ests, q.est_off, q.est_len, q.n_exons, q.suffpref_length_on_est,
+                                            q.suffpref_length_for_intron, q.suffpref_length_on_gen, q.min_intron_length,
+                                            exons + q.first_exon, out_exons + q.first_exon, out_steps + q.first_exon, w, S, lane, cells);
+    if (lane == 0) out[c] = cr;
+  }
+}
+
+__global__ __launch_bounds__(64, 4)
+void chain_jobs_kernel(const uint8_t* __restrict__ T, uint32_t n, const uint8_t* __restrict__ arena, const DevJob* __restrict__ jobs, uint32_t n_jobs,
+                       DevResult* __restrict__ results, uint8_t* __restrict__ ws, uint8_t* __restrict__ strs) {
+  __shared__ ChainLds S;
+  const int lane = (int)threadIdx.x;
+  for (uint32_t c = blockIdx.x; c < n_jobs; c += gridDim.x) {
+    const DevJob job = jobs[c];
+    uint8_t* const w = ws + job.ws_off + (size_t)blockIdx.x * WS_WAVE;
+    const uint64_t a_off = (uint64_t)(job.a - arena), b_off = (uint64_t)(job.b - arena);
+    const int32_t* const head = reinterpret_cast<const int32_t*>(arena + b_off);
+    const pgpu_factor* const ex_in = reinterpret_cast<const pgpu_factor*>(arena + b_off + 16);
+    const uint32_t n_exons = (job.lb - 16u) / 16u;
+    pgpu_factor* const ex_out = reinterpret_cast<pgpu_factor*>(strs + job.str_off);
+    uint8_t* const steps_out = strs + job.str_off + (size_t)n_exons * sizeof(pgpu_factor);
+    for (uint32_t k = (uint32_t)lane; k < n_exons; k += 64) { ex_out[k] = ex_in[k]; steps_out[k] = 0; }
+    own_stores_visible();
+    uint64_t cells = 0;
+    const pgpu_chain_result cr = chain_body(T, n, arena, a_off, job.la, n_exons, __builtin_amdgcn_readfirstlane(head[0]),
+                                            __builtin_amdgcn_readfirstlane(head[1]), __builtin_amdgcn_readfirstlane(head[2]),
+                                            __builtin_amdgcn_readfirstlane(head[3]), ex_in, ex_out, steps_out, w, S, lane, cells);
+    if (lane == 0) {
+      DevResult r;
+      r.status = cr.status;
+      r.v[0] = (int32_t)cr.done; r.v[1] = (int32_t)cr.dropped_first; r.v[2] = (int32_t)n_exons;
+      r.v[3] = (int32_t)(uint32_t)cells; r.v[4] = (int32_t)(uint32_t)(cells >> 32); r.v[5] = 0;
+      r.pad = 0; r.str[0] = job.str_off; r.str[1] = 0;
+      results[job.out_idx] = r;
     }
-    cr.done = i;
-    if (lane == 0) out_exons[q.first_exon + i] = donor;
-    if (cr.status == PGPU_OK && q.n_exons > 1 && first_est_start == second_est_start) cr.dropped_first = 1;
-    if (lane == 0) out[c] = cr;
   }
 }
 
@@ -145,8 +69,13 @@
 
 bool coordinate_ok(int32_t v, size_t len) { return v >= -1 && (v < 0 || (size_t)v <= len); }
 
-constexpr unsigned WAVES_PER_CU = 16;
+}
 
+size_t chain_jobs_ws_bytes(size_t njobs, int cus) { return chain_jobs_waves(njobs, cus) * WS_WAVE; }
+
+void launch_chain_jobs(const DpLaunch& l) {
+  hipLaunchKernelGGL(chain_jobs_kernel, dim3((unsigned)chain_jobs_waves((size_t)l.njobs, l.cus)), dim3(64), 0, l.st, l.genomic,
+                     l.genomic_len, l.arena, l.jobs, (uint32_t)l.njobs, l.res, l.ws, l.strs);
 }
 
 #define TRY_HIP(call)                                                                        \
@@ -205,7 +134,7 @@
   int dev = 0, cus = 0;
   TRY_HIP(hipGetDevice(&dev));
   TRY_HIP(hipDeviceGetAttribute(&cus, hipDeviceAttributeMultiprocessorCount, dev));
-  const size_t waves = n < (size_t)cus * WAVES_PER_CU ? n : (size_t)cus * WAVES_PER_CU;
+  const size_t waves = chain_jobs_waves(n, cus);
   const size_t ex_bytes = n_exons_total * sizeof(pgpu_factor);
   const size_t o_ex = up256(ests_len + 64), o_q = o_ex + up256(ex_bytes), o_oex = o_q + up256(n * sizeof(pgpu_chain_query)),
                o_st = o_oex + up256(ex_bytes), o_r = o_st + up256(n_exons_total), o_ws = o_r + up256(n * sizeof(pgpu_chain_result)),
diff --git a/pintron_amd/csrc/pgpu_chain_body.h b/pintron_amd/csrc/pgpu_chain_body.h
--- /dev/null
+++ b/pintron_amd/csrc/pgpu_chain_body.h
@@ -0,0 +1,127 @@
+#pragma once
+
+#include "pgpu_internal.h"
+#include "pgpu_wave_dp.h"
+#include "pgpu_refine_body.h"
+
+namespace {
+
+
+constexpr int MAX_EW = PGPU_CHAIN_MAX_EST_WINDOW;
+constexpr int MAX_GW = PGPU_CHAIN_MAX_GEN_WINDOW;
+constexpr uint32_t CHAIN_R = 4;
+static_assert(MAX_EW <= 64 * (int)CHAIN_R && MAX_EW + MAX_GW <= MAX_DIM, "the caps fit the sweep and the decision");
+
+constexpr size_t WS_DIRS = ((size_t)MAX_GW + 64) * 64 * CHAIN_R;
+constexpr size_t WS_STRS = WS_DIRS;
+constexpr size_t WS_STRS_BYTES = (2 * ((size_t)MAX_EW + MAX_GW + 1) + 15) & ~(size_t)15;
+constexpr size_t WS_WIN_E = WS_STRS + WS_STRS_BYTES;
+constexpr size_t WS_WIN_G = WS_WIN_E + ((MAX_EW + 15) & ~15);
+constexpr size_t WS_RES = WS_WIN_G + ((MAX_GW + 15) & ~15);
+constexpr size_t WS_WAVE = (WS_RES + sizeof(DevResult) + 255) & ~(size_t)255;
+
+struct ChainLds {
+  union {
+    struct { __attribute__((aligned(16))) uint8_t win[TB_WIN_BYTES]; uint8_t path[TB_PATH]; } tb;
+    RefineLds refine;
+  };
+};
+
+__device__ __forceinline__ int append_piece(uint8_t* dst, int at, int cap, const Seq& s, int index, int length, int lane) {
+  if (at > cap) return at;
+  if (index < 0) { length += index; index = 0; }
+  if (length > cap - at + 1) length = cap - at + 1;
+  const Piece p = substring(s, index, length, lane);
+  if (p.len > cap - at) return cap + 1;
+  for (int k = lane; k < p.len; k += 64) dst[at + k] = s.p[p.start + k];
+  return at + p.len;
+}
+
+__device__ __forceinline__ pgpu_chain_result chain_body(const uint8_t* __restrict__ T, uint32_t n, const uint8_t* __restrict__ ests,
+                                                        uint64_t est_off, uint32_t est_len, uint32_t n_exons, int sp_est, int sp_int,
+                                                        int sp_gen, int32_t min_intron_length, const pgpu_factor* __restrict__ ex_in,
+                                                        pgpu_factor* __restrict__ ex_out, uint8_t* __restrict__ steps_out,
+                                                        uint8_t* __restrict__ w, ChainLds& S, int lane, uint64_t& cells) {
+  uint8_t* const win_e = w + WS_WIN_E;
+  uint8_t* const win_g = w + WS_WIN_G;
+  DevResult* const res = reinterpret_cast<DevResult*>(w + WS_RES);
+  Seq est, gen;
+  est.p = ests + est_off; est.len = (int)est_len;
+  gen.p = T; gen.len = (int)n;
+  pgpu_chain_result cr;
+  cr.status = PGPU_OK; cr.done = 0; cr.dropped_first = 0; cr.pad = 0;
+  pgpu_factor donor = ex_in[0];
+  const int first_est_start = donor.EST_start;
+  int second_est_start = 0;
+  uint32_t i = 0;
+  for (; i + 1 < n_exons; ++i) {
+    const pgpu_factor acceptor = ex_in[i + 1];
+    int dsl_gen = donor.GEN_start;
+    if (donor.GEN_end - sp_gen + 1 >= dsl_gen) dsl_gen = donor.GEN_end - sp_gen + 1;
+    int dsl_est = donor.EST_start;
+    if (donor.EST_end - sp_est + 1 >= dsl_est) dsl_est = donor.EST_end - sp_est + 1;
+    int apr_gen = acceptor.GEN_end;
+    if (acceptor.GEN_start + sp_gen - 1 <= apr_gen) apr_gen = acceptor.GEN_start + sp_gen - 1;
+    int apr_est = acceptor.EST_end;
+    if (acceptor.EST_start + sp_est - 1 <= apr_est) apr_est = acceptor.EST_start + sp_est - 1;
+    int le = 0, lg = 0;
+    le = append_piece(win_e, le, MAX_EW, est, dsl_est, donor.EST_end - dsl_est + 1, lane);
+    if (donor.EST_end != acceptor.EST_start - 1)
+      le = append_piece(win_e, le, MAX_EW, est, donor.EST_end + 1, acceptor.EST_start - donor.EST_end - 1, lane);
+    le = append_piece(win_e, le, MAX_EW, est, acceptor.EST_start, apr_est - acceptor.EST_start + 1, lane);
+    lg = append_piece(win_g, lg, MAX_GW, gen, dsl_gen, donor.GEN_end - dsl_gen + 1, lane);
+    lg = append_piece(win_g, lg, MAX_GW, gen, donor.GEN_end + 1, sp_int, lane);
+    lg = append_piece(win_g, lg, MAX_GW, gen, acceptor.GEN_start - sp_int, sp_int, lane);
+    lg = append_piece(win_g, lg, MAX_GW, gen, acceptor.GEN_start, apr_gen - acceptor.GEN_start + 1, lane);
+    if (le > MAX_EW || lg > MAX_GW) { cr.status = PGPU_ERANGE; break; }
+    cells += 3ull * (uint32_t)le * (uint32_t)lg;
+    DevJob job;
+    job.a = win_e; job.b = win_g; job.la = (uint32_t)le; job.lb = (uint32_t)lg;
+    job.p0 = job.p1 = job.p2 = job.tail = 0;
+    job.ws_off = 0; job.str_off = WS_STRS; job.out_idx = 0;
+    job.r_class = le <= 64 ? 1u : (le <= 128 ? 2u : 4u);
+    own_stores_visible();
+    switch (job.r_class) {
+      case 1:  gap_wave_body<1>(job, res, w, (uint32_t)lane); break;
+      case 2:  gap_wave_body<2>(job, res, w, (uint32_t)lane); break;
+      default: gap_wave_body<4>(job, res, w, (uint32_t)lane); break;
+    }
+    own_stores_visible();
+    gap_traceback_wave(job, res, w, w, (uint32_t)lane, S.tb.win, S.tb.path);
+    own_stores_visible();
+    pgpu_refine_query rq;
+    rq.est_off = est_off; rq.est_len = est_len; rq.flags = i == 0 ? PGPU_REFINE_FIRST_INTRON : 0u;
+    rq.rows_off = 0; rq.dim = (uint32_t)__builtin_amdgcn_readfirstlane(res->v[0]);
+    rq.factor_cut = __builtin_amdgcn_readfirstlane(res->v[1]);
+    rq.intron_start = __builtin_amdgcn_readfirstlane(res->v[2]);
+    rq.intron_end = __builtin_amdgcn_readfirstlane(res->v[3]);
+    rq.intron_start_on_align = __builtin_amdgcn_readfirstlane(res->v[4]);
+    rq.intron_end_on_align = __builtin_amdgcn_readfirstlane(res->v[5]);
+    rq.donor = donor; rq.acceptor = acceptor;
+    rq.suffpref_length_on_est = sp_est; rq.suffpref_length_for_intron = sp_int; rq.suffpref_length_on_gen = sp_gen;
+    rq.min_intron_length = min_intron_length;
+    const int dim = (int)rq.dim;
+    const uint8_t* const row_e = w + (uint32_t)__builtin_amdgcn_readfirstlane((int)res->str[0]);
+    const uint8_t* const row_g = w + (uint32_t)__builtin_amdgcn_readfirstlane((int)res->str[1]);
+    __syncthreads();
+    for (int k = lane; k < dim; k += 64) { S.refine.rows[k] = row_e[k]; S.refine.rows[dim + k] = row_g[k]; }
+    __syncthreads();
+    pgpu_refine_result r;
+    r.status = PGPU_OK; r.refined = 0; r.path = 0; r.pad = 0; r.donor = donor; r.acceptor = acceptor;
+    refine_decide(S.refine, S.refine.rows, S.refine.rows + dim, dim, rq, T, n, ests, lane, r);
+    __syncthreads();
+    if (r.status != PGPU_OK) { cr.status = PGPU_ERANGE; break; }
+    if (lane == 0) {
+      ex_out[i] = r.donor;
+      steps_out[i + 1] = (uint8_t)((uint32_t)r.path | ((uint32_t)r.refined << 7));
+    }
+    if (i == 0) second_est_start = r.acceptor.EST_start;
+    donor = r.acceptor;
+  }
+  cr.done = i;
+  if (lane == 0) ex_out[i] = donor;
+  if (cr.status == PGPU_OK && n_exons > 1 && first_est_start == second_est_start) cr.dropped_first = 1;
+  return cr;
+}
+
+}
diff --git a/pintron_amd/csrc/pgpu_internal.h b/pintron_amd/csrc/pgpu_internal.h
--- a/pintron_amd/csrc/pgpu_internal.h
+++ b/pintron_amd/csrc/pgpu_internal.h
@@ -25,6 +25,7 @@
   KF_LCFSA,
   KF_LCFW,
   KF_ALIGNB,
+  KF_CHAIN,
   KF_COUNT
 };
 
@@ -48,6 +49,7 @@
   DevResult* res; uint8_t* ws; uint8_t* strs;
   unsigned long long* keys;
   hipStream_t st;
+  const uint8_t* genomic; uint32_t genomic_len; const uint8_t* arena; int cus;
 };
 using DpLauncher = void (*)(const DpLaunch&);
 void launch_align_big(const DpLaunch& l);
@@ -59,6 +61,9 @@
 void launch_borders_slow(const DpLaunch& l);
 void launch_affix_strips(const DpLaunch& l);
 void launch_lcf(const DpLaunch& l);
+void launch_chain_jobs(const DpLaunch& l);
+inline size_t chain_jobs_waves(size_t njobs, int cus) { const size_t cap = (size_t)(cus > 0 ? cus : 1) * 16; return njobs < cap ? njobs : cap; }
+size_t chain_jobs_ws_bytes(size_t njobs, int cus);
 
 __host__ __device__ inline size_t strip_bnd_bytes(uint32_t nc) { return (((size_t)nc + 1) * 4 + 15) & ~(size_t)15; }
 static inline uint32_t align_entry_bytes(uint32_t R) { return R == ROW_CLASS_STRIPS ? 16u : (R <= 4 ? 1u : R / 4); }
diff --git a/pintron_amd/host/ef_fact.c b/pintron_amd/host/ef_fact.c
--- a/pintron_amd/host/ef_fact.c
+++ b/pintron_amd/host/ef_fact.c
@@ -888,6 +888,62 @@
   return true;
 }
 
+static void refine_introns_by_chains(ef_list* flist, const ef_config* cfg, const ef_seq* gen_info, const ef_seq* est_info, ef_backend* be) {
+  size_t n_req = 0, n_ex = 0;
+  ef_iter it = efl_begin(flist);
+  while (efi_has_next(&it)) { const size_t k = efl_size((ef_list*)efi_next(&it)); if (k >= 2) { ++n_req; n_ex += k; } }
+  if (n_req == 0) return;
+  ef_dp_req* rq = (ef_dp_req*)calloc(n_req, sizeof(ef_dp_req));
+  ef_dp_res* rs = (ef_dp_res*)calloc(n_req, sizeof(ef_dp_res));
+  int32_t* blocks = (int32_t*)malloc((n_req + n_ex) * 4 * sizeof(int32_t));
+  const size_t est_len = strlen(est_info->seq);
+  size_t r = 0, at = 0;
+  it = efl_begin(flist);
+  while (efi_has_next(&it)) {
+    ef_list* f = (ef_list*)efi_next(&it);
+    const size_t k = efl_size(f);
+    if (k < 2) continue;
+    int32_t* b = blocks + at;
+    b[0] = cfg->suffpref_length_on_est; b[1] = cfg->suffpref_length_for_intron; b[2] = cfg->suffpref_length_on_gen; b[3] = cfg->min_intron_length;
+    size_t e = 0;
+    ef_iter fi = efl_begin(f);
+    while (efi_has_next(&fi)) memcpy(b + 4 + 4 * e++, efi_next(&fi), sizeof(ef_factor));
+    rq[r].kind = EF_DP_CHAIN; rq[r].a = est_info->seq; rq[r].la = est_len; rq[r].b = (const char*)b; rq[r].lb = 16 + 16 * k; rq[r].temp = 1;
+    ++r; at += 4 + 4 * k;
+  }
+  if (ef_backend_ask(be, rq, rs, n_req) != 0) { fprintf(stderr, "* FATAL intron refinement backend failed\n"); abort(); }
+  r = 0;
+  it = efl_begin(flist);
+  while (efi_has_next(&it)) {
+    ef_list* f = (ef_list*)efi_next(&it);
+    const size_t k = efl_size(f);
+    if (k < 2) continue;
+    const ef_dp_res* a = &rs[r++];
+    if ((size_t)a->v[2] != k) { fprintf(stderr, "* FATAL intron refinement backend answered another chain\n"); abort(); }
+    size_t e = 0;
+    ef_iter fi = efl_begin(f);
+    while (efi_has_next(&fi)) memcpy(efi_next(&fi), a->s0 + sizeof(ef_factor) * e++, sizeof(ef_factor));
+    if (a->v[3] == 0) {
+      if (a->v[1]) free(efl_pop_front(f));
+      continue;
+    }
+    const size_t done = (size_t)a->v[0];
+    fi = efl_begin(f);
+    ef_factor* donor = (ef_factor*)efi_next(&fi);
+    for (e = 0; efi_has_next(&fi); ++e) {
+      ef_factor* acc = (ef_factor*)efi_next(&fi);
+      if (e >= done) ef_refine_intron(cfg, gen_info, est_info, donor, acc, e == 0, be, NULL);
+      donor = acc;
+    }
+    fi = efl_begin(f);
+    const ef_factor* e1 = (const ef_factor*)efi_next(&fi);
+    const ef_factor* e2 = (const ef_factor*)efi_next(&fi);
+    if (e1->EST_start == e2->EST_start) free(efl_pop_front(f));
+  }
+  for (r = 0; r < n_req; ++r) ef_dp_res_release(&rs[r]);
+  free(blocks); free(rs); free(rq);
+}
+
 ef_est* ef_get_est_factorizations(const ef_seq* est_info, ef_meg* V, const ef_config* cfg,
                                   const ef_seq* gen_info, ef_backend* be) {
   ef_phase(EFP_EMBED);
@@ -1020,7 +1076,8 @@
     flist = efl_new();
   }
   ef_phase(EFP_INTRON);
-  {
+  if (be->chains) refine_introns_by_chains(flist, cfg, gen_info, est_info, be);
+  else {
     enum { GAP_AHEAD_MAX = 24 };
     ef_gap_ahead* pre = NULL; size_t n_pre = 0;
     if (be->ahead && be->dp_many) {
diff --git a/pintron_amd/host/ef_gpu.h b/pintron_amd/host/ef_gpu.h
--- a/pintron_amd/host/ef_gpu.h
+++ b/pintron_amd/host/ef_gpu.h
@@ -18,6 +18,7 @@
 void ef_dp_trace(const ef_dp_req* q, const ef_dp_res* r, uint32_t unit);
 void ef_dp_trace_flush(void);
 int ef_gpu_device_from_env(void);
+int ef_gpu_chain_route(void);
 
 ef_backend* ef_gpu_open(const ef_seq* gen);
 void ef_gpu_close(ef_backend* be);
diff --git a/pintron_amd/host/ef_gpu_backend.c b/pintron_amd/host/ef_gpu_backend.c
--- a/pintron_amd/host/ef_gpu_backend.c
+++ b/pintron_amd/host/ef_gpu_backend.c
@@ -28,6 +28,15 @@
 }
 void ef_dp_trace_flush(void) { if (trace_file) { pthread_mutex_lock(&trace_mu); fflush(trace_file); pthread_mutex_unlock(&trace_mu); } }
 
+extern int pgpu_dp_has_kind(int kind) __attribute__((weak));
+static int chain_route;
+static pthread_once_t chain_once = PTHREAD_ONCE_INIT;
+static void chain_route_init(void) {
+  const char* e = getenv("PINTRON_REFINE_CHAINS");
+  chain_route = !(e && e[0] == '0' && e[1] == '\0') && !ef_dp_trace_enabled() && pgpu_dp_has_kind && pgpu_dp_has_kind(PGPU_DP_CHAIN);
+}
+int ef_gpu_chain_route(void) { pthread_once(&chain_once, chain_route_init); return chain_route; }
+
 int ef_gpu_device_from_env(void) {
   const char* d = getenv("PINTRON_GPU_DEVICE");
   return d ? atoi(d) : 0;
@@ -57,6 +66,12 @@
   j->kind = (uint32_t)q->kind;
   j->a_len = (uint32_t)q->la; j->b_len = (uint32_t)q->lb;
   j->p0 = q->p0; j->p1 = q->p1; j->p2 = q->p2; j->tail = q->tail;
+  if (q->kind == EF_DP_CHAIN) {
+    j->a_off = put(jb, q->a, q->la);
+    put(jb, "\0\0\0", (size_t)(-(long)jb->arena_len & 3));
+    j->b_off = put(jb, q->b, q->lb);
+    return jb->n++;
+  }
   if (q->a >= gen && q->a + q->la <= gen + gen_len) { j->flags |= PGPU_JOB_A_GENOMIC; j->a_off = (uint64_t)(q->a - gen); }
   else j->a_off = put(jb, q->a, q->la);
   if (q->b >= gen && q->b + q->lb + q->tail <= gen + gen_len) { j->flags |= PGPU_JOB_B_GENOMIC; j->b_off = (uint64_t)(q->b - gen); }
@@ -66,6 +81,14 @@
 
 int ef_decode_result(int kind, const pgpu_dp_result* r, const char* strings, ef_dp_res* out) {
   memset(out, 0, sizeof(*out));
+  if (kind == EF_DP_CHAIN && (r->status == PGPU_OK || r->status == PGPU_ERANGE)) {
+    const size_t n = (size_t)r->v[2];
+    out->v[0] = r->v[0]; out->v[1] = r->v[1]; out->v[2] = r->v[2]; out->v[3] = r->status;
+    out->s0 = (char*)malloc(n * (sizeof(ef_factor) + 1));
+    memcpy(out->s0, strings + r->str[0], n * (sizeof(ef_factor) + 1));
+    out->s1 = out->s0 + n * sizeof(ef_factor);
+    return 0;
+  }
   if (r->status != PGPU_OK) return r->status;
   for (int k = 0; k < 6; ++k) out->v[k] = r->v[k];
   if (kind == EF_DP_ALIGN || kind == EF_DP_GAP) {
@@ -114,7 +137,7 @@
   size_t used = 0;
   const int rc = pgpu_dp_batch(d->ctx, d->idx, d->jb.jobs, 1, d->jb.arena, d->jb.arena_len, &r, d->strings, d->strings_cap, &used);
   if (rc != PGPU_OK) { fprintf(stderr, "* FATAL pgpu_dp_batch: %s\n", pgpu_last_error(d->ctx)); return -1; }
-  if (r.status != PGPU_OK) { fprintf(stderr, "* FATAL DP job of kind %d and size %zu x %zu exceeds the device limits\n", q->kind, q->la, q->lb); return -1; }
+  if (r.status != PGPU_OK && q->kind != EF_DP_CHAIN) { fprintf(stderr, "* FATAL DP job of kind %d and size %zu x %zu exceeds the device limits\n", q->kind, q->la, q->lb); return -1; }
   const int drc = ef_decode_result(q->kind, &r, d->strings, res);
   if (drc == 0) ef_dp_trace(q, res, 0);
   return drc;
@@ -132,7 +155,7 @@
   int rc = pgpu_dp_batch(d->ctx, d->idx, d->jb.jobs, n, d->jb.arena, d->jb.arena_len, r, d->strings, d->strings_cap, &used);
   if (rc != PGPU_OK) fprintf(stderr, "* FATAL pgpu_dp_batch: %s\n", pgpu_last_error(d->ctx));
   for (size_t k = 0; k < n && rc == PGPU_OK; ++k) {
-    if (r[k].status != PGPU_OK) { fprintf(stderr, "* FATAL DP job of kind %d and size %zu x %zu exceeds the device limits\n", reqs[k].kind, reqs[k].la, reqs[k].lb); rc = -1; }
+    if (r[k].status != PGPU_OK && reqs[k].kind != EF_DP_CHAIN) { fprintf(stderr, "* FATAL DP job of kind %d and size %zu x %zu exceeds the device limits\n", reqs[k].kind, reqs[k].la, reqs[k].lb); rc = -1; }
     else { rc = ef_decode_result(reqs[k].kind, &r[k], d->strings, &res[k]); if (rc == PGPU_OK) ef_dp_trace(&reqs[k], &res[k], 0); }
   }
   free(r);
@@ -151,6 +174,7 @@
   ef_jobbuf_init(&d->jb);
   ef_backend* be = (ef_backend*)calloc(1, sizeof(ef_backend));
   be->self = d; be->pairings = direct_pairings; be->dp = direct_dp; be->dp_many = direct_dp_many;
+  be->chains = ef_gpu_chain_route();
   return be;
 }
 
diff --git a/pintron_amd/host/ef_sched.c b/pintron_amd/host/ef_sched.c
--- a/pintron_amd/host/ef_sched.c
+++ b/pintron_amd/host/ef_sched.c
@@ -418,6 +418,7 @@
   else { f = (fiber*)calloc(1, sizeof(fiber)); f->stack = stack_alloc(sh->stack_size, &f->guarded); }
   f->w = w; f->unit = u; f->state = F_RUNNABLE; f->lane = li;
   f->be.self = f; f->be.pairings = fiber_pairings; f->be.dp = fiber_dp; f->be.dp_many = fiber_dp_many; f->be.meg = fiber_meg;
+  f->be.chains = ef_gpu_chain_route();
   memcpy(f->stack, FIBER_SENTINEL, sizeof FIBER_SENTINEL);
 #if EF_TSAN
   if (f->tsan) __tsan_destroy_fiber(f->tsan);
diff --git a/pintron_amd/host/estfact.h b/pintron_amd/host/estfact.h
--- a/pintron_amd/host/estfact.h
+++ b/pintron_amd/host/estfact.h
@@ -215,7 +215,8 @@
 }
 
 enum { EF_DP_ALIGN = 0, EF_DP_GAP = 1, EF_DP_ED = 2, EF_DP_KBAND = 3, EF_DP_LCF = 4,
-       EF_DP_BORDERS = 5, EF_DP_AFFIX = 6 };
+       EF_DP_BORDERS = 5, EF_DP_AFFIX = 6,
+       EF_DP_CHAIN = 7 };
 typedef struct {
   int kind;
   const char* a; size_t la;
@@ -227,6 +228,7 @@
   int32_t v[6];
   char* s0; char* s1;
 } ef_dp_res;
+#define EF_CHAIN_ERANGE (-34)
 #define EF_ROW_PAD 64
 static inline void ef_dp_res_rows(ef_dp_res* r, size_t cap) {
   r->s0 = (char*)calloc(2 * (cap + EF_ROW_PAD), 1);
@@ -253,6 +255,7 @@
   int (*dp_many)(void* self, const ef_dp_req* reqs, ef_dp_res* res, size_t n);
   const void* (*meg)(void* self, const char* pattern, size_t m, const ef_config* cfg);
   ef_ahead* ahead;
+  int chains;
 } ef_backend;
 
 static inline bool ef_req_same(const ef_dp_req* x, const ef_dp_req* y) {
```

After: 468,100. 0.532x the previous value.
